# praateekmahajan/moving-mnist-vae

Hardware: AMD Instinct MI355X
Metric: frames/sec/GPU VAE train step, 20×64×64 batch; ELBO vs CPU ref (higher is better)
Workload: dtype bf16; 1 GPU; BASELINE configs[1]: 256 clips x 20 frames x 64x64 per GPU per step (=5120 frames), conv-VAE z=128, Gaussian NLL sigma=0.1 + KL (normal_vae_1_kl_0_mmd), Adam, random-init weights, Bernoulli(0.0521) q=2 labels; parallelism=dp1, rccl_ranks=1, grad_exchange=none, bn=per-rank batch statistics

## Files before the change

### include/mmvae.h

```cpp
#ifndef MMVAE_H_
#define MMVAE_H_

#include <stddef.h>
#include <stdint.h>

#ifdef __cplusplus
extern "C" {
#endif

#if defined(__GNUC__)
#define MMVAE_API __attribute__((visibility("default")))
#else
#define MMVAE_API
#endif

#define MMVAE_OK 0
#define MMVAE_ERR_ARG (-1)
#define MMVAE_ERR_HIP (-2)
#define MMVAE_ERR_WORKSPACE (-3)
#define MMVAE_ERR_UNSUPPORTED (-4)

#define MMVAE_F32 0
#define MMVAE_BF16 1
#define MMVAE_FP8 2

#define MMVAE_ABI_VERSION 3
MMVAE_API int mmvae_abi_version(void);
MMVAE_API const char* mmvae_last_error(void);

typedef struct mmvae_net mmvae_net;
MMVAE_API int mmvae_net_create(mmvae_net** out, int in_channels, int z_dimension, int out_channels, int image_size,
                     int need_logvar, int dtype);
MMVAE_API int mmvae_net_create_ex(mmvae_net** out, int in_channels, int z_dimension, int out_channels, int image_size,
                        int need_logvar, int dtype, int blocks_per_stage);
MMVAE_API void mmvae_net_destroy(mmvae_net* net);
MMVAE_API int mmvae_net_sizes(const mmvae_net* net, int64_t* n_params, int64_t* n_bn_f32, int32_t* n_bn_i64,
                    int64_t* decoder_param_offset, int32_t* decoder_side);
MMVAE_API int mmvae_net_num_entries(const mmvae_net* net);
MMVAE_API int mmvae_net_entry(const mmvae_net* net, int index, char* name, int name_cap, int32_t* ndim, int32_t shape[4],
                    int32_t* kind, int64_t* offset);
MMVAE_API size_t mmvae_net_workspace_bytes(mmvae_net* net, int N);

MMVAE_API int mmvae_encoder_fwd(mmvae_net* net, int N, const float* x, const float* params, float* bn_f32, int64_t* bn_i64,
                      void* workspace, size_t workspace_bytes, float* mu, float* logvar, int training, void* stream);
MMVAE_API int mmvae_net_stage_labels(mmvae_net* net, int N, const void* labels, int label_bytes, float mean, float stdv, float* image,
                           void* workspace, size_t workspace_bytes, void* stream);
MMVAE_API int mmvae_encoder_fwd_staged(mmvae_net* net, int N, const float* x, const float* params, float* bn_f32, int64_t* bn_i64,
                             void* workspace, size_t workspace_bytes, float* mu, float* logvar, int training, void* stream);
MMVAE_API int mmvae_encoder_bwd(mmvae_net* net, int N, const float* d_mu, const float* d_logvar, const float* params, float* grads,
                      void* workspace, size_t workspace_bytes, void* stream);
MMVAE_API int mmvae_decoder_fwd(mmvae_net* net, int N, const float* encoding, const float* params, float* bn_f32, int64_t* bn_i64,
                      void* workspace, size_t workspace_bytes, float* recon, int training, void* stream);
MMVAE_API int mmvae_decoder_bwd(mmvae_net* net, int N, const float* d_recon, const float* params, float* grads, void* workspace,
                      size_t workspace_bytes, float* d_encoding , void* stream);
MMVAE_API int mmvae_decoder_bwd_gauss(mmvae_net* net, int N, const float* target, float sigma, float coef, const float* gscale, const float* params,
                            float* grads, void* workspace, size_t workspace_bytes, float* d_enc, void* stream);

MMVAE_API int mmvae_net_defer_join(mmvae_net* net, int enable);
MMVAE_API int mmvae_net_join(mmvae_net* net, void* stream);
MMVAE_API void* mmvae_net_fork(mmvae_net* net, void* stream);
MMVAE_API void* mmvae_net_side_stream(mmvae_net* net);
MMVAE_API int mmvae_net_set_join_grad(mmvae_net* net, int enable);

typedef int (*mmvae_allreduce_fn)(float* buf, int64_t n, void* stream, void* user);
MMVAE_API int mmvae_net_set_sync_bn(mmvae_net* net, mmvae_allreduce_fn fn, void* user, int world);

typedef struct mmvae_comm mmvae_comm;
#define MMVAE_COMM_ID_BYTES 128
MMVAE_API int mmvae_comm_unique_id(void* id_host );
MMVAE_API int mmvae_comm_init(mmvae_comm** out, int world, int rank, const void* id_host);
MMVAE_API int mmvae_comm_allreduce(mmvae_comm* comm, float* buf, int64_t n, void* stream);
MMVAE_API int mmvae_comm_destroy(mmvae_comm* comm);
MMVAE_API int mmvae_net_set_sync_bn_comm(mmvae_net* net, mmvae_comm* comm);
MMVAE_API int mmvae_net_set_sync_bn_comm2(mmvae_net* net, mmvae_comm* comm_main, mmvae_comm* comm_side);

MMVAE_API int mmvae_rsample_fwd(const float* mu, const float* logvar, const float* eps, float* enc, int64_t n, void* stream);
MMVAE_API int mmvae_rsample_bwd(const float* d_enc, const float* logvar, const float* eps, float* d_mu, float* d_logvar, int64_t n,
                      void* stream);
#define MMVAE_SUM_PARTIALS 1025
MMVAE_API int mmvae_kl_fwd(const float* mu, const float* logvar, int64_t n, double* acc, void* stream);
MMVAE_API int mmvae_kl_fwd_ex(const float* mu, const float* logvar, int64_t n, double* acc, double* partials, void* stream);
MMVAE_API int mmvae_kl_bwd(const float* mu, const float* logvar, float coef, const float* gscale, float* d_mu, float* d_logvar, int64_t n,
                 void* stream);
MMVAE_API int mmvae_gauss_nll_fwd(const float* recon, const float* target, int64_t n, float sigma, double* acc, void* stream);
MMVAE_API int mmvae_gauss_nll_fwd_ex(const float* recon, const float* target, int64_t n, float sigma, double* acc, double* partials,
                                     void* stream);
MMVAE_API int mmvae_gauss_nll_bwd(const float* recon, const float* target, int64_t n, float sigma, float coef, const float* gscale,
                        float* d_recon, void* stream);
MMVAE_API int mmvae_ce_fwd(const float* recon, const int64_t* target, const float* weight, int N, int Q, int HW, double* acc, void* stream);
MMVAE_API int mmvae_ce_fwd_ex(const float* recon, const int64_t* target, const float* weight, int N, int Q, int HW, double* acc,
                              double* partials, void* stream);
MMVAE_API int mmvae_ce_bwd(const float* recon, const int64_t* target, const float* weight, int N, int Q, int HW, float coef,
                 const float* gscale, float* d_recon, void* stream);
MMVAE_API int mmvae_mmd_fwd(const float* x, const float* y, int n, int d, float* scratch, double* acc, void* stream);
MMVAE_API int mmvae_mmd_fwd_ex(const float* x, const float* y, int n, int d, float* scratch, double* acc, double* partials, void* stream);
MMVAE_API int mmvae_mmd_bwd(const float* x, const float* y, int n, int d, float coef, const float* gscale, float* d_y, void* stream);
MMVAE_API int mmvae_rbf_kernel(const float* x, const float* y, int n, int m, int d, float* out, void* stream);
MMVAE_API int mmvae_loss_finish(const double* acc, float* out, float nll, float kl_coef, float mmd_coef, float n, void* stream);

MMVAE_API int mmvae_gauss_nll_per_image(const float* recon, const float* target, int N, int64_t per, float sigma, double* out, void* stream);
MMVAE_API int mmvae_ce_per_image(const float* recon, const int64_t* target, const float* weight, int N, int Q, int HW, double* out, void* stream);
MMVAE_API int mmvae_kl_per_image(const float* mu, const float* logvar, int N, int d, double* out, void* stream);
MMVAE_API int mmvae_latent_logratio(const float* mu, const float* logvar, const float* eps, int N, int d, double* out, void* stream);
MMVAE_API int mmvae_iw_bound(const double* nll, const double* logratio, int K, int N, double* out, void* stream);

MMVAE_API int mmvae_normalise_labels(const int64_t* labels, int64_t n, float mean, float stdv, float* image, void* stream);
MMVAE_API int mmvae_quantise_normalise(const uint8_t* frames, int64_t n, const float* centres, int q, float mean, float stdv,
                             int64_t* labels, float* image, void* stream);
MMVAE_API int mmvae_u8_histogram(const uint8_t* frames, int64_t clip_bytes, const int64_t* clip_index, int64_t n_clips, uint64_t* counts,
                       void* stream);
MMVAE_API int mmvae_kmeans1d_fit(const uint64_t* counts, int q, double* centres, double* inertia);
MMVAE_API int mmvae_quantiser_stats(const uint64_t* counts, const float* centres, int q, uint8_t* lut, double* ratios, double* label_mean,
                          double* label_std);
MMVAE_API int mmvae_resample_coeffs(int in_size, int out_size, int* ksize, int32_t* bounds, int32_t* coeffs);
MMVAE_API int mmvae_resize_quantise_normalise(const uint8_t* frames, int64_t frame_stride_bytes, const int64_t* clip_index,
// ... 32 lines not shown
MMVAE_API int mmvae_scatter_panel(const float* pts, int64_t n, int stride, int col_x, int col_y, const float* xform, int side, int radius16,
                                  const uint8_t* tone, uint8_t* out, int64_t out_row_stride, void* stream);
MMVAE_API int mmvae_latent_stats(const float* mu, const float* logvar, const float* enc, int N, int d, int accumulate, double* acc,
                                 void* stream);

MMVAE_API size_t mmvae_nearest_frames_scratch_bytes(int M, int64_t F, int D, int k);
MMVAE_API int mmvae_nearest_frames(const uint8_t* queries, int M, const uint8_t* frames, int64_t F, int D, const uint8_t* lut, int k,
                                   int32_t* out_dist, int64_t* out_index, void* scratch, size_t scratch_bytes, void* stream);

#define MMVAE_TENSOR_HIST_BINS 64
#define MMVAE_TENSOR_HIST_STATS 8
MMVAE_API int64_t mmvae_tensor_hist_chunks(const int64_t* segments, int T, int64_t chunk_elems, int64_t* chunks, int64_t capacity);
MMVAE_API size_t mmvae_tensor_hist_scratch_bytes(int T, int64_t n_chunks);
MMVAE_API int mmvae_tensor_hist(const float* flat, int64_t flat_numel, const int64_t* segments, const int64_t* segments_dev, int T,
                                const int64_t* chunks, const int64_t* chunks_dev, int64_t n_chunks, int32_t* counts, float* lo, float* hi,
                                double* stats, void* scratch, size_t scratch_bytes, void* stream);

MMVAE_API int mmvae_adam_step(float* params, const float* grads, float* exp_avg, float* exp_avg_sq, int64_t n, float lr, float beta1,
                    float beta2, float eps, float weight_decay, float bc1, float bc2_sqrt, float grad_scale, void* stream);

MMVAE_API int mmvae_adam_step_dev(float* params, const float* grads, float* exp_avg, float* exp_avg_sq, int64_t n, float lr, float beta1,
                        float beta2, float eps, float weight_decay, double* step_dev, float grad_scale, void* stream);

MMVAE_API int mmvae_grad_norm_sq(const float* grads, int64_t n, float grad_scale, double* acc, double* partials, void* stream);

MMVAE_API int mmvae_adam_step_guarded(float* params, const float* grads, float* exp_avg, float* exp_avg_sq, int64_t n, float lr, float beta1,
                            float beta2, float eps, float weight_decay, double* state, double* partials, float grad_scale,
                            float max_norm, void* stream);

MMVAE_API int mmvae_conv2d_fwd(int dtype, int transposed, const void* x, const float* weight, void* y, int N, int H, int W, int Cin, int Cout,
                     int k, int stride, int pad, const float* pro_scale, const float* pro_shift, int pro_relu, float* stats,
                     void* scratch, void* stream);
MMVAE_API int mmvae_conv2d_dgrad(int dtype, int transposed, const void* dy, const float* weight, void* dx, int N, int H, int W, int Cin,
                       int Cout, int k, int stride, int pad, void* scratch, void* stream);
#define MMVAE_DGRAD_EX_W2_OFFSET(numel_w, esize) ((((size_t)(numel_w) * (esize) + 255) / 256) * 256)
#define MMVAE_DGRAD_EX_SCRATCH_BYTES(numel_w, numel_w2, esize) \
  ((numel_w2) > 0 ? MMVAE_DGRAD_EX_W2_OFFSET(numel_w, esize) + (size_t)(numel_w2) * (esize) : (size_t)(numel_w) * (esize))
MMVAE_API int mmvae_conv2d_dgrad_ex(int dtype, int transposed, const void* dy, const float* weight, void* dx, int N, int H, int W, int Cin,
                          int Cout, int k, int stride, int pad, int accumulate, const void* dy2, const float* w2, int C2, void* scratch,
                          void* stream);
#define MMVAE_WGRAD_SCRATCH_BYTES (64u << 20)
MMVAE_API int mmvae_conv2d_wgrad(int dtype, int transposed, const void* x, const void* dy, float* dweight, int N, int H, int W, int Cin,
                       int Cout, int k, int stride, int pad, const float* pro_scale, const float* pro_shift, int pro_relu,
                       void* scratch, void* stream);
MMVAE_API int mmvae_conv2d_wgrad_pair(int dtype, const void* x, const void* dy, const void* dy_shortcut, float* dweight, float* dweight_sc, int N,
                            int H, int W, int Cin, int Cout, const float* pro_scale, const float* pro_shift, int pro_relu, void* scratch,
                            void* stream);
#define MMVAE_BN_SCRATCH_BYTES (16u << 20)
MMVAE_API int mmvae_batchnorm_fwd(int dtype, const void* y, int64_t npix, int C, const float* gamma, const float* beta, float* running_mean,
                        float* running_var, int64_t* nbt, float momentum, float eps, int relu, void* out, float* save_mean, float* save_istd,
                        void* scratch, void* stream);
MMVAE_API int mmvae_batchnorm_bwd(int dtype, const void* dout, const void* y, const void* out, int64_t npix, int C, const float* gamma,
                        const float* save_mean, const float* save_istd, void* dy, float* dgamma, float* dbeta, void* scratch, void* stream);
#define MMVAE_STEM_SCRATCH_BYTES 12800u
MMVAE_API int mmvae_stem_fwd(int dtype, const void* x, const float* weight, void* y, int N, int S, float* stats, void* scratch, void* stream);
MMVAE_API int mmvae_stem_bwd(int dtype, const void* g, const void* y0, const void* x, const float* weight, const float* gamma,
                   const float* bn_scale, const float* bn_shift, const float* save_mean, const float* save_istd, float* dweight,
                   float* dgamma, float* dbeta, int N, int S, void* scratch, void* stream);
MMVAE_API int mmvae_convT_bwd_fused(int dtype, const void* x, const void* dy, const float* weight, float* dweight, void* dx, int N, int H, int W,
                          int Cin, int Cout, int k, int stride, int pad, const float* pro_scale, const float* pro_shift, int pro_relu,
                          const void* x2, const float* w2, float* dw2, void* scratch, void* wscratch, void* stream);
MMVAE_API int mmvae_tail_join_fwd(int dtype, const void* y2, const float* s2, const float* b2, const void* ys, const float* ss, const float* bs,
                        const float* weight, const float* bias, float* r_raw, float* stats, int N, int H, int W, void* stream);
MMVAE_API int mmvae_tail_join_fwd_stream(int dtype, const void* y2, const float* s2, const float* b2, const void* ys, const float* ss, const float* bs,
                               const float* weight, const float* bias, float* r_raw, float* stats, int N, int H, int W, void* stream);
MMVAE_API int mmvae_tail_join_bwd_reduce(int dtype, const float* d_raw, const float* weight, int out_planes, const void* y2, const float* s2,
                               const float* b2, const void* ys, const float* ss, const float* bs, float* partials, float* wpartials,
                               int N, int H, int W, void* stream);
MMVAE_API int mmvae_tail_join_bwd_apply(int dtype, const float* d_raw, const float* weight, int out_planes, const void* y2, const float* s2,
                              const float* b2, const void* ys, const float* ss, const float* bs, const float* A2, const float* B2,
                              const float* C2, const float* As, const float* Bs, const float* Cs, void* dy2, void* dys, int N, int H, int W,
                              void* stream);
MMVAE_API int mmvae_upblock_bwd_fused(const float* d_raw, const float* tail_weight, const void* y2, const float* s2, const float* b2,
                            const void* ys, const float* ss, const float* bs, const float* A2, const float* B2, const float* C2,
                            const float* As, const float* Bs, const float* Cs, const void* y1, const float* s1, const float* b1,
                            const float* w_conv2, float* dw_conv2, void* d_a1, float* bn1_sums, const void* xin, const float* sx,
                            const float* bx, const float* w_up, float* dw_up, void* g_in, int N, void* scratch, void* stream);
MMVAE_API int mmvae_upblock_tail_fwd(const void* y1, const float* s1, const float* b1, const float* w2, const void* x_in, const float* sx,
                                     const float* bx, const float* wu, const float* s2, const float* b2, const float* ss, const float* bs,
                                     const float* tail_weight, const float* tail_bias, float* r_raw, float* stats, int N, void* scratch,
                                     void* stream);
MMVAE_API int mmvae_upblock_tail_fwd_store(const void* y1, const float* s1, const float* b1, const float* w2, const void* x_in, const float* sx,
                                           const float* bx, const float* wu, const float* s2, const float* b2, const float* ss, const float* bs,
                                           const float* tail_weight, const float* tail_bias, float* r_raw, float* stats, void* y2, void* ys,
                                           int N, void* scratch, void* stream);
MMVAE_API int mmvae_convT4_stats(int dtype, const void* x, const float* weight, const float* pro_scale, const float* pro_shift, float* stats,
                                 int N, int e4m3_out, void* scratch, void* stream);
MMVAE_API int mmvae_join_conv1x1_fwd(const void* y2, const float* s2, const float* b2, const void* ys, const float* ss, const float* bs,
                           const float* w_conv1, int C, void* out, void* y1, float* stats, int64_t npix, void* scratch, void* stream);
MMVAE_API int mmvae_conv1x1_bwd_fused(const void* d_a1, const void* y1, const float* s1, const float* b1, const float* A1, const float* B1,
                            const float* C1, const void* xin, const float* sx, const float* bx, const float* w_conv1, float* dw_conv1,
                            void* g_in, int64_t rows, void* scratch, void* stream);
typedef struct mmvae_pixelcnn mmvae_pixelcnn;
MMVAE_API int mmvae_pixelcnn_create(mmvae_pixelcnn** out, int in_channels, int intermediate_channels, int out_channels, int layers, int dtype);
MMVAE_API void mmvae_pixelcnn_destroy(mmvae_pixelcnn* net);
MMVAE_API int64_t mmvae_pixelcnn_num_params(mmvae_pixelcnn* net);
MMVAE_API size_t mmvae_pixelcnn_workspace_bytes(mmvae_pixelcnn* net, int N, int S);
MMVAE_API int mmvae_pixelcnn_fwd(mmvae_pixelcnn* net, int N, int S, const float* x, const float* params, void* workspace, size_t workspace_bytes,
                       float* out, void* stream);
MMVAE_API int mmvae_pixelcnn_bwd(mmvae_pixelcnn* net, int N, int S, const float* x, const float* d_out, const float* params, float* grads,
                       void* workspace, size_t workspace_bytes, float* d_x, void* stream);
MMVAE_API size_t mmvae_pixelcnn_sample_workspace_bytes(mmvae_pixelcnn* net, int N, int S);
MMVAE_API int mmvae_pixelcnn_sample(mmvae_pixelcnn* net, int N, int S, const float* cond, int cond_channels, float* sample, int sample_channels,
                          const float* uniforms, float sub_mean, float data_std, const float* params, void* workspace, size_t workspace_bytes,
                          float* out_logits, float* probs, int64_t* labels, void* stream);

// ... 7 lines not shown
```

### moving-mnist-vae_amd/_lib.py

```python
from __future__ import annotations

import ctypes
import os
from ctypes import POINTER, c_char_p, c_double, c_float, c_int, c_int32, c_int64, c_size_t, c_uint64, c_void_p

import torch

_HERE = os.path.dirname(os.path.abspath(__file__))
LIB_PATH = os.environ.get("MMVAE_LIB_PATH") or os.path.join(_HERE, "libmmvae_hip.so")
_lib = None
ABI_VERSION = 3
SUM_PARTIALS = 1025
BN_SCRATCH_BYTES = 16 << 20
STEM_SCRATCH_BYTES = 12800

P = c_void_p

PROTOTYPES = {
    "mmvae_abi_version": (c_int, []),
    "mmvae_last_error": (c_char_p, []),
    "mmvae_net_create": (c_int, [POINTER(c_void_p), c_int, c_int, c_int, c_int, c_int, c_int]),
    "mmvae_net_create_ex": (c_int, [POINTER(c_void_p), c_int, c_int, c_int, c_int, c_int, c_int, c_int]),
    "mmvae_net_destroy": (None, [P]),
    "mmvae_net_sizes": (c_int, [P, POINTER(c_int64), POINTER(c_int64), POINTER(c_int32), POINTER(c_int64), POINTER(c_int32)]),
    "mmvae_net_num_entries": (c_int, [P]),
    "mmvae_net_entry": (c_int, [P, c_int, c_char_p, c_int, POINTER(c_int32), POINTER(c_int32), POINTER(c_int32), POINTER(c_int64)]),
    "mmvae_net_workspace_bytes": (c_size_t, [P, c_int]),
    "mmvae_encoder_fwd": (c_int, [P, c_int, P, P, P, P, P, c_size_t, P, P, c_int, P]),
    "mmvae_net_stage_labels": (c_int, [P, c_int, P, c_int, c_float, c_float, P, P, c_size_t, P]),
    "mmvae_encoder_fwd_staged": (c_int, [P, c_int, P, P, P, P, P, c_size_t, P, P, c_int, P]),
    "mmvae_encoder_bwd": (c_int, [P, c_int, P, P, P, P, P, c_size_t, P]),
    "mmvae_decoder_fwd": (c_int, [P, c_int, P, P, P, P, P, c_size_t, P, c_int, P]),
    "mmvae_decoder_bwd": (c_int, [P, c_int, P, P, P, P, c_size_t, P, P]),
    "mmvae_decoder_bwd_gauss": (c_int, [P, c_int, P, c_float, c_float, P, P, P, P, c_size_t, P, P]),
    "mmvae_net_defer_join": (c_int, [P, c_int]),
    "mmvae_net_join": (c_int, [P, P]),
    "mmvae_net_fork": (P, [P, P]),
    "mmvae_net_side_stream": (P, [P]),
    "mmvae_net_set_join_grad": (c_int, [P, c_int]),
    "mmvae_net_set_sync_bn": (c_int, [P, P, P, c_int]),
    "mmvae_rsample_fwd": (c_int, [P, P, P, P, c_int64, P]),
    "mmvae_rsample_bwd": (c_int, [P, P, P, P, P, c_int64, P]),
    "mmvae_kl_fwd": (c_int, [P, P, c_int64, P, P]),
    "mmvae_kl_fwd_ex": (c_int, [P, P, c_int64, P, P, P]),
    "mmvae_kl_bwd": (c_int, [P, P, c_float, P, P, P, c_int64, P]),
    "mmvae_gauss_nll_fwd": (c_int, [P, P, c_int64, c_float, P, P]),
    "mmvae_gauss_nll_fwd_ex": (c_int, [P, P, c_int64, c_float, P, P, P]),
    "mmvae_gauss_nll_bwd": (c_int, [P, P, c_int64, c_float, c_float, P, P, P]),
    "mmvae_ce_fwd": (c_int, [P, P, P, c_int, c_int, c_int, P, P]),
    "mmvae_ce_fwd_ex": (c_int, [P, P, P, c_int, c_int, c_int, P, P, P]),
    "mmvae_ce_bwd": (c_int, [P, P, P, c_int, c_int, c_int, c_float, P, P, P]),
    "mmvae_mmd_fwd": (c_int, [P, P, c_int, c_int, P, P, P]),
    "mmvae_mmd_fwd_ex": (c_int, [P, P, c_int, c_int, P, P, P, P]),
    "mmvae_mmd_bwd": (c_int, [P, P, c_int, c_int, c_float, P, P, P]),
    "mmvae_loss_finish": (c_int, [P, P, c_float, c_float, c_float, c_float, P]),
    "mmvae_gauss_nll_per_image": (c_int, [P, P, c_int, c_int64, c_float, P, P]),
    "mmvae_ce_per_image": (c_int, [P, P, P, c_int, c_int, c_int, P, P]),
    "mmvae_kl_per_image": (c_int, [P, P, c_int, c_int, P, P]),
    "mmvae_latent_logratio": (c_int, [P, P, P, c_int, c_int, P, P]),
    "mmvae_iw_bound": (c_int, [P, P, c_int, c_int, P, P]),
    "mmvae_normalise_labels": (c_int, [P, c_int64, c_float, c_float, P, P]),
    "mmvae_quantise_normalise": (c_int, [P, c_int64, P, c_int, c_float, c_float, P, P, P]),
    "mmvae_u8_histogram": (c_int, [P, c_int64, P, c_int64, P, P]),
    "mmvae_kmeans1d_fit": (c_int, [P, c_int, P, P]),
    "mmvae_quantiser_stats": (c_int, [P, P, c_int, P, P, P, P]),
    "mmvae_resample_coeffs": (c_int, [c_int, c_int, POINTER(c_int), P, P]),
    "mmvae_resize_quantise_normalise": (c_int, [P, c_int64, P, c_int, c_int64, c_int, c_int, c_int, c_int, P, P, c_int, P, P, c_int, P, c_int,
                                                c_float, c_float, P, P, P, P]),
    "mmvae_generate_clips": (c_int, [P, c_int64, c_int, P, c_uint64, c_int64, c_int64, c_int, c_int, c_int, P, c_int, c_float, c_float, P, P, P, P]),
    "mmvae_logits_to_labels": (c_int, [P, c_int, c_int, c_int, c_int, P, P, P]),
    "mmvae_panel_sheet": (c_int, [P, c_int, c_int, c_int, P, P]),
    "mmvae_scatter_panel": (c_int, [P, c_int64, c_int, c_int, c_int, P, c_int, c_int, P, P, c_int64, P]),
    "mmvae_latent_stats": (c_int, [P, P, P, c_int, c_int, c_int, P, P]),
    "mmvae_nearest_frames_scratch_bytes": (c_size_t, [c_int, c_int64, c_int, c_int]),
    "mmvae_nearest_frames": (c_int, [P, c_int, P, c_int64, c_int, P, c_int, P, P, P, c_size_t, P]),
    "mmvae_tensor_hist_chunks": (c_int64, [P, c_int, c_int64, P, c_int64]),
    "mmvae_tensor_hist_scratch_bytes": (c_size_t, [c_int, c_int64]),
    "mmvae_tensor_hist": (c_int, [P, c_int64, P, P, c_int, P, P, c_int64, P, P, P, P, P, c_size_t, P]),
    "mmvae_adam_step": (c_int, [P, P, P, P, c_int64, c_float, c_float, c_float, c_float, c_float, c_float, c_float, c_float, P]),
    "mmvae_adam_step_dev": (c_int, [P, P, P, P, c_int64, c_float, c_float, c_float, c_float, c_float, P, c_float, P]),
    "mmvae_grad_norm_sq": (c_int, [P, c_int64, c_float, P, P, P]),
    "mmvae_adam_step_guarded": (c_int, [P, P, P, P, c_int64, c_float, c_float, c_float, c_float, c_float, P, P, c_float, c_float, P]),
    "mmvae_conv2d_fwd": (c_int, [c_int, c_int, P, P, P, c_int, c_int, c_int, c_int, c_int, c_int, c_int, c_int, P, P, c_int, P, P, P]),
    "mmvae_conv2d_dgrad": (c_int, [c_int, c_int, P, P, P, c_int, c_int, c_int, c_int, c_int, c_int, c_int, c_int, P, P]),
    "mmvae_conv2d_dgrad_ex": (c_int, [c_int, c_int, P, P, P, c_int, c_int, c_int, c_int, c_int, c_int, c_int, c_int, c_int, P, P, c_int, P, P]),
    "mmvae_conv2d_wgrad": (c_int, [c_int, c_int, P, P, P, c_int, c_int, c_int, c_int, c_int, c_int, c_int, c_int, P, P, c_int, P, P]),
    "mmvae_conv2d_wgrad_pair": (c_int, [c_int, P, P, P, P, P, c_int, c_int, c_int, c_int, c_int, P, P, c_int, P, P]),
    "mmvae_rbf_kernel": (c_int, [P, P, c_int, c_int, c_int, P, P]),
    "mmvae_comm_unique_id": (c_int, [P]),
    "mmvae_comm_init": (c_int, [POINTER(c_void_p), c_int, c_int, P]),
    "mmvae_comm_allreduce": (c_int, [P, P, c_int64, P]),
    "mmvae_comm_destroy": (c_int, [P]),
    "mmvae_net_set_sync_bn_comm": (c_int, [P, P]),
    "mmvae_net_set_sync_bn_comm2": (c_int, [P, P, P]),
    "mmvae_convT_bwd_fused": (c_int, [c_int, P, P, P, P, P, c_int, c_int, c_int, c_int, c_int, c_int, c_int, c_int, P, P, c_int, P, P, P, P, P, P]),
    "mmvae_batchnorm_fwd": (c_int, [c_int, P, c_int64, c_int, P, P, P, P, P, c_float, c_float, c_int, P, P, P, P, P]),
    "mmvae_batchnorm_bwd": (c_int, [c_int, P, P, P, c_int64, c_int, P, P, P, P, P, P, P, P]),
    "mmvae_stem_fwd": (c_int, [c_int, P, P, P, c_int, c_int, P, P, P]),
    "mmvae_stem_bwd": (c_int, [c_int, P, P, P, P, P, P, P, P, P, P, P, P, c_int, c_int, P, P]),
    "mmvae_tail_join_fwd": (c_int, [c_int, P, P, P, P, P, P, P, P, P, P, c_int, c_int, c_int, P]),
    "mmvae_tail_join_fwd_stream": (c_int, [c_int, P, P, P, P, P, P, P, P, P, P, c_int, c_int, c_int, P]),
    "mmvae_tail_join_bwd_reduce": (c_int, [c_int, P, P, c_int, P, P, P, P, P, P, P, P, c_int, c_int, c_int, P]),
    "mmvae_tail_join_bwd_apply": (c_int, [c_int, P, P, c_int, P, P, P, P, P, P, P, P, P, P, P, P, P, P, c_int, c_int, c_int, P]),
    "mmvae_upblock_bwd_fused": (c_int, [P] * 27 + [c_int, P, P]),
    "mmvae_join_conv1x1_fwd": (c_int, [P, P, P, P, P, P, P, c_int, P, P, P, c_int64, P, P]),
    "mmvae_conv1x1_bwd_fused": (c_int, [P] * 13 + [c_int64, P, P]),
    "mmvae_upblock_tail_fwd": (c_int, [P] * 16 + [c_int, P, P]),
    "mmvae_upblock_tail_fwd_store": (c_int, [P] * 18 + [c_int, P, P]),
    "mmvae_convT4_stats": (c_int, [c_int, P, P, P, P, P, c_int, c_int, P, P]),
    "mmvae_pixelcnn_create": (c_int, [POINTER(c_void_p), c_int, c_int, c_int, c_int, c_int]),
    "mmvae_pixelcnn_destroy": (None, [P]),
    "mmvae_pixelcnn_num_params": (c_int64, [P]),
    "mmvae_pixelcnn_workspace_bytes": (c_size_t, [P, c_int, c_int]),
    "mmvae_pixelcnn_fwd": (c_int, [P, c_int, c_int, P, P, P, c_size_t, P, P]),
    "mmvae_pixelcnn_bwd": (c_int, [P, c_int, c_int, P, P, P, P, P, c_size_t, P, P]),
    "mmvae_pixelcnn_sample_workspace_bytes": (c_size_t, [P, c_int, c_int]),
    "mmvae_pixelcnn_sample": (c_int, [P, c_int, c_int, P, c_int, P, c_int, P, c_float, c_float, P, P, c_size_t, P, P, P, P]),
    "mmvae_convert": (c_int, [c_int, c_int, P, P, c_int64, P]),
}


class MmvaeError(RuntimeError):
    pass


PICK_ARGMAX, PICK_SAMPLE = 0, 1
PANEL_LABELS_U8, PANEL_LABELS_I64, PANEL_LOGITS_ARGMAX, PANEL_LOGITS_SAMPLE, PANEL_IMAGE_F32 = range(5)
PANEL_MAX_COLS, PANEL_MAX_Q, PANEL_MAX_S = 8, 16, 64
SCATTER_MAX_SIDE, SCATTER_MIN_RADIUS16, SCATTER_MAX_RADIUS16 = 512, 12, 128
LATENT_STATS_ROWS, LATENT_STATS_MAX_D = 6, 512
NEAREST_MAX_M, NEAREST_MAX_K, NEAREST_MAX_D = 64, 8, 16384
CLIPGEN_MAX_G, CLIPGEN_MAX_T, CLIPGEN_MAX_K, CLIPGEN_MAX_D, CLIPGEN_DIRECTIONS = 32, 32, 4, 1 << 24, 4096


class PanelCol(ctypes.Structure):
    _fields_ = [("kind", c_int32), ("src", c_void_p), ("Q", c_int32), ("uniforms", c_void_p), ("lut", c_void_p), ("lo", c_float),
                ("hi", c_float)]


def lib():
    global _lib
    if _lib is not None:
        return _lib
    if not os.path.exists(LIB_PATH):
        raise MmvaeError(
            f"{LIB_PATH} is missing: the HIP extension has not been built. "
            "Run `python -c 'import __graft_entry__ as g; g.build()'` (or `make -C moving-mnist-vae_amd/csrc`). "
            "There is no CPU fallback for the product path.")
    l = ctypes.CDLL(LIB_PATH)
    l.mmvae_abi_version.restype, l.mmvae_abi_version.argtypes = c_int, []
# ... 45 lines not shown
```

### moving-mnist-vae_amd/csrc/bn_elem.hip

```cpp
#include "kernels.hpp"
#include "tile_common.hpp"
#include <cstdlib>

namespace mmvae {

constexpr int kElemMaxBlocks = 768;

__host__ __device__ inline int block_threads_for(int cvecs) {
  int b = 256 - (256 % cvecs);
  return b < cvecs ? cvecs : b;
}

static int elem_blocks(long nvec, int threads) {
  constexpr int cap = kElemMaxBlocks;
  long b = (nvec + (long)threads * 4 - 1) / ((long)threads * 4);
  if (b < 1) b = 1;
  if (b > cap) b = cap;
  return (int)b;
}

template <int NV, int VE>
__device__ __forceinline__ void block_channel_reduce(float (&vals)[NV][VE], int cvecs, int C, float* smem, float* out) {
  const int t = threadIdx.x;
#pragma unroll
// ... 266 lines not shown
      if (MODE == 3) { float x = a0[j] * msc[j] + msh[j]; x += a1[j] * msc1[j] + msh1[j]; on = x > 0.f; }
      const float gg = on ? g[j] : 0.f;
      acc[0][j] += gg;
      acc[1][j] += gg * a0[j];
      if (NY == 2) acc[2][j] += gg * a1[j];
    }
  }
  block_channel_reduce<1 + NY, VE>(acc, cvecs, C, smem, partials + (long)blockIdx.x * (1 + NY) * C);
}

template <typename T>
static int launch_bn_bwd_reduce_t(const void* dout, const void* out, const float* ms, const float* mb, const float* ms1,
                                  const float* mb1, const void* y0, const void* y1, long npix, int C, float* partials, hipStream_t s) {
  constexpr int VE = Elem<T>::kVec;
  if (C % VE) { set_error("bn_bwd_reduce: C=%d not a multiple of %d", C, VE); return MMVAE_ERR_UNSUPPORTED; }
  const int cvecs = C / VE, threads = block_threads_for(cvecs);
  const long nvec = npix * cvecs;
  int blocks = elem_blocks(nvec, threads);
  if (blocks > 1024) blocks = 1024;
  const int ny = y1 ? 2 : 1;
  const size_t sm = (size_t)threads * (1 + ny) * VE * sizeof(float);
  const int mode = out ? 0 : (ms ? ((ms1 && ny == 2) ? 3 : 1) : 2);
#define MMVAE_LAUNCH(NY, MODE) hipLaunchKernelGGL((bn_bwd_reduce_kernel<T, NY, MODE>), dim3(blocks), dim3(threads), sm, s, \
    (const T*)dout, (const T*)out, ms, mb, ms1, mb1, (const T*)y0, (const T*)y1, nvec, C, partials)
  if (ny == 2) { if (mode == 0) MMVAE_LAUNCH(2, 0); else if (mode == 1) MMVAE_LAUNCH(2, 1); else if (mode == 3) MMVAE_LAUNCH(2, 3); else MMVAE_LAUNCH(2, 2); }
  else { if (mode == 0) MMVAE_LAUNCH(1, 0); else if (mode == 1) MMVAE_LAUNCH(1, 1); else MMVAE_LAUNCH(1, 2); }
#undef MMVAE_LAUNCH
  note_launch_bytes((double)npix * C * sizeof(T) * (1 + ny + (out ? 1 : 0)));
  int rc = check_launch("bn_bwd_reduce");
  return rc ? rc : blocks;
}
int launch_bn_bwd_reduce(int dt, const void* dout, const void* out, const float* msk_scale, const float* msk_shift,
                         const void* y0, const void* y1, long npix, int C, float* partials, hipStream_t s,
                         const float* msk_scale1, const float* msk_shift1) {
  return dt == DT_F32 ? launch_bn_bwd_reduce_t<float>(dout, out, msk_scale, msk_shift, msk_scale1, msk_shift1, y0, y1, npix, C, partials, s)
                      : launch_bn_bwd_reduce_t<bf16_t>(dout, out, msk_scale, msk_shift, msk_scale1, msk_shift1, y0, y1, npix, C, partials, s);
}

__global__ void bn_bwd_finalize_kernel(BnBwdFinalizeArgs a0, BnBwdFinalizeArgs a1) {
  const BnBwdFinalizeArgs& a = blockIdx.y ? a1 : a0;
  __shared__ double sRed[2 * 4];
  const int c = blockIdx.x;
  const int rows = 1 + a.ny;
  double s0 = 0.0, s1 = 0.0;
  strided_pair_sum<8>(a.partials + c, a.partials + (long)(1 + a.which) * a.C + c, (long)rows * a.C, a.nparts, s0, s1);
  s0 = wave_sum_d(s0); s1 = wave_sum_d(s1);
  const int lane = threadIdx.x & 63, wid = threadIdx.x >> 6;
  if (lane == 0) { sRed[wid] = s0; sRed[4 + wid] = s1; }
  __syncthreads();
  if (threadIdx.x == 0) {
    const int nw = blockDim.x >> 6;
    s0 = 0.0; s1 = 0.0;
    for (int w = 0; w < nw; ++w) { s0 += sRed[w]; s1 += sRed[4 + w]; }
    const double mean = a.mean[c], istd = a.istd[c], g = a.gamma ? a.gamma[c] : 1.0;
    const double sgy = istd * (s1 - mean * s0);
    if (a.dgamma) a.dgamma[c] += (float)sgy;
    if (a.dbeta) a.dbeta[c] += (float)s0;
    const double m1 = s0 / a.count, m2 = sgy / a.count;
    const double A = g * istd;
    const float Af = (float)A, Bf = (float)(-A * m2 * istd), Cf = (float)(-A * m1 + A * m2 * istd * mean);
    a.coefA[c] = Af;
    a.coefB[c] = Bf;
    a.coefC[c] = Cf;
    if (a.dbias_conv) a.dbias_conv[c] += (float)(((double)Af * s0 + (double)Bf * (mean * a.count) + (double)Cf * a.count) * (double)a.dbias_scale);
  }
}
int launch_bn_bwd_finalize(const BnBwdFinalizeArgs& a, hipStream_t s) {
  hipLaunchKernelGGL(bn_bwd_finalize_kernel, dim3(a.C), dim3(256), 0, s, a, a);
  return check_launch("bn_bwd_finalize");
}
int launch_bn_bwd_finalize2(const BnBwdFinalizeArgs& a0, const BnBwdFinalizeArgs& a1, hipStream_t s) {
  if (a0.C != a1.C) { set_error("bn_bwd_finalize2: channel counts differ"); return MMVAE_ERR_ARG; }
  hipLaunchKernelGGL(bn_bwd_finalize_kernel, dim3(a0.C, 2), dim3(256), 0, s, a0, a1);
  return check_launch("bn_bwd_finalize2");
}

template <typename T, int NY, int MODE>
__global__ void bn_bwd_apply_kernel(const T* __restrict__ dout, const T* __restrict__ out, const float* __restrict__ ms,
                                    const float* __restrict__ mb, const float* __restrict__ ms1, const float* __restrict__ mb1,
                                    const T* __restrict__ y0, const float* __restrict__ A0,
                                    const float* __restrict__ B0, const float* __restrict__ C0, T* __restrict__ dy0,
                                    const T* __restrict__ y1, const float* __restrict__ A1, const float* __restrict__ B1,
                                    const float* __restrict__ C1, T* __restrict__ dy1, long nvec, int C) {
  constexpr int VE = Elem<T>::kVec;
  const int cvecs = C / VE;
  const int cg = (int)(((long)blockIdx.x * blockDim.x + threadIdx.x) % cvecs);
  float msc[VE], msh[VE], msc1[VE], msh1[VE], a0[VE], b0[VE], c0[VE], a1[VE], b1[VE], c1[VE];
#pragma unroll
  for (int j = 0; j < VE; ++j) {
    const int ch = cg * VE + j;
    msc[j] = (MODE == 1 || MODE == 3) ? ms[ch] : 0.f; msh[j] = (MODE == 1 || MODE == 3) ? mb[ch] : 0.f;
    msc1[j] = MODE == 3 ? ms1[ch] : 0.f; msh1[j] = MODE == 3 ? mb1[ch] : 0.f;
    a0[j] = A0[ch]; b0[j] = B0[ch]; c0[j] = C0[ch];
    a1[j] = NY == 2 ? A1[ch] : 0.f; b1[j] = NY == 2 ? B1[ch] : 0.f; c1[j] = NY == 2 ? C1[ch] : 0.f;
  }
  const long stride = (long)gridDim.x * blockDim.x;
  for (long v = (long)blockIdx.x * blockDim.x + threadIdx.x; v < nvec; v += stride) {
    float g[VE], o[VE], f0[VE], f1[VE], r0[VE], r1[VE];
    Elem<T>::unpack(reinterpret_cast<const Vec16*>(dout)[v], g);
    Elem<T>::unpack(reinterpret_cast<const Vec16*>(y0)[v], f0);
    if (MODE == 0) Elem<T>::unpack(reinterpret_cast<const Vec16*>(out)[v], o);
    if (NY == 2) Elem<T>::unpack(reinterpret_cast<const Vec16*>(y1)[v], f1);
#pragma unroll
    for (int j = 0; j < VE; ++j) {
      bool on = true;
      if (MODE == 0) on = o[j] > 0.f;
// ... 714 lines not shown
int launch_affine_nchw(const float* raw, const float* scale, const float* shift, float* out, int N, int C, int HW, hipStream_t s) {
  const long total = (long)N * C * HW;
  const int blocks = elem_blocks(total / 4 + 1, 256);
  hipLaunchKernelGGL(affine_nchw_kernel, dim3(blocks), dim3(256), 0, s, raw, scale, shift, out, total, C, HW);
  note_launch_bytes((double)total * 8.0);
  return check_launch("affine_nchw");
}
__global__ __launch_bounds__(256) void gauss_tail_reduce_kernel(const float* __restrict__ raw, const float* __restrict__ tgt, const float* __restrict__ scale,
                                                                 const float* __restrict__ shift, float k, const float* __restrict__ gs, int N, int C,
                                                                 int HW, float* __restrict__ partials) {
  extern __shared__ float sm[];
  float* sAcc = sm;
  const int wid = threadIdx.x >> 6;
  if (gs) k *= gs[0];
  for (int i = threadIdx.x; i < 4 * 2 * C; i += blockDim.x) sAcc[i] = 0.f;
  __syncthreads();
  const int planes = N * C;
  for (int p = blockIdx.x; p < planes; p += gridDim.x) {
    const int c = p % C;
    const float sc = scale[c], sh = shift[c];
    const float* pa = raw + (long)p * HW;
    const float* pt = tgt + (long)p * HW;
    float v0 = 0.f, v1 = 0.f;
    if ((HW & 3) == 0) {
      for (int i = threadIdx.x * 4; i < HW; i += 4 * blockDim.x) {
        const float4 x = *reinterpret_cast<const float4*>(pa + i);
        const float4 t = *reinterpret_cast<const float4*>(pt + i);
        const float d0 = k * ((sc * x.x + sh) - t.x), d1 = k * ((sc * x.y + sh) - t.y), d2 = k * ((sc * x.z + sh) - t.z), d3 = k * ((sc * x.w + sh) - t.w);
        v0 += (d0 + d1) + (d2 + d3);
        v1 += (d0 * x.x + d1 * x.y) + (d2 * x.z + d3 * x.w);
      }
    } else {
      for (int i = threadIdx.x; i < HW; i += blockDim.x) {
        const float x = pa[i], d = k * ((sc * x + sh) - pt[i]);
        v0 += d; v1 += d * x;
      }
    }
    v0 = wave_sum(v0); v1 = wave_sum(v1);
    if ((threadIdx.x & 63) == 0) { sAcc[wid * 2 * C + c] += v0; sAcc[wid * 2 * C + C + c] += v1; }
  }
  __syncthreads();
  for (int i = threadIdx.x; i < 2 * C; i += blockDim.x)
    partials[(long)blockIdx.x * 2 * C + i] = (sAcc[i] + sAcc[2 * C + i]) + (sAcc[2 * 2 * C + i] + sAcc[3 * 2 * C + i]);
}
int launch_gauss_tail_reduce(const float* raw, const float* target, const float* scale, const float* shift, float sigma, float coef, const float* gscale,
                             int N, int C, int HW, float* partials, hipStream_t s) {
  const int blocks = nchw_parts(N, C);
  const size_t sm = (size_t)4 * 2 * C * sizeof(float);
  hipLaunchKernelGGL(gauss_tail_reduce_kernel, dim3(blocks), dim3(256), sm, s, raw, target, scale, shift, coef / (sigma * sigma), gscale, N, C, HW, partials);
  note_launch_bytes((double)N * C * HW * 8.0);
  const int rc = check_launch("gauss_tail_reduce");
  return rc ? rc : blocks;
}
__global__ __launch_bounds__(256) void gauss_tail_apply_kernel(const float* __restrict__ raw, const float* __restrict__ tgt, const float* __restrict__ scale,
                                                                const float* __restrict__ shift, float k, const float* __restrict__ gs,
                                                                const float* __restrict__ A, const float* __restrict__ B, const float* __restrict__ Cc,
                                                                float* __restrict__ dy, int planes, int C, int HW) {
  if (gs) k *= gs[0];
  for (int p = blockIdx.x; p < planes; p += gridDim.x) {
    const int c = p % C;
    const float sc = scale[c], sh = shift[c], ca = A[c], cb = B[c], cc = Cc[c];
    const long base = (long)p * HW;
    if ((HW & 3) == 0) {
      for (int i = threadIdx.x * 4; i < HW; i += 1024) {
        const float4 x = *reinterpret_cast<const float4*>(raw + base + i);
        const float4 t = *reinterpret_cast<const float4*>(tgt + base + i);
        float4 o;
        o.x = ca * (k * ((sc * x.x + sh) - t.x)) + cb * x.x + cc; o.y = ca * (k * ((sc * x.y + sh) - t.y)) + cb * x.y + cc;
        o.z = ca * (k * ((sc * x.z + sh) - t.z)) + cb * x.z + cc; o.w = ca * (k * ((sc * x.w + sh) - t.w)) + cb * x.w + cc;
        *reinterpret_cast<float4*>(dy + base + i) = o;
      }
    } else {
      for (int i = threadIdx.x; i < HW; i += 256) {
        const float x = raw[base + i];
        dy[base + i] = ca * (k * ((sc * x + sh) - tgt[base + i])) + cb * x + cc;
      }
    }
  }
}
int launch_gauss_tail_apply(const float* raw, const float* target, const float* scale, const float* shift, float sigma, float coef, const float* gscale,
                            const float* A, const float* B, const float* Cc, float* dy, int N, int C, int HW, hipStream_t s) {
  if (C > 64) { set_error("gauss_tail_apply: C=%d > 64", C); return MMVAE_ERR_UNSUPPORTED; }
  const int planes = N * C;
  const int blocks = planes < 4096 ? planes : 4096;
  hipLaunchKernelGGL(gauss_tail_apply_kernel, dim3(blocks), dim3(256), 0, s, raw, target, scale, shift, coef / (sigma * sigma), gscale, A, B, Cc, dy, planes, C, HW);
  note_launch_bytes((double)N * C * HW * 12.0);
  return check_launch("gauss_tail_apply");
}

__global__ __launch_bounds__(256) void bn_bwd_apply_nchw_kernel(const float* __restrict__ dout, const float* __restrict__ y,
                                                                const float* __restrict__ A, const float* __restrict__ B,
                                                                const float* __restrict__ Cc, float* __restrict__ dy, int planes, int C,
                                                                int HW) {
  for (int p = blockIdx.x; p < planes; p += gridDim.x) {
    const int c = p % C;
    const float ca = A[c], cb = B[c], cc = Cc[c];
    const long base = (long)p * HW;
    if ((HW & 3) == 0) {
      for (int i = threadIdx.x * 4; i < HW; i += 1024) {
        const float4 d = *reinterpret_cast<const float4*>(dout + base + i);
        const float4 v = *reinterpret_cast<const float4*>(y + base + i);
        float4 o;
        o.x = ca * d.x + cb * v.x + cc; o.y = ca * d.y + cb * v.y + cc; o.z = ca * d.z + cb * v.z + cc; o.w = ca * d.w + cb * v.w + cc;
        *reinterpret_cast<float4*>(dy + base + i) = o;
      }
    } else {
      for (int i = threadIdx.x; i < HW; i += 256) dy[base + i] = ca * dout[base + i] + cb * y[base + i] + cc;
    }
  }
}
int launch_bn_bwd_apply_nchw(const float* dout, const float* y, const float* A, const float* B, const float* Cc, float* dy,
                             int N, int C, int HW, hipStream_t s) {
  if (C > 64) { set_error("bn_bwd_apply_nchw: C=%d > 64", C); return MMVAE_ERR_UNSUPPORTED; }
  const int planes = N * C;
  const int blocks = planes < 4096 ? planes : 4096;
  hipLaunchKernelGGL(bn_bwd_apply_nchw_kernel, dim3(blocks), dim3(256), 0, s, dout, y, A, B, Cc, dy, planes, C, HW);
  return check_launch("bn_bwd_apply_nchw");
}

}
```

### moving-mnist-vae_amd/csrc/capi.cpp

```cpp
#include <cstring>
#include <new>

#include "../../include/mmvae.h"
#include "conv_ops.hpp"
#include "pixel_net.hpp"
#include "quantiser_fit.hpp"
#include "resample.hpp"
#include "vae_net.hpp"

namespace mmvae { const char* last_error(); }
using namespace mmvae;

struct mmvae_net { Net* net; };
struct mmvae_comm { Comm* c; };

static inline hipStream_t stream_of(void* s) { return static_cast<hipStream_t>(s); }

extern "C" {

int mmvae_abi_version(void) { return MMVAE_ABI_VERSION; }
const char* mmvae_last_error(void) { return last_error(); }

int mmvae_net_create(mmvae_net** out, int in_channels, int z, int out_channels, int image_size, int need_logvar, int dtype) {
  return mmvae_net_create_ex(out, in_channels, z, out_channels, image_size, need_logvar, dtype, 1);
// ... 33 lines not shown
  const Entry& e = n->net->entries[i];
  if (name && cap > 0) { std::strncpy(name, e.name.c_str(), cap - 1); name[cap - 1] = 0; }
  if (ndim) *ndim = e.ndim;
  if (shape) for (int k = 0; k < 4; ++k) shape[k] = e.shape[k];
  if (kind) *kind = e.kind;
  if (offset) *offset = e.offset;
  return MMVAE_OK;
}
size_t mmvae_net_workspace_bytes(mmvae_net* n, int N) { return n && N > 0 ? n->net->workspace_bytes(N) : 0; }

int mmvae_encoder_fwd(mmvae_net* n, int N, const float* x, const float* params, float* bn_f32, int64_t* bn_i64, void* ws, size_t wsb,
                      float* mu, float* logvar, int training, void* stream) {
  if (!n || N <= 0 || !x || !params || !ws || !mu) { set_error("encoder_fwd: bad argument"); return MMVAE_ERR_ARG; }
  if (n->net->cfg.need_logvar && !logvar) { set_error("encoder_fwd: logvar required"); return MMVAE_ERR_ARG; }
  if (!bn_f32) { set_error("encoder_fwd: BN buffers required"); return MMVAE_ERR_ARG; }
  return n->net->encoder_fwd(N, x, params, bn_f32, reinterpret_cast<long long*>(bn_i64), ws, wsb, mu, logvar, training, stream_of(stream));
}
int mmvae_net_stage_labels(mmvae_net* n, int N, const void* labels, int label_bytes, float mean, float stdv, float* image, void* ws, size_t wsb,
                           void* stream) {
  if (!n || N <= 0 || !labels || !image || !ws) { set_error("net_stage_labels: bad argument"); return MMVAE_ERR_ARG; }
  return n->net->stage_labels(N, labels, label_bytes, mean, stdv, image, ws, wsb, stream_of(stream));
}
int mmvae_encoder_fwd_staged(mmvae_net* n, int N, const float* x, const float* params, float* bn_f32, int64_t* bn_i64, void* ws, size_t wsb,
                             float* mu, float* logvar, int training, void* stream) {
  if (!n || N <= 0 || !x || !params || !ws || !mu) { set_error("encoder_fwd_staged: bad argument"); return MMVAE_ERR_ARG; }
  if (n->net->cfg.need_logvar && !logvar) { set_error("encoder_fwd_staged: logvar required"); return MMVAE_ERR_ARG; }
  if (!bn_f32) { set_error("encoder_fwd_staged: BN buffers required"); return MMVAE_ERR_ARG; }
  return n->net->encoder_fwd(N, x, params, bn_f32, reinterpret_cast<long long*>(bn_i64), ws, wsb, mu, logvar, training, stream_of(stream), true);
}
int mmvae_encoder_bwd(mmvae_net* n, int N, const float* d_mu, const float* d_logvar, const float* params, float* grads, void* ws,
                      size_t wsb, void* stream) {
  if (!n || N <= 0 || !d_mu || !params || !grads || !ws) { set_error("encoder_bwd: bad argument"); return MMVAE_ERR_ARG; }
  if (n->net->cfg.need_logvar && !d_logvar) { set_error("encoder_bwd: d_logvar required"); return MMVAE_ERR_ARG; }
  return n->net->encoder_bwd(N, d_mu, d_logvar, params, grads, ws, wsb, stream_of(stream));
}
int mmvae_decoder_fwd(mmvae_net* n, int N, const float* enc, const float* params, float* bn_f32, int64_t* bn_i64, void* ws, size_t wsb,
                      float* recon, int training, void* stream) {
  if (!n || N <= 0 || !enc || !params || !ws || !recon || !bn_f32) { set_error("decoder_fwd: bad argument"); return MMVAE_ERR_ARG; }
  return n->net->decoder_fwd(N, enc, params, bn_f32, reinterpret_cast<long long*>(bn_i64), ws, wsb, recon, training, stream_of(stream));
}
int mmvae_decoder_bwd(mmvae_net* n, int N, const float* d_recon, const float* params, float* grads, void* ws, size_t wsb, float* d_enc,
                      void* stream) {
  if (!n || N <= 0 || !d_recon || !params || !grads || !ws) { set_error("decoder_bwd: bad argument"); return MMVAE_ERR_ARG; }
  return n->net->decoder_bwd(N, d_recon, params, grads, ws, wsb, d_enc, stream_of(stream));
}

int mmvae_decoder_bwd_gauss(mmvae_net* n, int N, const float* target, float sigma, float coef, const float* gscale, const float* params, float* grads,
                            void* ws, size_t wsb, float* d_enc, void* stream) {
  if (!n || N <= 0 || !target || !params || !grads || !ws || !(sigma > 0.f)) { set_error("decoder_bwd_gauss: bad argument"); return MMVAE_ERR_ARG; }
  const Net::GaussTail gt{target, sigma, coef, gscale};
  return n->net->decoder_bwd(N, nullptr, params, grads, ws, wsb, d_enc, stream_of(stream), &gt);
}

int mmvae_net_defer_join(mmvae_net* n, int enable) {
  if (!n) { set_error("net_defer_join: bad argument"); return MMVAE_ERR_ARG; }
  n->net->set_defer_join(enable != 0);
  return MMVAE_OK;
}
int mmvae_net_join(mmvae_net* n, void* stream) {
  if (!n) { set_error("net_join: bad argument"); return MMVAE_ERR_ARG; }
  return n->net->join(stream_of(stream));
}

void* mmvae_net_fork(mmvae_net* n, void* stream) {
  if (!n) return stream;
  return reinterpret_cast<void*>(n->net->fork(stream_of(stream)));
}

int mmvae_net_set_join_grad(mmvae_net* n, int enable) {
  if (!n) { set_error("net_set_join_grad: bad argument"); return MMVAE_ERR_ARG; }
  n->net->set_join_grad(enable != 0);
  return MMVAE_OK;
}

void* mmvae_net_side_stream(mmvae_net* n) { return n ? reinterpret_cast<void*>(n->net->side()) : nullptr; }

int mmvae_net_set_sync_bn(mmvae_net* n, mmvae_allreduce_fn fn, void* user, int world) {
  if (!n || (fn && world < 1)) { set_error("net_set_sync_bn: bad argument"); return MMVAE_ERR_ARG; }
  n->net->set_sync_bn(reinterpret_cast<mmvae::Net::AllReduceFn>(fn), user, world);
  return MMVAE_OK;
}

int mmvae_comm_unique_id(void* id) {
  if (!id) { set_error("comm_unique_id: bad argument"); return MMVAE_ERR_ARG; }
  return comm_unique_id(id);
}
int mmvae_comm_init(mmvae_comm** out, int world, int rank, const void* id) {
  if (!out || !id || world < 1 || rank < 0 || rank >= world) { set_error("comm_init: bad argument"); return MMVAE_ERR_ARG; }
  mmvae_comm* h = new (std::nothrow) mmvae_comm;
  if (!h) return MMVAE_ERR_ARG;
  h->c = nullptr;
  const int rc = comm_init(&h->c, world, rank, id);
  if (rc < 0) { delete h; return rc; }
  *out = h;
  return MMVAE_OK;
}
int mmvae_comm_allreduce(mmvae_comm* c, float* buf, int64_t n, void* st) {
  if (!c || (!buf && n > 0)) { set_error("comm_allreduce: bad argument"); return MMVAE_ERR_ARG; }
  return comm_allreduce_sum(c->c, buf, (long long)n, stream_of(st));
}
int mmvae_comm_destroy(mmvae_comm* c) {
  if (!c) return MMVAE_OK;
  const int rc = comm_destroy(c->c);
  delete c;
  return rc;
}
// ... 318 lines not shown
  if (rc == 0) { set_error("conv2d_wgrad_pair: shape not supported (bf16, 32 -> 32 channels, 32x32 -> 16x16)"); return MMVAE_ERR_UNSUPPORTED; }
  return rc < 0 ? rc : MMVAE_OK;
}
int mmvae_convT_bwd_fused(int dt, const void* x, const void* dy, const float* w, float* dw, void* dx, int N, int H, int W, int Cin, int Cout, int k,
                          int s, int p, const float* ps, const float* pb, int relu, const void* x2, const float* w2, float* dw2, void* scratch,
                          void* wscratch, void* st) {
  const ConvGeom g = geom_for(1, Cin, Cout, k, s, p);
  const int Ho = out_size(1, H, k, s, p), Wo = out_size(1, W, k, s, p);
  if (!scratch || !wscratch) { set_error("convT_bwd_fused: scratch buffers required"); return MMVAE_ERR_ARG; }
  if (!op_bwd_fusable(dt, g, N, H, W, Ho, Wo)) { set_error("convT_bwd_fused: shape not supported (bf16, 16 / 32 -> 16 channels, k4 s2 p1, 32x32 -> 64x64 or 16x16 -> 32x32)"); return MMVAE_ERR_UNSUPPORTED; }
  char* sc = static_cast<char*>(scratch);
  int rc = op_pack_down(dt, g, w, sc, stream_of(st)); if (rc < 0) return rc;
  const void* w2p = nullptr;
  if (x2 && w2) {
    PackArgs pa; std::memset(&pa, 0, sizeof(pa));
    pa.src = w2; pa.dst = sc + (size_t)Cin * Cout * k * k * dtype_size(dt); pa.cols = Cin; pa.K = 16; pa.ntaps = 1; pa.s_col = 16; pa.s_k = 1; pa.scale = 1.f; pa.tap_off[0] = 0;
    rc = launch_pack(dt, pa, stream_of(st)); if (rc < 0) return rc;
    w2p = pa.dst;
  }
  if (dw2 && !w2p) { set_error("convT_bwd_fused: dw2 needs x2 and w2"); return MMVAE_ERR_ARG; }
  rc = op_run_bwd_fused(dt, g, N, x, H, W, ps, pb, relu, dy, Ho, Wo, sc, dx, w2p ? x2 : nullptr, w2p, dw, stream_of(st), static_cast<float*>(wscratch), 1.f,
                        nullptr, dw2, 1.f);
  if (rc == 0) { set_error("convT_bwd_fused: not taken"); return MMVAE_ERR_UNSUPPORTED; }
  return rc < 0 ? rc : MMVAE_OK;
}
static_assert(MMVAE_BN_SCRATCH_BYTES >= (1024u * 3 * 512 + 8 * 512) * 4, "BatchNorm scratch: 1024 partial rows x 3 x C<=512 + coefficient rows");
int mmvae_batchnorm_fwd(int dt, const void* y, int64_t npix, int C, const float* gamma, const float* beta, float* rm, float* rv, int64_t* nbt,
                        float momentum, float eps, int relu, void* out, float* save_mean, float* save_istd, void* scratch, void* st) {
  if (!scratch || !save_mean || !save_istd || C < 1 || C > 512 || npix < 1) { set_error("batchnorm_fwd: bad arguments (C <= 512, scratch and save_* required)"); return MMVAE_ERR_ARG; }
  float* part = static_cast<float*>(scratch);
  float* coef = part + 1024L * 3 * 512;
  const int np = launch_chan_stats_nhwc(dt, y, npix, C, part, stream_of(st));
  if (np < 0) return np;
  BnFinalizeArgs f;
  f.partials = part; f.nparts = np; f.C = C; f.count = (double)npix; f.gamma = gamma; f.beta = beta; f.running_mean = rm; f.running_var = rv;
  f.nbt = reinterpret_cast<long long*>(nbt); f.mean = save_mean; f.istd = save_istd; f.scale = coef; f.shift = coef + C; f.momentum = momentum; f.eps = eps;
  int rc = launch_bn_finalize(f, stream_of(st));
  if (rc < 0) return rc;
  return launch_affine_act(dt, y, coef, coef + C, relu, out, npix, C, stream_of(st));
}
int mmvae_batchnorm_bwd(int dt, const void* dout, const void* y, const void* out, int64_t npix, int C, const float* gamma, const float* save_mean,
                        const float* save_istd, void* dy, float* dgamma, float* dbeta, void* scratch, void* st) {
  if (!scratch || C < 1 || C > 512 || npix < 1) { set_error("batchnorm_bwd: bad arguments (C <= 512, scratch required)"); return MMVAE_ERR_ARG; }
  float* part = static_cast<float*>(scratch);
  float* coef = part + 1024L * 3 * 512;
  const int np = launch_bn_bwd_reduce(dt, dout, out, nullptr, nullptr, y, nullptr, npix, C, part, stream_of(st));
  if (np < 0) return np;
  BnBwdFinalizeArgs f; std::memset(&f, 0, sizeof(f));
  f.partials = part; f.nparts = np; f.C = C; f.which = 0; f.ny = 1; f.count = (double)npix; f.gamma = gamma; f.mean = save_mean; f.istd = save_istd;
  f.dgamma = dgamma; f.dbeta = dbeta; f.coefA = coef; f.coefB = coef + C; f.coefC = coef + 2 * C;
  int rc = launch_bn_bwd_finalize(f, stream_of(st));
  if (rc < 0) return rc;
  return launch_bn_bwd_apply(dt, dout, out, nullptr, nullptr, y, coef, coef + C, coef + 2 * C, dy, nullptr, nullptr, nullptr, nullptr, nullptr, npix, C, stream_of(st));
}
static_assert(MMVAE_STEM_SCRATCH_BYTES >= 32 * 25 * 16, "stem scratch: 32 columns x 25 taps x one 16-byte vector of padded input channels");
int mmvae_stem_fwd(int dt, const void* x, const float* w, void* y, int N, int Sz, float* stats, void* scratch, void* st) {
  if (!scratch || N < 1 || Sz < 9 || Sz > 64) { set_error("stem_fwd: bad arguments"); return MMVAE_ERR_ARG; }
  if (stem_fwd_stream_ok(dt, Sz)) return launch_stem_fwd_stream(dt, x, w, y, stats, N, Sz, stream_of(st));
  const int H1 = (Sz + 4 - 5) / 2 + 1;
  const int cpad = dt == DT_F32 ? 4 : 8;
  PackArgs pa; std::memset(&pa, 0, sizeof(pa));
  pa.src = w; pa.dst = scratch;
  pa.cols = 32; pa.K = cpad; pa.K_valid = 1; pa.ntaps = 25; pa.s_col = 25; pa.s_k = 25; pa.scale = 1.f;
  for (int t = 0; t < 25; ++t) pa.tap_off[t] = t;
  int rc = launch_pack(dt, pa, stream_of(st));
  if (rc < 0) return rc;
  GatherArgs a; std::memset(&a, 0, sizeof(a));
  a.x = x; a.w = scratch; a.y = y; a.stats = stats;
  a.x_planar = 2; a.x_planes = 1;
  a.N = N; a.Hi = Sz; a.Wi = Sz; a.Cin = cpad; a.Ho = H1; a.Wo = H1; a.Cout = 32; a.SI = 2; a.SO = 1;
  a.nphase = 1; a.phases[0] = Phase{0, 0, H1, H1, 25, 0, 0};
  for (int kh = 0; kh < 5; ++kh) for (int kw = 0; kw < 5; ++kw) a.taps[kh * 5 + kw] = Tap{kh - 2, kw - 2};
  return launch_gather_gemm(dt, dt, a, stream_of(st));
}
int mmvae_stem_bwd(int dt, const void* g, const void* y0, const void* x, const float* w, const float* gamma, const float* bn_scale,
                   const float* bn_shift, const float* save_mean, const float* save_istd, float* dw, float* dgamma, float* dbeta, int N, int Sz,
                   void* scratch, void* st) {
  if (!scratch || N < 1) { set_error("stem_bwd: bad arguments"); return MMVAE_ERR_ARG; }
  if (!stem_bwd_fusable(Sz)) { set_error("stem_bwd: image size %d unsupported (64, 32, 16)", Sz); return MMVAE_ERR_UNSUPPORTED; }
  const int H1 = (Sz + 4 - 5) / 2 + 1;
  double* R = static_cast<double*>(scratch);
  float* gram = reinterpret_cast<float*>(R + 1024);
  const long gram_floats = 1024L * stem_bwd_part_floats();
  float* part = gram + gram_floats;
  const long part_floats = (long)(MMVAE_BN_SCRATCH_BYTES - 1024 * 8) / 4 - gram_floats;
  int rc = launch_stem_gram(dt, x, gram, gram_floats, R, N, Sz, H1, H1, stream_of(st));
  if (rc < 0) return rc;
  const int np = launch_stem_bwd(dt, g, y0, x, bn_scale, bn_shift, part, part_floats, N, Sz, H1, H1, stream_of(st));
  if (np < 0) return np;
  return launch_stem_bwd_finalize(part, np, R, w, nullptr, (double)N * H1 * H1, gamma, save_mean, save_istd, dgamma, dbeta, dw, stream_of(st));
}
int mmvae_tail_join_fwd(int dt, const void* y2, const float* s2, const float* b2, const void* ys, const float* ss, const float* bs,
                        const float* w, const float* bias, float* r_raw, float* stats, int N, int H, int W, void* st) {
  return launch_tail_join_fwd(dt, y2, s2, b2, ys, ss, bs, w, bias, r_raw, stats, N, H, W, stream_of(st));
}
int mmvae_tail_join_fwd_stream(int dt, const void* y2, const float* s2, const float* b2, const void* ys, const float* ss, const float* bs,
                               const float* w, const float* bias, float* r_raw, float* stats, int N, int H, int W, void* st) {
  return launch_tail_fwd_stream(dt, y2, s2, b2, ys, ss, bs, w, bias, r_raw, stats, N, H, W, stream_of(st));
}
int mmvae_tail_join_bwd_reduce(int dt, const float* d_raw, const float* w, int oc, const void* y2, const float* s2, const float* b2,
                               const void* ys, const float* ss, const float* bs, float* partials, float* wpartials, int N, int H, int W,
                               void* st) {
  return launch_tail_join_bwd_reduce(dt, d_raw, w, oc, N, H, W, s2, b2, ss, bs, y2, ys, partials, stream_of(st), wpartials);
}
int mmvae_tail_join_bwd_apply(int dt, const float* d_raw, const float* w, int oc, const void* y2, const float* s2, const float* b2,
                              const void* ys, const float* ss, const float* bs, const float* A2, const float* B2, const float* C2,
// ... 95 lines not shown
```

### moving-mnist-vae_amd/csrc/kernels.hpp

```cpp
#pragma once
#include "common.hpp"

namespace mmvae {

enum DType : int { DT_F32 = 0, DT_BF16 = 1 };
inline size_t dtype_size(int dt) { return dt == DT_F32 ? 4 : 2; }

struct Tap { int dh, dw; };
constexpr int kMaxTaps = 25;
constexpr int kMaxPhases = 4;
struct Phase { int ph, pw, Hq, Wq, ntaps, tap0; long w_off;  };
struct GatherArgs {
  const void* x; const void* w; void* y;
  const float* pro_scale; const float* pro_shift; int pro_relu;
  const float* bias;
  float* stats;
  int accumulate;
  int N, Hi, Wi, Cin, Ho, Wo, Cout;
  int SI, SO;
  int nphase; Phase phases[kMaxPhases]; Tap taps[kMaxTaps];
  int cin_vecs;
  int x_planar, x_planes;
  int y_planes;
  const void* x2; const void* w2; int Cin2, x2_ph, x2_pw;
// ... 139 lines not shown
bool stem_bwd_fusable(int S);
bool conv3_stream_ok(int dt, int Cin, int Cout, int k, int s, int p, int Hin, int Win);
int launch_conv3_stream_bwd(int dt, const void* dy, const void* w_flipped, void* dx, const void* ym, const float* ms, const float* mb, float* sums,
                            int N, int H, hipStream_t s);
int launch_conv3_stream(int dt, int stride, const void* x, const void* w, const void* wsc, void* y, void* ysc, const float* pro_scale,
                        const float* pro_shift, int pro_relu, float* stats, float* stats_sc, int N, int Ho, hipStream_t s);
bool convT4_stream_ok(int dt, int Cin, int Cout, int k, int s, int p, int Hin, int Win);
int launch_convT4_stream(int dt, const void* x, const void* w_up, void* y, const float* pro_scale, const float* pro_shift, int pro_relu, float* stats,
                         int N, int Hin, hipStream_t s, int f8out = 0);
bool tail_fwd_stream_ok(int dt, int OC, int H, int W);
int launch_tail_fwd_stream(int dt, const void* y2, const float* s2, const float* b2, const void* ys, const float* ss, const float* bs, const float* w,
                           const float* bias, float* r_raw, float* stats, int N, int H, int W, hipStream_t s, int f8in = 0);
bool up5_tail_fwd_ok(int dt, int OC, int C, int Cin, int Hin, int Hout);
int launch_up5_tail_fwd(const void* y1, const float* p1s, const float* p1b, const void* w2_up, const void* xin, const float* pxs, const float* pxb,
                        const void* wu_up, const float* s2, const float* b2, const float* ss, const float* bs, const float* w, const float* bias,
                        float* r_raw, float* stats, int N, hipStream_t s, void* y2 = nullptr, void* ys = nullptr);
bool stem_fwd_stream_ok(int dt, int S);
int launch_stem_fwd_stream(int dt, const void* x, const float* w, void* y, float* stats, int N, int S, hipStream_t s);
int stem_bwd_part_floats();
int launch_stem_gram(int dt, const void* x, float* scratch, long scratch_cap_floats, double* R, int N, int S, int Ho, int Wo, hipStream_t s);
int launch_stem_bwd(int dt, const void* g, const void* y0, const void* x, const float* ms, const float* mb, float* partials,
                    long partials_cap_floats, int N, int S, int Ho, int Wo, hipStream_t s);
bool stem_bwd_dg_ok(int dt, int S);
int launch_stem_bwd_dg(const void* dy1, const void* dys, const void* wd1, const void* wds, const void* y0, const void* x, const float* ms, const float* mb,
                       float* partials, long partials_cap_floats, int N, int S, int Ho, int Wo, hipStream_t s);
int launch_stem_bwd_finalize(const float* partials, int nparts, const double* R, const float* w, const float* global_sums, double count,
                             const float* gamma, const float* mean, const float* istd, float* dgamma, float* dbeta, float* dW, hipStream_t s);

int launch_chan_stats_nhwc(int dt, const void* y, long npix, int C, float* partials, hipStream_t s);
int chan_stats_parts(long npix, int C);
struct BnFinalizeArgs {
  float in_scale = 1.f;
  const float* partials; int nparts; int C; double count;
  const float* gamma; const float* beta; float* running_mean; float* running_var; long long* nbt;
  float* mean; float* istd; float* scale; float* shift; float momentum, eps;
};
int launch_bn_finalize(const BnFinalizeArgs& a, hipStream_t s);
int launch_partial_rowsum(const float* partials, int nparts, int width, float* out, hipStream_t s, int row_stride = 0);
struct BnFoldEntry { int g_off, b_off, rm_off, rv_off, scale_off, shift_off, C; float in_scale; };
constexpr int kBnFoldMax = 96;
struct BnFoldTable { BnFoldEntry e[kBnFoldMax]; };
int launch_bn_fold_eval(const BnFoldEntry* entries, int n, const float* params, const float* bnbuf, float* bnws, float eps, hipStream_t s);
int launch_join_fwd(int dt, const void* a, const float* sa, const float* ba, const void* b, const float* sb, const float* bb,
                    void* out, long npix, int C, hipStream_t s);
int launch_affine_act(int dt, const void* a, const float* sa, const float* ba, int relu, void* out, long npix, int C,
                      hipStream_t s);
int launch_bn_bwd_reduce(int dt, const void* dout, const void* out, const float* msk_scale, const float* msk_shift,
                         const void* y0, const void* y1, long npix, int C, float* partials, hipStream_t s,
                         const float* msk_scale1 = nullptr, const float* msk_shift1 = nullptr);
struct BnBwdFinalizeArgs {
  const float* partials; int nparts; int C; int which ; int ny; double count;
  const float* gamma; const float* mean; const float* istd; float* dgamma; float* dbeta; float* coefA; float* coefB; float* coefC;
  float* dbias_conv = nullptr; float dbias_scale = 1.f;
};
int launch_bn_bwd_finalize(const BnBwdFinalizeArgs& a, hipStream_t s);
int launch_bn_bwd_finalize2(const BnBwdFinalizeArgs& a0, const BnBwdFinalizeArgs& a1, hipStream_t s);
int launch_bn_bwd_apply(int dt, const void* dout, const void* out, const float* msk_scale, const float* msk_shift,
                        const void* y0, const float* A0, const float* B0, const float* C0, void* dy0,
                        const void* y1, const float* A1, const float* B1, const float* C1, void* dy1,
                        long npix, int C, hipStream_t s, const float* msk_scale1 = nullptr, const float* msk_shift1 = nullptr);
bool tail_join_fusable(int dt, int OC, int N, int H, int W);
int launch_tail_join_bwd_reduce(int dt, const float* d_raw, const float* w, int OC, int N, int H, int W, const float* ms, const float* mb,
                                const float* ms1, const float* mb1, const void* y0, const void* y1, float* partials, hipStream_t s,
                                float* wpartials = nullptr, int f8in = 0);
int launch_tail_wgrad_finalize(const float* wpartials, int nparts, float* dW, hipStream_t s);
int launch_tail_join_bwd_apply(int dt, const float* d_raw, const float* w, int OC, int N, int H, int W, const float* ms, const float* mb,
                               const float* ms1, const float* mb1, const void* y0, const float* A0, const float* B0, const float* C0, void* dy0,
                               const void* y1, const float* A1, const float* B1, const float* C1, void* dy1, hipStream_t s);
bool tail_fwd_fusable(int dt, int OC, int N, int H, int W);
int launch_tail_join_fwd(int dt, const void* y0, const float* ms, const float* mb, const void* y1, const float* ms1, const float* mb1,
                         const float* w, const float* bias, float* r_raw, float* stats, int N, int H, int W, hipStream_t s);
int launch_affine_nchw(const float* raw, const float* scale, const float* shift, float* out, int N, int C, int HW, hipStream_t s);
int launch_bn_bwd_reduce_nchw(const float* dout, const float* y, int N, int C, int HW, float* partials, hipStream_t s);
int launch_bn_bwd_apply_nchw(const float* dout, const float* y, const float* A, const float* B, const float* Cc, float* dy,
                             int N, int C, int HW, hipStream_t s);
int launch_gauss_tail_reduce(const float* raw, const float* target, const float* scale, const float* shift, float sigma, float coef, const float* gscale,
                             int N, int C, int HW, float* partials, hipStream_t s);
int launch_gauss_tail_apply(const float* raw, const float* target, const float* scale, const float* shift, float sigma, float coef, const float* gscale,
                            const float* A, const float* B, const float* Cc, float* dy, int N, int C, int HW, hipStream_t s);

int launch_inorm_planar_fwd(int dt, const float* x, void* xn16, float* stats, int N, int C, int HW, hipStream_t s);
int launch_inorm_planar2_fwd(int dt, const float* xa, int Ca, const float* xb, int Cb, void* xn16, float* stats, int N, int HW, hipStream_t s);
int launch_inorm_planar_bwd(int dt, const void* g16, const float* x, const float* stats, float* dx, int N, int C, int HW, hipStream_t s);
int launch_inorm_nhwc_fwd(int dt, const void* h, void* a, float* stats, int N, int C, int HW, int relu, hipStream_t s);
int launch_inorm_nhwc_bwd(int dt, const void* g, const void* h, const float* stats, void* dh, int N, int C, int HW, int relu, hipStream_t s);
int launch_nhwc16_to_planar(int dt, const void* o16, float* out, int N, int C, int HW, hipStream_t s);
int launch_planar_to_nhwc16(int dt, const float* in, void* o16, int N, int C, int HW, hipStream_t s);
int launch_planar_to_nhwc16(int dt, const void* in, int in_dt, void* o16, int N, int C, int HW, hipStream_t s);

struct PixelHeadArgs {
  const void* a;
  const void* w;
  const float* bias;
  const float* uniforms;
  float* sample;
  float* probs;
  long long* labels;
  int S, C, Q, ntaps, Cs, pix;
  float sub_mean, data_std;
};
int launch_pixel_head(int dt, const PixelHeadArgs& h, int N, hipStream_t s);

int launch_rsample_fwd(int dt, const float* mu, const float* logvar, const float* eps, float* enc_f32, void* enc_t, long n,
                       hipStream_t s);
int launch_rsample_bwd(const float* d_enc, const float* logvar, const float* eps, float* d_mu, float* d_logvar, long n, hipStream_t s);
int launch_kl_fwd(const float* mu, const float* logvar, long n, double* out, double* part, hipStream_t s);
int launch_kl_bwd(const float* mu, const float* logvar, float coef, const float* gscale, float* d_mu, float* d_logvar, long n, hipStream_t s);
int launch_gauss_nll_fwd(const float* r, const float* t, long n, float sigma, double* out, double* part, hipStream_t s);
int launch_gauss_nll_bwd(const float* r, const float* t, long n, float sigma, float coef, const float* gscale, float* d_r, hipStream_t s);
int launch_ce_fwd(const float* r, const long long* t, const float* w, int N, int Q, int HW, double* out, double* part, hipStream_t s);
int launch_ce_bwd(const float* r, const long long* t, const float* w, int N, int Q, int HW, float coef, const float* gscale, float* d_r,
                  hipStream_t s);
int launch_mmd_fwd(const float* x, const float* y, int n, int d, double* out, double* part, hipStream_t s);
int launch_mmd_fwd_mfma(const float* x, const float* y, int n, int d, float* scratch , double* out, double* part, hipStream_t s);
int launch_rbf_matrix(const float* x, const float* y, int n, int m, int d, float* out, hipStream_t s);
int launch_mmd_bwd(const float* x, const float* y, int n, int d, float coef, const float* gscale, float* d_y, hipStream_t s);

int launch_gauss_nll_per_image(const float* r, const float* t, int N, long per, float sigma, double* out, hipStream_t s);
int launch_ce_per_image(const float* r, const long long* t, const float* w, int N, int Q, int HW, double* out, hipStream_t s);
int launch_kl_per_image(const float* mu, const float* logvar, int N, int d, double* out, hipStream_t s);
int launch_latent_logratio(const float* mu, const float* logvar, const float* eps, int N, int d, double* out, hipStream_t s);
int launch_iw_bound(const double* nll, const double* logratio, int K, int N, double* out, hipStream_t s);

struct AdamArgs { float* p; const float* g; float* m; float* v; long n; float lr, beta1, beta2, eps, weight_decay; float bc1, bc2; float grad_scale; };
int launch_adam(const AdamArgs& a, hipStream_t s);
int launch_adam_dev(const AdamArgs& a, double* state, hipStream_t s);
int launch_grad_norm_sq(const float* g, long n, float grad_scale, double* acc, double* part, hipStream_t s);
int launch_adam_guarded(const AdamArgs& a, double* state, double* part, float max_norm, hipStream_t s);
int launch_normalise(int dt, const void* labels, int label_bytes, long n, float mean, float stdv, void* img_t, float* img_f32, hipStream_t s);
int launch_quantise_normalise(const unsigned char* frames, long n, const float* centres, int q, float mean, float stdv,
                              long long* labels, float* image, hipStream_t s);
int launch_u8_histogram(const unsigned char* frames, long clip_bytes, const long long* clip_index, long n_clips,
                        unsigned long long* counts, hipStream_t s);
int launch_resize_quantise_normalise(const unsigned char* frames, long frame_stride, const long long* clip_index, int frames_per_clip,
                                     long n_frames, int in_h, int in_w, int out_h, int out_w, const int* h_bounds, const int* h_coeffs,
                                     int h_ksize, const int* v_bounds, const int* v_coeffs, int v_ksize, const float* centres, int q,
                                     float mean, float stdv, long long* labels, float* image, unsigned char* resized, hipStream_t s);
constexpr int kClipGenMaxG = MMVAE_CLIPGEN_MAX_G, kClipGenMaxT = MMVAE_CLIPGEN_MAX_T, kClipGenMaxK = MMVAE_CLIPGEN_MAX_K;
constexpr long kClipGenMaxD = MMVAE_CLIPGEN_MAX_D;
int launch_generate_clips(const unsigned char* bank, long D, int G, const int* vel, unsigned long long seed, long first_clip, long n_clips,
                          int T, int S, int K, const float* centres, int q, float mean, float stdv, long long* labels, float* image,
                          unsigned char* bytes, hipStream_t s);
int launch_logits_to_labels(const float* logits, int N, int Q, int HW, int mode, const float* uniforms, long long* labels, hipStream_t s);
int launch_panel_sheet(const mmvae_panel_col* cols, int ncols, int n, int S, unsigned char* out, hipStream_t s);
int launch_scatter_panel(const float* pts, long n, int stride, int col_x, int col_y, const float* xform, int side, int radius16,
                         const unsigned char* tone, unsigned char* out, long out_row_stride, hipStream_t s);
int launch_latent_stats(const float* mu, const float* logvar, const float* enc, int N, int d, int accumulate, double* acc, hipStream_t s);
size_t nearest_frames_scratch_bytes(int M, long F, int D, int k);
int launch_nearest_frames(const unsigned char* queries, int M, const unsigned char* frames, long F, int D, const unsigned char* lut, int k,
                          int* out_dist, long long* out_index, void* scratch, size_t scratch_bytes, hipStream_t s);
long long tensor_hist_chunks(const long long* segments, int T, long long chunk_elems, long long* chunks, long long capacity);
size_t tensor_hist_scratch_bytes(int T, long long n_chunks);
int launch_tensor_hist(const float* flat, long long flat_numel, const long long* seg_host, const long long* seg_dev, int T,
                       const long long* chunk_host, const long long* chunk_dev, long long n_chunks, int* counts, float* lo, float* hi,
                       double* stats, void* scratch, size_t scratch_bytes, hipStream_t s);
int launch_convert(int dt_in, int dt_out, const void* in, void* out, long n, hipStream_t s);
int launch_fill_f32(float* p, float v, long n, hipStream_t s);
int launch_concat2_to_t(int dt, const float* a, const float* b, int rows, int ca, int cb, void* out, hipStream_t s);
int launch_loss_finish(const double* acc, float* out, float nll, float klc, float mmdc, float n, hipStream_t s);
int launch_partials_add(const float* partials, int nparts, int row_stride, int C, float* out, hipStream_t s);

}
```

### moving-mnist-vae_amd/csrc/latent_loss.hip

```cpp
#include "kernels.hpp"

namespace mmvae {

static int rblocks(long n, int cap = 1024) {
  long b = (n + 1023) / 1024;
  if (b < 1) b = 1;
  if (b > cap) b = cap;
  return (int)b;
}

constexpr int kSumBlocks = MMVAE_SUM_PARTIALS - 1;
static unsigned sum_grid(long blocks, const double* part) { return part ? (unsigned)(blocks < kSumBlocks ? blocks : kSumBlocks) : 1u; }
__device__ __forceinline__ void block_sum_ordered(double v, double* out, double* part, double extra = 0.0) {
  __shared__ double sred[4];
  __shared__ int last;
  v = wave_sum_d(v);
  const int lane = threadIdx.x & 63, wid = threadIdx.x >> 6;
  if (lane == 0) sred[wid] = v;
  __syncthreads();
  unsigned* ticket = reinterpret_cast<unsigned*>(part);
  if (threadIdx.x == 0) {
    double s = 0.0;
    for (int w = 0; w < (int)(blockDim.x >> 6); ++w) s += sred[w];
    if (!part) {
// ... 504 lines not shown
  block_sum_ordered(acc, out, part);
}
int launch_grad_norm_sq(const float* g, long n, float grad_scale, double* acc, double* part, hipStream_t s) {
  if (n <= 0) return MMVAE_OK;
  long head = (long)((16 - reinterpret_cast<uintptr_t>(g) % 16) % 16 / 4);
  if (head > n) head = n;
  hipLaunchKernelGGL(grad_norm_sq_kernel, dim3(sum_grid(rblocks((n - head) / 4 + 1, 256), part)), dim3(256), 0, s, g, n, head, grad_scale, acc, part);
  return check_launch("grad_norm_sq");
}
__global__ void adam_guarded_kernel(AdamArgs a, const double* state, float max_norm) {
  __shared__ float sbc[3];
  __shared__ int skip;
  if (threadIdx.x == 0) {
    const double nsq = state[3];
    skip = !isfinite(nsq);
    const double t = state[0] + 1.0;
    const double total = sqrt(nsq);
    const double clip = max_norm > 0.f ? fmin(1.0, (double)max_norm / (total + 1e-6)) : 1.0;
    sbc[0] = (float)(1.0 - pow((double)a.beta1, t));
    sbc[1] = (float)sqrt(1.0 - pow((double)a.beta2, t));
    sbc[2] = (float)((double)a.grad_scale * clip);
  }
  __syncthreads();
  if (skip) return;
  const float bc1 = sbc[0], bc2 = sbc[1], gscale = sbc[2];
  for (long i = (long)blockIdx.x * blockDim.x + threadIdx.x; i < a.n; i += (long)gridDim.x * blockDim.x) {
    float g = a.g[i] * gscale;
    float p = a.p[i];
    if (a.weight_decay != 0.f) g += a.weight_decay * p;
    float m = a.m[i], v = a.v[i];
    m = m + (g - m) * (1.0f - a.beta1);
    v = v * a.beta2 + (1.0f - a.beta2) * g * g;
    const float denom = sqrtf(v) / bc2 + a.eps;
    p = p - (a.lr / bc1) * (m / denom);
    a.p[i] = p; a.m[i] = m; a.v[i] = v;
  }
}
__global__ void adam_guard_tail_kernel(double* state) {
  const double nsq = state[3];
  state[1] = sqrt(nsq);
  if (isfinite(nsq)) state[0] += 1.0;
  else state[2] += 1.0;
  state[3] = 0.0;
}
int launch_adam_guarded(const AdamArgs& a, double* state, double* part, float max_norm, hipStream_t s) {
  if (a.n <= 0) return MMVAE_OK;
  const int rc = launch_grad_norm_sq(a.g, a.n, a.grad_scale, state + 3, part, s);
  if (rc != MMVAE_OK) return rc;
  hipLaunchKernelGGL(adam_guarded_kernel, dim3(rblocks(a.n, 2048)), dim3(256), 0, s, a, (const double*)state, max_norm);
  hipLaunchKernelGGL(adam_guard_tail_kernel, dim3(1), dim3(1), 0, s, state);
  return check_launch("adam_guarded");
}

template <typename T, typename TL>
__global__ void normalise_kernel(const TL* __restrict__ labels, long n, long nq, float mean, float stdv, T* __restrict__ img, float* __restrict__ img32) {
  for (long q = (long)blockIdx.x * blockDim.x + threadIdx.x; q < nq; q += (long)gridDim.x * blockDim.x) {
    float v[4];
    if constexpr (sizeof(TL) == 8) {
      const longlong2 a = reinterpret_cast<const longlong2*>(labels)[2 * q], b = reinterpret_cast<const longlong2*>(labels)[2 * q + 1];
      v[0] = (float)a.x; v[1] = (float)a.y; v[2] = (float)b.x; v[3] = (float)b.y;
    } else {
      const uchar4 a = reinterpret_cast<const uchar4*>(labels)[q];
      v[0] = (float)a.x; v[1] = (float)a.y; v[2] = (float)a.z; v[3] = (float)a.w;
    }
#pragma unroll
    for (int j = 0; j < 4; ++j) v[j] = (v[j] - mean) / stdv;
    if (img32) reinterpret_cast<float4*>(img32)[q] = make_float4(v[0], v[1], v[2], v[3]);
    if (img) {
      if constexpr (sizeof(T) == 4) reinterpret_cast<float4*>(img)[q] = make_float4(v[0], v[1], v[2], v[3]);
      else reinterpret_cast<uint2*>(img)[q] = make_uint2(pack2_bf16(v[0], v[1]), pack2_bf16(v[2], v[3]));
    }
  }
  for (long i = (nq << 2) + (long)blockIdx.x * blockDim.x + threadIdx.x; i < n; i += (long)gridDim.x * blockDim.x) {
    const float v = ((float)labels[i] - mean) / stdv;
    if (img) Elem<T>::store(img + i, v);
    if (img32) img32[i] = v;
  }
}
int launch_normalise(int dt, const void* labels, int label_bytes, long n, float mean, float stdv, void* img_t, float* img_f32, hipStream_t s) {
  if (n <= 0) return MMVAE_OK;
  if (label_bytes != 8 && label_bytes != 1) { set_error("normalise: labels must be int64 or uint8"); return MMVAE_ERR_ARG; }
  const bool aligned = reinterpret_cast<uintptr_t>(labels) % (label_bytes == 8 ? 16 : 4) == 0 && reinterpret_cast<uintptr_t>(img_f32) % 16 == 0 &&
                       reinterpret_cast<uintptr_t>(img_t) % (dt == DT_F32 ? 16 : 8) == 0;
  const long nq = aligned ? n >> 2 : 0;
  const dim3 g(rblocks(aligned ? (n >> 2) + 1 : n, 2048)), b(256);
  if (label_bytes == 8) {
    if (dt == DT_F32) hipLaunchKernelGGL((normalise_kernel<float, long long>), g, b, 0, s, (const long long*)labels, n, nq, mean, stdv, (float*)img_t, img_f32);
    else hipLaunchKernelGGL((normalise_kernel<bf16_t, long long>), g, b, 0, s, (const long long*)labels, n, nq, mean, stdv, (bf16_t*)img_t, img_f32);
  } else {
    if (dt == DT_F32) hipLaunchKernelGGL((normalise_kernel<float, unsigned char>), g, b, 0, s, (const unsigned char*)labels, n, nq, mean, stdv, (float*)img_t, img_f32);
    else hipLaunchKernelGGL((normalise_kernel<bf16_t, unsigned char>), g, b, 0, s, (const unsigned char*)labels, n, nq, mean, stdv, (bf16_t*)img_t, img_f32);
  }
  return check_launch("normalise");
}

__global__ void quantise_normalise_kernel(const unsigned char* __restrict__ frames, long n, const float* __restrict__ centres, int q,
                                          float mean, float stdv, long long* __restrict__ labels, float* __restrict__ image) {
  for (long i = (long)blockIdx.x * blockDim.x + threadIdx.x; i < n; i += (long)gridDim.x * blockDim.x) {
    const int best = quantise_byte(frames[i], centres, q);
    if (labels) labels[i] = best;
    if (image) image[i] = ((float)best - mean) / stdv;
  }
}
int launch_quantise_normalise(const unsigned char* frames, long n, const float* centres, int q, float mean, float stdv,
                              long long* labels, float* image, hipStream_t s) {
  if (n <= 0) return MMVAE_OK;
  if (q < 1 || q > 256) { set_error("quantise: q=%d out of range", q); return MMVAE_ERR_ARG; }
  hipLaunchKernelGGL(quantise_normalise_kernel, dim3(rblocks(n, 2048)), dim3(256), 0, s, frames, n, centres, q, mean, stdv, labels, image);
  return check_launch("quantise_normalise");
}

template <typename TI, typename TOo>
__global__ void convert_kernel(const TI* __restrict__ in, TOo* __restrict__ out, long n) {
  for (long i = (long)blockIdx.x * blockDim.x + threadIdx.x; i < n; i += (long)gridDim.x * blockDim.x)
    Elem<TOo>::store(out + i, Elem<TI>::load(in + i));
}
int launch_convert(int dt_in, int dt_out, const void* in, void* out, long n, hipStream_t s) {
  if (n <= 0) return MMVAE_OK;
  const dim3 g(rblocks(n, 2048)), b(256);
  if (dt_in == DT_F32 && dt_out == DT_F32) hipLaunchKernelGGL((convert_kernel<float, float>), g, b, 0, s, (const float*)in, (float*)out, n);
  else if (dt_in == DT_F32) hipLaunchKernelGGL((convert_kernel<float, bf16_t>), g, b, 0, s, (const float*)in, (bf16_t*)out, n);
  else if (dt_out == DT_F32) hipLaunchKernelGGL((convert_kernel<bf16_t, float>), g, b, 0, s, (const bf16_t*)in, (float*)out, n);
  else hipLaunchKernelGGL((convert_kernel<bf16_t, bf16_t>), g, b, 0, s, (const bf16_t*)in, (bf16_t*)out, n);
  return check_launch("convert");
}

__global__ void fill_f32_kernel(float* p, float v, long n) {
  const long i = (long)blockIdx.x * blockDim.x + threadIdx.x;
  if (i < n) p[i] = v;
}
int launch_fill_f32(float* p, float v, long n, hipStream_t s) {
  if (n <= 0) return MMVAE_OK;
  hipLaunchKernelGGL(fill_f32_kernel, dim3((unsigned)((n + 255) / 256)), dim3(256), 0, s, p, v, n);
  return check_launch("fill_f32");
}

template <typename T>
__global__ void concat2_kernel(const float* __restrict__ a, const float* __restrict__ b, int rows, int ca, int cb, T* __restrict__ out) {
  const long total = (long)rows * (ca + cb);
  for (long i = (long)blockIdx.x * blockDim.x + threadIdx.x; i < total; i += (long)gridDim.x * blockDim.x) {
    const int r = (int)(i / (ca + cb)), c = (int)(i - (long)r * (ca + cb));
    const float v = c < ca ? a[(long)r * ca + c] : b[(long)r * cb + (c - ca)];
    Elem<T>::store(out + i, v);
  }
// ... 39 lines not shown
```

### moving-mnist-vae_amd/csrc/vae_net.cpp

```cpp
#include "vae_net.hpp"

#include <algorithm>
#include <cmath>
#include <cstdlib>
#include <cstring>

#include "conv_ops.hpp"

namespace mmvae {

#define MM_TRY(expr)            \
  do {                          \
    int rc__ = (expr);          \
    if (rc__ < 0) return rc__;  \
  } while (0)

static inline long align_up(long v, long a) { return (v + a - 1) / a * a; }
static inline int down_size(int H, int k, int s, int p) { return conv_down_size(H, k, s, p); }

void Net::add_entry(const std::string& name, std::initializer_list<int> shape, int kind, long off) {
  Entry e; e.name = name; e.ndim = (int)shape.size(); e.kind = kind; e.offset = off;
  int i = 0; for (int d : shape) e.shape[i++] = d;
  for (; i < 4; ++i) e.shape[i] = 1;
  entries.push_back(e);
// ... 127 lines not shown

Net::~Net() {
  if (side_state_ != 1) return;
  if (side_) { (void)hipStreamSynchronize(side_); (void)hipStreamDestroy(side_); }
  for (hipEvent_t e : ev_) if (e) (void)hipEventDestroy(e);
  for (hipEvent_t e : blk_ev_) if (e) (void)hipEventDestroy(e);
  if (gram_ev_) (void)hipEventDestroy(gram_ev_);
  (void)hipGetLastError();
}

size_t Net::workspace_bytes(int N) { return plan(N).bytes; }

const Plan& Net::plan(int N) {
  if (plan_.N == N) return plan_;
  Plan P; P.N = N;
  long cur = 0, maxact = 0;
  const long e = (long)esz();
  auto take = [&](long bytes) { long o = cur; cur = align_up(cur + std::max(bytes, 16L), 256); return o; };
  auto act = [&](long elems) { maxact = std::max(maxact, elems * e); return take(elems * e); };
  P.x_t = act((long)N * cfg.in_ch * cfg.S * cfg.S);
  P.y0 = act((long)N * H1 * W1 * 32);
  for (Block& B : enc) {
    const long n = (long)N * B.Hout * B.Wout * B.C;
    B.y1 = act(n); B.y2 = act(n); B.ys = B.identity ? 0 : act(n); B.out = act(n);
  }
  P.enc_t = act((long)N * cfg.z);
  P.y0d = act((long)N * 4 * 128);
  P.act0d = cfg.blocks > 1 ? act((long)N * 4 * 128) : 0;
  for (Block& B : dec) {
    const long n = (long)N * B.Hout * B.Wout * B.C;
    B.y1 = act((long)N * B.Hin * B.Win * B.C); B.y2 = act(n); B.ys = B.identity ? 0 : act(n); B.out = act(n);
  }
  P.cvec = take(512 * 4);
  P.r_raw = take((long)N * cfg.out_ch * Sd * Sd * 4);
  P.d_raw = take((long)N * cfg.out_ch * Sd * Sd * 4);
  P.col = act(cfg.in_ch == 1 ? (long)N * H1 * W1 * 32 : (long)N * cfg.S * cfg.S * 16);
  P.packed = take(n_packed * e);
  P.bnws = take(n_bnws * 4);
  P.partials = take(2 * kPartialFloats * 4);
  P.syncbuf = take(2 * 1024 * 4);
  for (int i = 0; i < 2; ++i) P.g[i] = take(maxact);
  for (int i = 0; i < 2; ++i) { P.dy1[i] = take(maxact); P.dy2[i] = take(maxact); P.dys[i] = take(maxact); }
  for (int i = 0; i < 2; ++i) {
    const Block& B = enc[enc.size() - 2 + i];
    const long nb = (long)N * B.Hout * B.Wout * B.C * e;
    P.edy1[i] = take(nb); P.edy2[i] = take(nb); P.edys[i] = take(nb);
  }
  P.da1 = take(maxact);
  P.dh = take((long)N * 2 * cfg.z * e);
  P.wscratch = take((long)kWgradScratchBytes);
  P.wscratch2 = take(2L * 1024 * 4096 * 4);
  P.stem_R = take(1024 * 8);
  P.stem_gram = take(1024L * stem_bwd_part_floats() * 4);
  P.bytes = (size_t)cur;
  plan_ = P;
  return plan_;
}

int Net::begin_pass(Pass& ps, int N, void* ws, size_t ws_bytes, const float* params, float* grads, float* bnbuf, long long* nbt, bool training) {
  const Plan& P = plan(N);
  if (ws_bytes < P.bytes) { set_error("workspace too small: %zu < %zu", ws_bytes, P.bytes); return MMVAE_ERR_WORKSPACE; }
  ps.P = &P; ps.base = static_cast<char*>(ws); ps.params = params; ps.grads = grads; ps.bnbuf = bnbuf; ps.nbt = nbt; ps.N = N;
  ps.training = training; ps.esz = esz();
  ps.part = reinterpret_cast<float*>(ps.base + P.partials);
  ps.wscratch = reinterpret_cast<float*>(ps.base + P.wscratch);
  return MMVAE_OK;
}

int Net::fill_consts(const Pass& ps, hipStream_t s) {
  float* c = reinterpret_cast<float*>(ps.base + ps.P->cvec);
  MM_TRY(launch_fill_f32(c, 1.f, 256, s));
  return launch_fill_f32(c + 256, 0.f, 256, s);
}

static inline ConvGeom geom(const ConvW& w) { return ConvGeom{w.D0, w.D1, w.k, w.s, w.p}; }

int Net::pack_down(const Pass& ps, const ConvW& w, hipStream_t s) {
  return op_pack_down(dt(), geom(w), ps.params + w.off, ps.packed(w.packD), s, w.wscale, (w.fp8 && !w.tr) ? 1 : 0, w.fragD);
}
int Net::pack_up(const Pass& ps, const ConvW& w, hipStream_t s) {
  return op_pack_up(dt(), geom(w), ps.params + w.off, ps.packed(w.packU), s, w.wscale, (w.fp8 && w.tr) ? 1 : 0, w.fragU);
}
int Net::run_down(const Pass& ps, const ConvW& w, const void* L, int Hl, int Wl, void* S, int Hs, int Ws,
                  const float* pro_s, const float* pro_b, int relu, float* stats, int accumulate, int out_dt, hipStream_t s,
                  const ConvW* w2, const void* x2) {
  SecondSrc q;
  if (w2) { q.x2 = x2; q.w2 = ps.packed(w2->packU); q.Cin2 = w2->D0; }
  q.fp8 = (w.fp8 && !w.tr) ? 1 : 0;
  q.wfrag = w.fragD; q.wfrag2 = w2 ? w2->fragU : 0;
  return op_run_down(dt(), out_dt, geom(w), ps.packed(w.packD), ps.N, L, Hl, Wl, S, Hs, Ws, pro_s, pro_b, relu, stats, accumulate, s, q);
}
int Net::run_up(const Pass& ps, const ConvW& w, const void* S, int Hs, int Ws, void* L, int Hl, int Wl,
                const float* pro_s, const float* pro_b, int relu, float* stats, int accumulate, hipStream_t s,
                const ConvW* w2, const void* x2) {
  SecondSrc q;
  if (w2) { q.x2 = x2; q.w2 = ps.packed(w2->packU); q.Cin2 = w2->D0; }
  q.fp8 = (w.fp8 && w.tr) ? 1 : 0;
  q.wfrag = w.fragU; q.wfrag2 = w2 ? w2->fragU : 0;
  return op_run_up(dt(), geom(w), ps.packed(w.packU), ps.N, S, Hs, Ws, L, Hl, Wl, pro_s, pro_b, relu, stats, accumulate, s, q);
}
hipStream_t Net::wgrad_stream(hipStream_t s) {
  if (side_state_ == 0) {
    side_state_ = 1;
    bool ok = hipStreamCreateWithFlags(&side_, hipStreamNonBlocking) == hipSuccess;
    for (int i = 0; i < kForkEvents && ok; ++i) ok = hipEventCreateWithFlags(&ev_[i], hipEventDisableTiming) == hipSuccess;
    for (int i = 0; i < 16 && ok; ++i) ok = hipEventCreateWithFlags(&blk_ev_[i], hipEventDisableTiming) == hipSuccess;
// ... 82 lines not shown
}

int Net::bn_fwd(const Pass& ps, const Bn& bn, int nparts, double count, hipStream_t s, long part_off, float in_scale) {
  if (!ps.training) {
    if (eval_folded_) return MMVAE_OK;
    set_error("bn_eval: the entry point did not fold its BatchNorms"); return MMVAE_ERR_ARG;
  }
  BnFinalizeArgs a;
  a.in_scale = in_scale;
  a.partials = ps.part + part_off; a.nparts = nparts; a.C = bn.C; a.count = count;
  if (sync_bn_on()) {
    float* row = nullptr;
    MM_TRY(sync_rows(ps, a.partials, nparts, 2 * bn.C, s, &row));
    a.partials = row; a.nparts = 1; a.count = count * ar_world_;
  }
  a.gamma = ps.params + bn.g_off; a.beta = ps.params + bn.b_off;
  a.running_mean = ps.bnbuf ? ps.bnbuf + bn.rm_off : nullptr; a.running_var = ps.bnbuf ? ps.bnbuf + bn.rv_off : nullptr;
  a.nbt = ps.nbt ? ps.nbt + bn.nbt_idx : nullptr;
  const BnRows r = ps.rows(bn);
  a.mean = r.mean; a.istd = r.istd; a.scale = r.scale; a.shift = r.shift;
  a.momentum = 0.1f; a.eps = 1e-5f;
  return launch_bn_finalize(a, s);
}

int Net::fold_bn_eval(const Pass& ps, int which, hipStream_t s) {
  std::vector<BnFoldEntry> tab;
  auto add = [&](const Bn& bn, float in_scale) {
    BnFoldEntry e;
    e.g_off = (int)bn.g_off; e.b_off = (int)bn.b_off; e.rm_off = (int)bn.rm_off; e.rv_off = (int)bn.rv_off;
    e.scale_off = (int)bn.row(Bn::SCALE); e.shift_off = (int)bn.row(Bn::SHIFT); e.C = bn.C; e.in_scale = in_scale;
    tab.push_back(e);
  };
  if (which == 0) add(bn0, 1.f); else add(dbn0, dstem.wscale);
  for (const Block& B : which == 0 ? enc : dec) {
    add(B.b1, B.c1.wscale); add(B.b2, B.c2.wscale);
    if (!B.identity) add(B.bs, B.cs.wscale);
  }
  if (which == 1) add(bn_out, 1.f);
  MM_TRY(launch_bn_fold_eval(tab.data(), (int)tab.size(), ps.params, ps.bnbuf, reinterpret_cast<float*>(ps.base + ps.P->bnws), 1e-5f, s));
  eval_folded_ = true;
  return MMVAE_OK;
}

BnBwdFinalizeArgs Net::bwd_finalize_args(const Pass& ps, const Bn& bn, const float* partials, int nparts, int ny, int which,
                                         double count) const {
  const BnRows r = ps.rows(bn);
  BnBwdFinalizeArgs a;
  a.partials = partials; a.nparts = nparts; a.C = bn.C; a.which = which; a.ny = ny;
  a.count = count; a.gamma = ps.params + bn.g_off; a.mean = r.mean; a.istd = r.istd;
  a.dgamma = ps.grads + bn.g_off; a.dbeta = ps.grads + bn.b_off;
  a.coefA = r.A; a.coefB = r.B; a.coefC = r.C;
  return a;
}
int Net::bn_backward_coefs(const Pass& ps, const Bn& bn, int nparts, int ny, int which, double count, hipStream_t s, float* dbias_conv) {
  BnBwdFinalizeArgs l = bwd_finalize_args(ps, bn, ps.part, nparts, ny, which, count);
  if (!sync_bn_on()) l.dbias_conv = dbias_conv;
  MM_TRY(launch_bn_bwd_finalize(l, s));
  if (!sync_bn_on()) return MMVAE_OK;
  float* row = nullptr;
  MM_TRY(sync_rows(ps, ps.part, nparts, (1 + ny) * bn.C, s, &row));
  BnBwdFinalizeArgs g = bwd_finalize_args(ps, bn, row, 1, ny, which, count * ar_world_);
  g.dgamma = nullptr; g.dbeta = nullptr;
  g.dbias_conv = dbias_conv; g.dbias_scale = 1.f / (float)ar_world_;
  return launch_bn_bwd_finalize(g, s);
}
int Net::bn_backward_coefs_join(const Pass& ps, const Bn& b2, const Bn& bs, int nparts, double count, hipStream_t s) {
  MM_TRY(launch_bn_bwd_finalize2(bwd_finalize_args(ps, b2, ps.part, nparts, 2, 0, count),
                                 bwd_finalize_args(ps, bs, ps.part, nparts, 2, 1, count), s));
  if (!sync_bn_on()) return MMVAE_OK;
  float* row = nullptr;
  MM_TRY(sync_rows(ps, ps.part, nparts, 3 * b2.C, s, &row));
  BnBwdFinalizeArgs g2 = bwd_finalize_args(ps, b2, row, 1, 2, 0, count * ar_world_);
  BnBwdFinalizeArgs gs = bwd_finalize_args(ps, bs, row, 1, 2, 1, count * ar_world_);
  g2.dgamma = g2.dbeta = gs.dgamma = gs.dbeta = nullptr;
  return launch_bn_bwd_finalize2(g2, gs, s);
}

int Net::packs_enc_fwd(const Pass& ps, hipStream_t s) {
  {
    const int cpad = dt() == DT_F32 ? 4 : 8;
    PackArgs pa; std::memset(&pa, 0, sizeof(pa));
    pa.src = ps.params + stem.off; pa.dst = ps.packed(stem_pack);
    pa.cols = 32; pa.K = cpad; pa.K_valid = cfg.in_ch; pa.ntaps = 25; pa.s_col = 25 * cfg.in_ch; pa.s_k = 25; pa.scale = 1.f;
    for (int t = 0; t < 25; ++t) pa.tap_off[t] = t;
    MM_TRY(launch_pack(dt(), pa, s));
  }
  for (const Block& B : enc) {
    MM_TRY(pack_down(ps, B.c1, s));
    MM_TRY(pack_down(ps, B.c2, s));
    if (!B.identity) MM_TRY(pack_down(ps, B.cs, s));
  }
  const int nt = Hf * Wf;
  for (int h = 0; h < (cfg.need_logvar ? 2 : 1); ++h) {
    const ConvW& hw = h == 0 ? head_mu : head_lv;
    const long poff = h == 0 ? head_pack_mu : head_pack_lv;
    PackArgs pa; std::memset(&pa, 0, sizeof(pa));
    pa.src = ps.params + hw.off; pa.dst = ps.packed(poff);
    pa.cols = cfg.z; pa.K = 256; pa.ntaps = nt; pa.s_col = 256; pa.s_k = 1; pa.scale = 1.0f / nt;
    MM_TRY(launch_pack(dt(), pa, s));
  }
  return MMVAE_OK;
}

int Net::packs_enc_bwd(const Pass& ps, hipStream_t s) {
  const int Ch = cfg.need_logvar ? 2 * cfg.z : cfg.z;
  PackArgs pa; std::memset(&pa, 0, sizeof(pa));
  pa.src = ps.params + head_mu.off; pa.dst = ps.packed(head_pack_dg);
  pa.cols = 256; pa.K = Ch; pa.ntaps = 1; pa.s_col = 1; pa.s_k = 256; pa.scale = 1.0f / (Hf * Wf);
  MM_TRY(launch_pack(dt(), pa, s));
  for (const Block& B : enc) {
    MM_TRY(pack_up(ps, B.c2, s));
    MM_TRY(pack_up(ps, B.c1, s));
    if (!B.identity) MM_TRY(pack_up(ps, B.cs, s));
  }
  if (l1_dgrad_stream()) {
    const ConvW& w = enc[0].c2;
    PackArgs pf; std::memset(&pf, 0, sizeof(pf));
    pf.src = ps.params + w.off; pf.dst = ps.packed(l1c2_flip);
    pf.cols = 32; pf.K = 32; pf.ntaps = 9; pf.s_col = 9; pf.s_k = 32 * 9; pf.scale = w.wscale;
    for (int t = 0; t < 9; ++t) pf.tap_off[t] = 8 - t;
    MM_TRY(launch_pack(dt(), pf, s));
  }
  return MMVAE_OK;
}

int Net::packs_dec_fwd(const Pass& ps, hipStream_t s) {
  MM_TRY(pack_up(ps, dstem, s));
  for (const Block& B : dec) {
    MM_TRY(pack_down(ps, B.c1, s));
    if (B.identity) MM_TRY(pack_down(ps, B.c2, s));
    else { MM_TRY(pack_up(ps, B.c2, s)); MM_TRY(pack_up(ps, B.cs, s)); }
  }
  PackArgs pa; std::memset(&pa, 0, sizeof(pa));
  pa.src = ps.params + tail.off; pa.dst = ps.packed(tail_pack_f);
  pa.cols = 16; pa.cols_valid = cfg.out_ch; pa.K = 16; pa.ntaps = 9; pa.s_col = 144; pa.s_k = 9; pa.scale = 1.f;
  for (int t = 0; t < 9; ++t) pa.tap_off[t] = t;
  MM_TRY(launch_pack(dt(), pa, s));
  return MMVAE_OK;
}

int Net::packs_dec_bwd(const Pass& ps, bool need_denc, hipStream_t s) {
  PackArgs pa; std::memset(&pa, 0, sizeof(pa));
  pa.src = ps.params + tail.off; pa.dst = ps.packed(tail_pack_d);
  pa.cols = 16; pa.K = 8; pa.K_valid = cfg.out_ch; pa.ntaps = 9; pa.s_col = 9; pa.s_k = 144; pa.scale = 1.f;
  for (int t = 0; t < 9; ++t) pa.tap_off[t] = t;
  MM_TRY(launch_pack(dt(), pa, s));
  for (const Block& B : dec) {
    MM_TRY(pack_up(ps, B.c1, s));
    if (B.identity) MM_TRY(pack_up(ps, B.c2, s));
    else { MM_TRY(pack_down(ps, B.c2, s)); MM_TRY(pack_down(ps, B.cs, s)); }
  }
  if (need_denc) MM_TRY(pack_down(ps, dstem, s));
  return MMVAE_OK;
}

int Net::stage_labels(int N, const void* labels, int label_bytes, float mean, float stdv, float* image, void* ws, size_t ws_bytes, hipStream_t s) {
  Pass ps;
  MM_TRY(begin_pass(ps, N, ws, ws_bytes));
  return launch_normalise(dt(), labels, label_bytes, (long)N * cfg.in_ch * cfg.S * cfg.S, mean, stdv, ps.base + ps.P->x_t, image, s);
}

int Net::encoder_fwd(int N, const float* x, const float* params, float* bnbuf, long long* nbt, void* ws, size_t ws_bytes,
                     float* mu, float* logvar, int training, hipStream_t s, bool staged) {
  if (Hf > 2) { set_error("encoder: image size %d unsupported (final map %dx%d)", cfg.S, Hf, Wf); return MMVAE_ERR_UNSUPPORTED; }
  Pass ps;
  MM_TRY(begin_pass(ps, N, ws, ws_bytes, params, nullptr, bnbuf, nbt, training != 0));
  const Plan& P = *ps.P;
  char* const base = ps.base;
  float* const part = ps.part;
  float* stats = training ? part : nullptr;
  const int S = cfg.S;
  pack_batch_begin();
  MM_TRY(packs_enc_fwd(ps, s));
  MM_TRY(pack_batch_flush(dt(), s));
  eval_folded_ = false;
  gram_ready_ = false; gram_fwd_N_ = training ? N : 0; gram_fwd_ws_ = ws;
  if (!training) MM_TRY(fold_bn_eval(ps, 0, s));
  if (!staged) MM_TRY(launch_convert(DT_F32, dt(), x, base + P.x_t, (long)N * cfg.in_ch * S * S, s));
  int np;
  if (cfg.in_ch == 1 && stem_fwd_stream_ok(dt(), S)) {
    np = launch_stem_fwd_stream(dt(), base + P.x_t, params + stem.off, base + P.y0, stats, N, S, s);
  } else {
    const int cpad = dt() == DT_F32 ? 4 : 8;
    GatherArgs a; std::memset(&a, 0, sizeof(a));
    a.x = base + P.x_t; a.w = ps.packed(stem_pack); a.y = base + P.y0; a.stats = stats;
    a.x_planar = 2; a.x_planes = cfg.in_ch;
    a.N = N; a.Hi = S; a.Wi = S; a.Cin = cpad; a.Ho = H1; a.Wo = W1; a.Cout = 32; a.SI = 2; a.SO = 1;
    a.nphase = 1; a.phases[0] = Phase{0, 0, H1, W1, 25, 0, 0};
    for (int kh = 0; kh < 5; ++kh) for (int kw = 0; kw < 5; ++kw) a.taps[kh * 5 + kw] = Tap{kh - 2, kw - 2};
    np = launch_gather_gemm(dt(), dt(), a, s);
  }
  MM_TRY(np);
  MM_TRY(bn_fwd(ps, bn0, np, (double)N * H1 * W1, s));
  const void* xin = base + P.y0;
  const float* xs = ps.rows(bn0).scale;
  const float* xb = ps.rows(bn0).shift;
  if (cfg.blocks > 1) MM_TRY(fill_consts(ps, s));
  for (size_t i = 0; i < enc.size(); ++i) {
    Block& B = enc[i];
    const double cnt = (double)N * B.Hout * B.Wout;
    const BnRows r1 = ps.rows(B.b1), r2 = ps.rows(B.b2);
    const Shortcut sc = ps.shortcut(B, xin);
    const bool stream1 = !B.identity && !B.c1.fp8 && !B.cs.fp8 && B.cs.k == 1 && B.cs.s == 2 &&
                         conv3_stream_ok(dt(), B.Cin, B.C, B.c1.k, B.c1.s, B.c1.p, B.Hin, B.Win);
    const bool stream2 = !B.c2.fp8 && conv3_stream_ok(dt(), B.C, B.C, B.c2.k, B.c2.s, B.c2.p, B.Hout, B.Wout);
    const bool fork = !B.identity && !stream1;
    if (stream1) {
      np = launch_conv3_stream(dt(), 2, xin, ps.packed(B.c1.packD), ps.packed(B.cs.packD), base + B.y1,
                               base + B.ys, xs, xb, 1, stats, stats ? stats + kPartialFloats : nullptr, N, B.Hout, s);
      MM_TRY(np);
      MM_TRY(bn_fwd(ps, B.bs, np, cnt, s, kPartialFloats, B.cs.wscale));
      MM_TRY(bn_fwd(ps, B.b1, np, cnt, s, 0, B.c1.wscale));
// ... 132 lines not shown
                    base + dyso));
    cur ^= 1;
  }
  if (stem_bwd_fused()) {
    const long npix = (long)N * H1 * W1;
    const Block& B0 = enc[0];
    const int np = stem_dg_fused()
        ? launch_stem_bwd_dg(base + stem_dy1, base + stem_dys, ps.packed(B0.c1.packU), ps.packed(B0.cs.packU), base + P.y0, base + P.x_t,
                             r0.scale, r0.shift, part, kPartialFloats, N, cfg.S, H1, W1, s)
        : launch_stem_bwd(dt(), base + P.g[cur], base + P.y0, base + P.x_t, r0.scale, r0.shift, part, kPartialFloats, N, cfg.S, H1, W1, s);
    MM_TRY(np);
    const float* gsum = nullptr; double cnt = (double)npix;
    if (sync_bn_on()) {
      float* row = nullptr;
      MM_TRY(sync_rows(ps, part, np, 64, s, &row, stem_bwd_part_floats()));
      gsum = row; cnt *= ar_world_;
    }
    if (side_state_ == 1 && hipStreamWaitEvent(s, gram_ev_, 0) != hipSuccess) { set_error("side stream wait failed"); return MMVAE_ERR_HIP; }
    MM_TRY(launch_stem_bwd_finalize(part, np, reinterpret_cast<const double*>(base + P.stem_R), params + stem.off, gsum, cnt,
                                    params + bn0.g_off, r0.mean, r0.istd, grads + bn0.g_off, grads + bn0.b_off, grads + stem.off, s));
    return side_join(s);
  }
  MM_TRY(side_wait_mark(1, s));
  const int ds = 1;
  {
    const long npix = (long)N * H1 * W1;
    int np = launch_bn_bwd_reduce(dt(), base + P.g[cur], nullptr, r0.scale, r0.shift, base + P.y0, nullptr, npix, 32, part, s);
    MM_TRY(np);
    MM_TRY(bn_backward_coefs(ps, bn0, np, 1, 0, (double)npix, s));
    MM_TRY(launch_bn_bwd_apply(dt(), base + P.g[cur], nullptr, r0.scale, r0.shift, base + P.y0, r0.A, r0.B, r0.C, base + P.dy1[ds], nullptr,
                               nullptr, nullptr, nullptr, nullptr, npix, 32, s));
    MM_TRY(side_fork(s));
    hipStream_t wsm = wgrad_stream(s);
    WgradArgs a; std::memset(&a, 0, sizeof(a));
    a.P = base + P.dy1[ds]; a.dW = grads + stem.off; a.scratch = ps.wscratch;
    a.N = N; a.Hp = H1; a.Wp = W1; a.Ca = 32; a.scale = 1.f;
    if (cfg.in_ch > 1) {
      MM_TRY(launch_planar_to_nhwc16(dt(), static_cast<const void*>(base + P.x_t), dt(), base + P.col, N, cfg.in_ch, cfg.S * cfg.S, wsm));
      a.G = base + P.col; a.Hg = cfg.S; a.Wg = cfg.S; a.Cb = 16; a.Cb_valid = cfg.in_ch;
      a.stride = 2; a.pad = 2; a.ksz = 5; a.sA = 25 * cfg.in_ch; a.sB = 25; a.ntaps = 25;
      for (int t = 0; t < 25; ++t) a.tap_off[t] = t;
    } else {
      if (wsm == s) MM_TRY(launch_stem_im2col(dt(), base + P.x_t, base + P.col, N, cfg.S, cfg.S, H1, W1, wsm));
      a.G = base + P.col; a.Hg = H1; a.Wg = W1; a.Cb = 32; a.Cb_valid = 25;
      a.stride = 1; a.pad = 0; a.ksz = 1; a.sA = 25; a.sB = 1; a.ntaps = 1;
    }
    MM_TRY(launch_wgrad(dt(), a, wsm));
    MM_TRY(side_join(s));
  }
  return MMVAE_OK;
}

int Net::decoder_fwd(int N, const float* encv, const float* params, float* bnbuf, long long* nbt, void* ws, size_t ws_bytes,
                     float* recon, int training, hipStream_t s) {
  Pass ps;
  MM_TRY(begin_pass(ps, N, ws, ws_bytes, params, nullptr, bnbuf, nbt, training != 0));
  const Plan& P = *ps.P;
  char* const base = ps.base;
  float* const part = ps.part;
  float* stats = training ? part : nullptr;
  pack_batch_begin();
  MM_TRY(packs_dec_fwd(ps, s));
  MM_TRY(pack_batch_flush(dt(), s));
  eval_folded_ = false;
  if (!training) MM_TRY(fold_bn_eval(ps, 1, s));
  MM_TRY(launch_convert(DT_F32, dt(), encv, base + P.enc_t, (long)N * cfg.z, s));
  int np = run_up(ps, dstem, base + P.enc_t, 1, 1, base + P.y0d, 2, 2, nullptr, nullptr, 0, stats, 0, s);
  MM_TRY(np);
  MM_TRY(bn_fwd(ps, dbn0, np, (double)N * 4, s, 0, dstem.wscale));
  const void* xin = base + P.y0d;
  const float* xs = ps.rows(dbn0).scale;
  const float* xb = ps.rows(dbn0).shift;
  const int nd = (int)dec.size();
  if (cfg.blocks > 1) {
    MM_TRY(fill_consts(ps, s));
    MM_TRY(launch_affine_act(dt(), base + P.y0d, xs, xb, 1, base + P.act0d, (long)N * 4, 128, s));
    xin = base + P.act0d; xs = xb = nullptr;
  }
  int c1_done = 0;
  bool up5_route = false;
  if (nd > 0 && tail_fwd_fused()) {
    const Block& B = dec.back();
    up5_route = !store8 && !B.identity && !B.c2.fp8 && !B.cs.fp8 && tail_fwd_stream_ok(dt(), cfg.out_ch, Sd, Sd) &&
                up5_tail_fwd_ok(dt(), cfg.out_ch, B.C, B.Cin, B.Hin, B.Hout) && convT4_stream_ok(dt(), B.c2.D0, B.c2.D1, B.c2.k, B.c2.s, B.c2.p, B.Hin, B.Win) &&
                convT4_stream_ok(dt(), B.cs.D0, B.cs.D1, B.cs.k, B.cs.s, B.cs.p, B.Hin, B.Win);
  }
  for (int i = 0; i < nd; ++i) {
    Block& B = dec[i];
    const double cnt = (double)N * B.Hout * B.Wout;
    const BnRows r1 = ps.rows(B.b1), r2 = ps.rows(B.b2);
    const Shortcut sc = ps.shortcut(B, xin);
    const bool stats_only = up5_route && i == nd - 1;
    if (!B.identity) {
      MM_TRY(side_fork(s));
      hipStream_t ss = wgrad_stream(s);
      if (stats_only && !stats) np = 1;
      else if (!B.cs.fp8 && convT4_stream_ok(dt(), B.cs.D0, B.cs.D1, B.cs.k, B.cs.s, B.cs.p, B.Hin, B.Win))
        np = launch_convT4_stream(dt(), xin, ps.packed(B.cs.packU), stats_only ? nullptr : base + B.ys, xs, xb, 1, stats ? stats + kPartialFloats : nullptr,
                                  N, B.Hin, ss, (store8 && i == nd - 1) ? 1 : 0);
      else
        np = run_up(ps, B.cs, xin, B.Hin, B.Win, base + B.ys, B.Hout, B.Wout, xs, xb, 1, stats ? stats + kPartialFloats : nullptr, 0, ss);
      MM_TRY(np);
      MM_TRY(bn_fwd(ps, B.bs, np, cnt, ss, kPartialFloats, B.cs.wscale));
    }
    np = c1_done > 0 ? c1_done : run_down(ps, B.c1, xin, B.Hin, B.Win, base + B.y1, B.Hin, B.Win, xs, xb, 1, stats, 0, dt(), s);
    c1_done = 0;
    MM_TRY(np);
    MM_TRY(bn_fwd(ps, B.b1, np, (double)N * B.Hin * B.Win, s, 0, B.c1.wscale));
    if (B.identity)
      np = run_down(ps, B.c2, base + B.y1, B.Hin, B.Win, base + B.y2, B.Hout, B.Wout, r1.scale, r1.shift, 1, stats, 0, dt(), s);
    else
      if (stats_only && !stats) np = 1;
      else if (!B.c2.fp8 && convT4_stream_ok(dt(), B.c2.D0, B.c2.D1, B.c2.k, B.c2.s, B.c2.p, B.Hin, B.Win))
        np = launch_convT4_stream(dt(), base + B.y1, ps.packed(B.c2.packU), stats_only ? nullptr : base + B.y2, r1.scale, r1.shift, 1, stats, N, B.Hin, s,
                                  (store8 && i == nd - 1) ? 1 : 0);
      else
        np = run_up(ps, B.c2, base + B.y1, B.Hin, B.Win, base + B.y2, B.Hout, B.Wout, r1.scale, r1.shift, 1, stats, 0, s);
    MM_TRY(np);
    MM_TRY(bn_fwd(ps, B.b2, np, cnt, s, 0, B.c2.wscale));
    if (!B.identity) MM_TRY(side_join(s));
    if (i == nd - 1 && tail_fwd_fused()) break;
    if (i == nd - 1 && store8) { set_error("fp8 storage of the last up-block needs the fused tail kernels"); return MMVAE_ERR_UNSUPPORTED; }
    const bool fuse_c1 = i + 1 < nd && !B.identity && !dec[i + 1].identity && !dec[i + 1].c1.fp8 && dec[i + 1].c1.k == 1 && dec[i + 1].c1.s == 1 &&
                         dec[i + 1].c1.D1 == B.C && !dec[i + 1].c1.fragD && dec[i + 1].c1.wscale == 1.f &&
                         join_conv1_fwd_ok(dt(), B.C, dec[i + 1].c1.D0, (long)N * B.Hout * B.Wout);
    if (fuse_c1) {
      c1_done = launch_join_conv1_fwd(B.C, base + B.y2, r2.scale, r2.shift, sc.y, sc.scale, sc.shift, ps.packed(dec[i + 1].c1.packD),
                                      base + B.out, base + dec[i + 1].y1, stats, (long)N * B.Hout * B.Wout, s);
      MM_TRY(c1_done);
    } else
    MM_TRY(launch_join_fwd(dt(), base + B.y2, r2.scale, r2.shift, sc.y, sc.scale, sc.shift, base + B.out,
                           (long)N * B.Hout * B.Wout, B.C, s));
    xin = base + B.out; xs = xb = nullptr;
  }
  float* r_raw = reinterpret_cast<float*>(base + P.r_raw);
  if (tail_fwd_fused()) {
    const Block& B = dec.back();
    const BnRows r1 = ps.rows(B.b1), r2 = ps.rows(B.b2);
    const Shortcut sc = ps.shortcut(B, xin);
    if (up5_route)
      np = launch_up5_tail_fwd(base + B.y1, r1.scale, r1.shift, ps.packed(B.c2.packU), xin, xs, xb, ps.packed(B.cs.packU), r2.scale, r2.shift,
                               sc.scale, sc.shift, params + tail.off, params + tail_bias, r_raw, stats, N, s,
                               stats ? base + B.y2 : nullptr, stats ? base + B.ys : nullptr);
    else if (tail_fwd_stream_ok(dt(), cfg.out_ch, Sd, Sd))
      np = launch_tail_fwd_stream(dt(), base + B.y2, r2.scale, r2.shift, sc.y, sc.scale, sc.shift, params + tail.off, params + tail_bias,
                                  r_raw, stats, N, Sd, Sd, s, store8 ? 1 : 0);
    else if (store8) { set_error("fp8 storage of the last up-block needs tail_fwd_stream"); return MMVAE_ERR_UNSUPPORTED; }
    else
      np = launch_tail_join_fwd(dt(), base + B.y2, r2.scale, r2.shift, sc.y, sc.scale, sc.shift, params + tail.off, params + tail_bias,
                                r_raw, stats, N, Sd, Sd, s);
  } else {
    GatherArgs a; std::memset(&a, 0, sizeof(a));
    a.x = xin; a.w = ps.packed(tail_pack_f); a.y = r_raw; a.bias = params + tail_bias; a.stats = stats; a.y_planes = cfg.out_ch;
    a.N = N; a.Hi = Sd; a.Wi = Sd; a.Cin = 16; a.Ho = Sd; a.Wo = Sd; a.Cout = 16; a.SI = 1; a.SO = 1;
    a.nphase = 1; a.phases[0] = Phase{0, 0, Sd, Sd, 9, 0, 0};
    for (int kh = 0; kh < 3; ++kh) for (int kw = 0; kw < 3; ++kw) a.taps[kh * 3 + kw] = Tap{kh - 1, kw - 1};
    np = launch_gather_gemm(dt(), DT_F32, a, s);
  }
  MM_TRY(np);
  MM_TRY(bn_fwd(ps, bn_out, np, (double)N * Sd * Sd, s));
  MM_TRY(launch_affine_nchw(r_raw, ps.rows(bn_out).scale, ps.rows(bn_out).shift, recon, N, cfg.out_ch, Sd * Sd, s));
  return MMVAE_OK;
}

int Net::decoder_bwd(int N, const float* d_recon, const float* params, float* grads, void* ws, size_t ws_bytes, float* d_enc,
                     hipStream_t s, const GaussTail* gauss) {
  Pass ps;
  MM_TRY(begin_pass(ps, N, ws, ws_bytes, params, grads));
  const Plan& P = *ps.P;
  char* const base = ps.base;
  float* const part = ps.part;
  float* r_raw = reinterpret_cast<float*>(base + P.r_raw);
  float* d_raw = reinterpret_cast<float*>(base + P.d_raw);
  const BnRows r0 = ps.rows(dbn0), ro = ps.rows(bn_out);
  const int HW = Sd * Sd;
  pack_batch_begin();
  MM_TRY(packs_dec_bwd(ps, d_enc != nullptr, s));
  MM_TRY(pack_batch_flush(dt(), s));
  if (stem_bwd_fused() && !gram_ready_ && gram_fwd_N_ == N && gram_fwd_ws_ == ws && wgrad_stream(s) != s) {
    MM_TRY(side_fork(s));
    MM_TRY(launch_stem_gram(dt(), base + P.x_t, reinterpret_cast<float*>(base + P.stem_gram), 1024L * stem_bwd_part_floats(),
                            reinterpret_cast<double*>(base + P.stem_R), N, cfg.S, H1, W1, wgrad_stream(s)));
    if (hipEventRecord(gram_ev_, side_) != hipSuccess) { set_error("side stream mark failed"); return MMVAE_ERR_HIP; }
    gram_ready_ = true;
  }
  int np = gauss ? launch_gauss_tail_reduce(r_raw, gauss->target, ro.scale, ro.shift, gauss->sigma, gauss->coef, gauss->gscale, N, cfg.out_ch,
                                            HW, part, s)
                 : launch_bn_bwd_reduce_nchw(d_recon, r_raw, N, cfg.out_ch, HW, part, s);
  MM_TRY(np);
  MM_TRY(bn_backward_coefs(ps, bn_out, np, 1, 0, (double)N * HW, s, grads + tail_bias));
  if (gauss)
    MM_TRY(launch_gauss_tail_apply(r_raw, gauss->target, ro.scale, ro.shift, gauss->sigma, gauss->coef, gauss->gscale, ro.A, ro.B, ro.C, d_raw,
                                   N, cfg.out_ch, HW, s));
  else
    MM_TRY(launch_bn_bwd_apply_nchw(d_recon, r_raw, ro.A, ro.B, ro.C, d_raw, N, cfg.out_ch, HW, s));
  const bool tail_fused = !dec.empty() && dec.back().C == 16 && tail_join_fusable(dt(), cfg.out_ch, N, Sd, Sd);
  const bool tail_wg_in_reduce = tail_fwd_fused() && tail_fused;
  if (store8 && !tail_wg_in_reduce) { set_error("fp8 storage of the last up-block needs the fused tail backward"); return MMVAE_ERR_UNSUPPORTED; }
  if (!tail_wg_in_reduce) {
    if (tail_fwd_fused()) { set_error("decoder_bwd: the fused tail forward (no stored join) needs the fused tail backward"); return MMVAE_ERR_UNSUPPORTED; }
    WgradArgs a; std::memset(&a, 0, sizeof(a));
    a.P = d_raw; a.P_planar = 1; a.P_planes = cfg.out_ch; a.G = base + dec.back().out; a.dW = grads + tail.off; a.scratch = ps.wscratch;
    a.N = N; a.Hp = Sd; a.Wp = Sd; a.Ca = 16; a.Ca_valid = cfg.out_ch; a.Hg = Sd; a.Wg = Sd; a.Cb = 16; a.Cb_valid = 16;
    a.stride = 1; a.pad = 1; a.ksz = 3; a.sA = 16 * 9; a.sB = 9; a.ntaps = 9; a.scale = 1.f;
    for (int t = 0; t < 9; ++t) a.tap_off[t] = t;
    MM_TRY(side_fork(s));
    MM_TRY(launch_wgrad(dt(), a, wgrad_stream(s)));
  }
  int cur = 0;
  if (!tail_fused) {
    GatherArgs a; std::memset(&a, 0, sizeof(a));
    a.x = d_raw; a.w = ps.packed(tail_pack_d); a.y = base + P.g[cur]; a.x_planar = 1; a.x_planes = cfg.out_ch;
    a.N = N; a.Hi = Sd; a.Wi = Sd; a.Cin = 8; a.Ho = Sd; a.Wo = Sd; a.Cout = 16; a.SI = 1; a.SO = 1;
    a.nphase = 1; a.phases[0] = Phase{0, 0, Sd, Sd, 9, 0, 0};
    for (int kh = 0; kh < 3; ++kh) for (int kw = 0; kw < 3; ++kw) a.taps[kh * 3 + kw] = Tap{1 - kh, 1 - kw};
    MM_TRY(launch_gather_gemm(dt(), dt(), a, s));
  }
  const int nd = (int)dec.size();
  auto jg_block = [&](int j) {
    if (j < 0 || j >= nd || dt() != DT_BF16 || !join_grad_) return false;
    const Block& Bj = dec[j];
    if (Bj.identity || Bj.C != 16 || Bj.c2.fp8 || Bj.cs.fp8 || Bj.c1.fp8 || (j == 0 && cfg.blocks <= 1)) return false;
    return op_bwd_fusable_jg(dt(), geom(Bj.c2), N, Bj.Hin, Bj.Win, Bj.Hout, Bj.Wout, true, false, true) &&
           op_bwd_fusable_jg(dt(), geom(Bj.cs), N, Bj.Hin, Bj.Win, Bj.Hout, Bj.Wout, false, true, false);
  };
  bool g_masked = false;
  for (int i = nd - 1; i >= 0; --i) {
    Block& B = dec[i];
    const bool jg = g_masked;
    g_masked = false;
    const long npo = (long)N * B.Hout * B.Wout, npi = (long)N * B.Hin * B.Win;
    const void* xin = i == 0 ? (cfg.blocks > 1 ? base + P.act0d : base + P.y0d) : base + dec[i - 1].out;
    const float* xs = (i == 0 && cfg.blocks <= 1) ? r0.scale : nullptr;
    const float* xb = (i == 0 && cfg.blocks <= 1) ? r0.shift : nullptr;
    const BnRows r1 = ps.rows(B.b1), r2 = ps.rows(B.b2);
    const Shortcut sc = ps.shortcut(B, xin);
    const int ds = i & 1;
    if (i + 2 <= nd - 1) MM_TRY(side_wait_mark(i + 2, s));
    const bool from_tail = tail_fused && i == nd - 1;
    const long dyso = B.identity ? P.g[cur ^ 1] : P.dys[ds];
    if (from_tail) {
      np = launch_tail_join_bwd_reduce(dt(), d_raw, params + tail.off, cfg.out_ch, N, Sd, Sd, r2.scale, r2.shift, sc.scale, sc.shift, base + B.y2,
                                       sc.y, part, s, tail_wg_in_reduce ? ps.wscratch : nullptr, store8 ? 1 : 0);
      if (tail_wg_in_reduce && np > 0) {
        MM_TRY(side_fork(s));
        MM_TRY(launch_tail_wgrad_finalize(ps.wscratch, np, grads + tail.off, wgrad_stream(s)));
// ... 115 lines not shown
```

### moving-mnist-vae_amd/csrc/vae_net.hpp

```cpp
#pragma once
#include <string>
#include <vector>

#include "comm.hpp"
#include "conv_ops.hpp"
#include "kernels.hpp"

namespace mmvae {

struct NetCfg { int in_ch, z, out_ch, S, need_logvar, dtype, blocks, fp8; };

enum EntryKind : int { EK_PARAM = 0, EK_BN_F32 = 1, EK_BN_I64 = 2 };
struct Entry { std::string name; int ndim; int shape[4]; int kind; long offset; };

struct ConvW { long off; int D0, D1, k, s, p; long packD, packU; int Hl = 0;  bool tr = false;  bool fp8 = false; float wscale = 1.f;
               bool fragD = false, fragU = false;  };
struct Bn {
  long g_off, b_off, rm_off, rv_off; int nbt_idx; int C; long ws;
  enum Row { MEAN, ISTD, SCALE, SHIFT, COEF_A, COEF_B, COEF_C, kRows };
  long row_floats() const { return (C + 3L) / 4 * 4; }
  long row(Row r) const { return ws + r * row_floats(); }
  long scratch_floats() const { return kRows * row_floats(); }
};
struct BnRows { float *mean, *istd, *scale, *shift, *A, *B, *C; };

struct Block {
  ConvW c1, c2, cs; Bn b1, b2, bs;
  int Cin, C, Hin, Win, Hmid, Wmid, Hout, Wout;
  long y1, y2, ys, out;
  bool identity = false;
};

struct Plan {
  int N = -1;
  size_t bytes = 0;
  long x_t, y0, enc_t, y0d, r_raw, d_raw, col;
  long packed;
  long bnws;
  long partials;
  long syncbuf;
  long edy1[2], edy2[2], edys[2];
  long g[2], dy1[2], dy2[2], dys[2], da1, dh;
  long wscratch;
  long wscratch2;
  long stem_R, stem_gram;
  long cvec;
  long act0d;
  long enc_ws_end;
};

constexpr long kPartialFloats = 4096L * 3 * 256;

class Net {
 public:
  explicit Net(const NetCfg& c);
  ~Net();
  Net(const Net&) = delete;
  Net& operator=(const Net&) = delete;
  NetCfg cfg;
  std::vector<Entry> entries;
  long n_params = 0, n_bnbuf = 0; int n_nbt = 0;
  long dec_param_off = 0;
  long n_packed = 0;
  long n_bnws = 0;
  long max_w = 0;
  int H1, W1, Hf, Wf, Sd, nup;
  ConvW stem; Bn bn0;
  std::vector<Block> enc;
  ConvW head_mu, head_lv; long head_pack_mu, head_pack_lv, head_pack_dg;
  ConvW dstem; Bn dbn0;
  std::vector<Block> dec;
  ConvW tail; long tail_bias; Bn bn_out;
  long stem_pack, tail_pack_f, tail_pack_d;

  size_t workspace_bytes(int N);
  const Plan& plan(int N);

  int encoder_fwd(int N, const float* x, const float* params, float* bnbuf, long long* nbt, void* ws, size_t ws_bytes,
                  float* mu, float* logvar, int training, hipStream_t s, bool staged = false);
  int stage_labels(int N, const void* labels, int label_bytes, float mean, float stdv, float* image, void* ws, size_t ws_bytes, hipStream_t s);
  int encoder_bwd(int N, const float* d_mu, const float* d_logvar, const float* params, float* grads, void* ws, size_t ws_bytes,
                  hipStream_t s);
  int decoder_fwd(int N, const float* enc, const float* params, float* bnbuf, long long* nbt, void* ws, size_t ws_bytes,
                  float* recon, int training, hipStream_t s);
  struct GaussTail { const float* target; float sigma; float coef; const float* gscale; };
  int decoder_bwd(int N, const float* d_recon, const float* params, float* grads, void* ws, size_t ws_bytes, float* d_enc,
                  hipStream_t s, const GaussTail* gauss = nullptr);

 private:
  Plan plan_;
  struct Shortcut { const void* y; const float *scale, *shift, *A, *B, *C; };
  struct Pass {
    const Plan* P; char* base; const float* params; float* grads; float* bnbuf; long long* nbt; int N; bool training;
    float* part;
    float* wscratch;
    size_t esz;
    BnRows rows(const Bn& bn) const {
      float* f = reinterpret_cast<float*>(base + P->bnws);
      return BnRows{f + bn.row(Bn::MEAN), f + bn.row(Bn::ISTD), f + bn.row(Bn::SCALE), f + bn.row(Bn::SHIFT),
                    f + bn.row(Bn::COEF_A), f + bn.row(Bn::COEF_B), f + bn.row(Bn::COEF_C)};
    }
    char* packed(long slot) const { return base + P->packed + slot * (long)esz; }
    const float* ones() const { return reinterpret_cast<const float*>(base + P->cvec); }
    const float* zeros() const { return ones() + 256; }
    Shortcut shortcut(const Block& B, const void* xin) const {
      if (B.identity) return Shortcut{xin, ones(), zeros(), ones(), zeros(), zeros()};
      const BnRows r = rows(B.bs);
      return Shortcut{base + B.ys, r.scale, r.shift, r.A, r.B, r.C};
    }
  };
  int begin_pass(Pass& ps, int N, void* ws, size_t ws_bytes, const float* params = nullptr, float* grads = nullptr, float* bnbuf = nullptr,
                 long long* nbt = nullptr, bool training = false);
  static constexpr int kForkEvents = 192;
  hipStream_t side_ = nullptr; hipEvent_t ev_[kForkEvents] = {}; int evi_ = 0; int side_state_ = 0;
  hipStream_t wgrad_stream(hipStream_t s);
  int side_fork(hipStream_t s);
  int side_join(hipStream_t s);
  hipEvent_t gram_ev_ = nullptr;
  bool gram_ready_ = false; int gram_fwd_N_ = 0; const void* gram_fwd_ws_ = nullptr;
  hipEvent_t blk_ev_[16] = {};
  int side_mark(int slot);
  int side_wait_mark(int slot, hipStream_t s);
  int dt() const { return cfg.dtype; }
  size_t esz() const { return dtype_size(cfg.dtype); }
  ConvW add_conv(const std::string& name, int D0, int D1, int k, int s, int p, bool pack, bool transposed = false);
  void settle_layout(ConvW& w) const;
  Bn add_bn(const std::string& prefix, int C);
  void add_entry(const std::string& name, std::initializer_list<int> shape, int kind, long off);

  int packs_enc_fwd(const Pass& ps, hipStream_t s);
  int packs_enc_bwd(const Pass& ps, hipStream_t s);
  int packs_dec_fwd(const Pass& ps, hipStream_t s);
  int packs_dec_bwd(const Pass& ps, bool need_denc, hipStream_t s);
  int pack_down(const Pass& ps, const ConvW& w, hipStream_t s);
  int pack_up(const Pass& ps, const ConvW& w, hipStream_t s);
  int run_down(const Pass& ps, const ConvW& w, const void* L, int Hl, int Wl, void* S, int Hs, int Ws,
               const float* pro_s, const float* pro_b, int relu, float* stats, int accumulate, int out_dt, hipStream_t s,
               const ConvW* w2 = nullptr, const void* x2 = nullptr);
  int run_up(const Pass& ps, const ConvW& w, const void* S, int Hs, int Ws, void* L, int Hl, int Wl,
             const float* pro_s, const float* pro_b, int relu, float* stats, int accumulate, hipStream_t s,
             const ConvW* w2 = nullptr, const void* x2 = nullptr);
  int run_wgrad(const Pass& ps, const ConvW& w, const void* P, int Hs, int Ws, const float* proP_s, const float* proP_b,
                const void* G, int Hl, int Wl, const float* proG_s, const float* proG_b, hipStream_t s);
  int reduce_wgrad_parts(const Pass& ps, const ConvW& w, const float* parts, int nparts, int ntaps, hipStream_t s);
  bool tail_fwd_fused() const;
  bool stem_bwd_fused() const;
  bool stem_dg_fused() const;
  bool defer_join_ = false;
  int (*ar_fn_)(float*, long long, void*, void*) = nullptr; void* ar_user_ = nullptr; int ar_world_ = 1;
  Comm* comm_ = nullptr; Comm* comm_side_ = nullptr;
  int sync_rows(const Pass& ps, const float* partials, int nparts, int width, hipStream_t s, float** out, int row_stride = 0);
 public:
  void set_defer_join(bool v) { defer_join_ = v; }
  bool join_grad_ = true;
  void set_join_grad(bool v) { join_grad_ = v; }
  typedef int (*AllReduceFn)(float* buf, long long n, void* stream, void* user);
  void set_sync_bn(AllReduceFn fn, void* user, int world) { ar_fn_ = fn; ar_user_ = user; ar_world_ = fn ? world : 1; comm_ = comm_side_ = nullptr; }
  void set_sync_bn_comm(Comm* c, Comm* side = nullptr) { comm_ = c; comm_side_ = c ? side : nullptr; ar_fn_ = nullptr; ar_user_ = nullptr; ar_world_ = c ? comm_world(c) : 1; }
  bool sync_bn_on() const { return ar_fn_ != nullptr || comm_ != nullptr; }
  int join(hipStream_t s) { return side_join(s); }
  hipStream_t side() const { return side_state_ == 1 ? side_ : nullptr; }
  hipStream_t fork(hipStream_t s) { return side_fork(s) == MMVAE_OK ? wgrad_stream(s) : s; }
 private:
  int bn_fwd(const Pass& ps, const Bn& bn, int nparts, double count, hipStream_t s, long part_off = 0, float in_scale = 1.f);
  int fold_bn_eval(const Pass& ps, int which, hipStream_t s);
  bool l1_dgrad_stream() const;
  long l1c2_flip = 0;
  bool eval_folded_ = false;
  bool store8 = false;
  int fill_consts(const Pass& ps, hipStream_t s);
  int bn_backward_coefs(const Pass& ps, const Bn& bn, int nparts, int ny, int which, double count, hipStream_t s, float* dbias_conv = nullptr);
  BnBwdFinalizeArgs bwd_finalize_args(const Pass& ps, const Bn& bn, const float* partials, int nparts, int ny, int which, double count) const;
  int bn_backward_coefs_join(const Pass& ps, const Bn& b2, const Bn& bs, int nparts, double count, hipStream_t s);
};

}
```

### moving-mnist-vae_amd/steps.py

```python
from typing import NamedTuple

import torch

from ._lib import SUM_PARTIALS, check, cur_stream, lib, ptr

_Staged = NamedTuple("_Staged", [("image_ref", object), ("version", int), ("ws_ptr", int), ("N", int)])
_Recon = NamedTuple("_Recon", [("data_ptr", int), ("stamp", int)])
_Tail = NamedTuple("_Tail", [("token", torch.Tensor), ("target", torch.Tensor), ("sigma", float), ("coef", float), ("gscale", torch.Tensor),
                             ("stamp", int)])


class _PendingLoss:
    __slots__ = ("side", "closure", "out", "launched")

    def __init__(self, side):
        self.side, self.closure, self.out, self.launched = side, None, None, False

    def launch_on(self, st):
        if not self.launched:
            self.launched = True
            self.closure(st)


class _StepState:
    __slots__ = ("staged", "recon", "tail", "nan_token", "loss")

    def __init__(self):
        self.loss = None
        self.reset()

    def reset(self):
        self.staged = self.recon = self.tail = None
        self.nan_token = None

    @property
    def loss_pending(self):
        return self.loss is not None and not self.loss.launched

    def flush_loss(self, st, only=None):
        if self.loss is not None and (only is None or self.loss.out is only):
            self.loss.launch_on(st)

    def take_staged(self, x, ws, N):
        s, self.staged = self.staged, None
        return s is not None and s.image_ref() is x and s.version == x._version and s.ws_ptr == ws.data_ptr() and s.N == N

    def tail_token(self, like):
        if self.nan_token is None or self.nan_token.device != like.device:
            self.nan_token = torch.full((1,), float("nan"), device=like.device, dtype=torch.float32)
        return self.nan_token.expand(like.shape)


class _EncoderFn(torch.autograd.Function):
    @staticmethod
    def forward(ctx, model, x, *params):
        N = x.shape[0]
        z = model.z_dimensions
        mu = torch.empty((N, z, 1, 1), device=x.device, dtype=torch.float32)
        logvar = torch.empty_like(mu) if model.require_rsample else None
        training = bool(model.training)
        ws = model._workspace(N, training)
        fn = lib().mmvae_encoder_fwd_staged if model._step.take_staged(x, ws, N) else lib().mmvae_encoder_fwd
        check(fn(model._h, N, ptr(x), model._net_ptr(model._flat), ptr(model._bnf), ptr(model._bni), ptr(ws), ws.numel(),
                 ptr(mu), ptr(logvar), int(training), cur_stream()), "mmvae_encoder_fwd")
        ctx.model, ctx.N, ctx.training = model, N, training
        ctx.token = model._stamp("enc", training)
        return mu if logvar is None else (mu, logvar)

    @staticmethod
    def backward(ctx, d_mu, d_logvar=None):
        model = ctx.model
        model._check_stamp("enc", ctx.token, ctx.training)
        z, N = model.z_dimensions, ctx.N
        dev = model._flat.device
        d_mu = torch.zeros((N, z), device=dev) if d_mu is None else d_mu.contiguous().float()
        if model.require_rsample:
            d_logvar = torch.zeros((N, z), device=dev) if d_logvar is None else d_logvar.contiguous().float()
        G = model._grad_target()
        G[model._poff:model._dec_off].zero_()
        ws = model._workspace(N, True)
        check(lib().mmvae_encoder_bwd(model._h, N, ptr(d_mu), ptr(d_logvar), model._net_ptr(model._flat), model._net_ptr(G), ptr(ws), ws.numel(),
                                      cur_stream()), "mmvae_encoder_bwd")
        if model._sync is not None:
            model._sync.bucket_ready(G, 0, model._dec_off)
        return (None, None) + model._grad_views(G, model._enc_rows)


class _DecoderFn(torch.autograd.Function):
    @staticmethod
    def forward(ctx, model, encoding, *params):
        N = encoding.shape[0]
        training = bool(model.training)
        recon = torch.empty((N, model.decoder_out_channels, model._dec_side, model._dec_side), device=encoding.device, dtype=torch.float32)
        ws = model._workspace(N, training)
        check(lib().mmvae_decoder_fwd(model._h, N, ptr(encoding), model._net_ptr(model._flat), ptr(model._bnf), ptr(model._bni), ptr(ws), ws.numel(),
                                      ptr(recon), int(training), cur_stream()), "mmvae_decoder_fwd")
        ctx.model, ctx.N, ctx.training = model, N, training
        ctx.token = model._stamp("dec", training)
        ctx.need_denc = bool(ctx.needs_input_grad[1])
        model._step.recon = _Recon(recon.data_ptr(), ctx.token) if training else None
        return recon

    @staticmethod
    def backward(ctx, d_recon):
        model = ctx.model
        model._check_stamp("dec", ctx.token, ctx.training)
        N = ctx.N
        step = model._step
        tail, step.tail = step.tail, None
        fused_tail = (tail is not None and tail.stamp == ctx.token and d_recon.stride(0) == 0 and d_recon.data_ptr() == tail.token.data_ptr())
        if not fused_tail:
            d_recon = d_recon.contiguous().float()
        d_enc = torch.empty((N, model.z_dimensions, 1, 1), device=d_recon.device, dtype=torch.float32) if ctx.need_denc else None
        G = model._grad_target()
        G[model._dec_off:].zero_()
        ws = model._workspace(N, True)
        h, st = model._h, cur_stream()

        def join_at_end_of_backward():
            torch.autograd.Variable._execution_engine.queue_callback(lambda: check(lib().mmvae_net_join(h, st), "mmvae_net_join"))
        defer = model.defer_join
        check(lib().mmvae_net_defer_join(h, int(defer)), "mmvae_net_defer_join")
        if fused_tail:
            check(lib().mmvae_decoder_bwd_gauss(h, N, ptr(tail.target), tail.sigma, tail.coef, ptr(tail.gscale), model._net_ptr(model._flat),
                                                model._net_ptr(G), ptr(ws), ws.numel(), ptr(d_enc), st), "mmvae_decoder_bwd_gauss")
        else:
            check(lib().mmvae_decoder_bwd(h, N, ptr(d_recon), model._net_ptr(model._flat), model._net_ptr(G), ptr(ws), ws.numel(), ptr(d_enc), st),
                  "mmvae_decoder_bwd")
        if defer:
            join_at_end_of_backward()
        if model._sync is not None:
            model._sync.bucket_ready(G, model._dec_off, model._n_params, side_of=model if defer else None)
        if step.loss_pending:
            side = lib().mmvae_net_side_stream(h)
            step.loss.launch_on(side if side else st)
            if side and not defer:
                join_at_end_of_backward()
        return (None, d_enc) + model._grad_views(G, model._dec_rows)


class _PixelFn(torch.autograd.Function):

    @staticmethod
    def forward(ctx, model, x, *params):
        N, S = x.shape[0], x.shape[2]
        x = x.contiguous().float()
        with torch.no_grad():
            model._flat[:model._poff].mul_(model._pix_mask)
        out = torch.empty((N, model.pixelcnn_out_channels, S, S), device=x.device, dtype=torch.float32)
        ws = model._pixel_workspace(N, S)
        check(lib().mmvae_pixelcnn_fwd(model._hp, N, S, ptr(x), ptr(model._flat), ptr(ws), ws.numel(), ptr(out), cur_stream()), "mmvae_pixelcnn_fwd")
        ctx.model, ctx.N, ctx.S = model, N, S
        ctx.token = model._stamp("pix", True)
        ctx.need_dx = bool(ctx.needs_input_grad[1])
        ctx.save_for_backward(x)
        return out

    @staticmethod
    def backward(ctx, d_out):
        model, N, S = ctx.model, ctx.N, ctx.S
        model._check_stamp("pix", ctx.token, True, "the saved activations of this PixelCNN forward were overwritten by a later forward")
        (x,) = ctx.saved_tensors
        d_out = d_out.contiguous().float()
        G = model._grad_target()
        G[:model._poff].zero_()
        d_x = torch.empty_like(x) if ctx.need_dx else None
        ws = model._pixel_workspace(N, S)
        check(lib().mmvae_pixelcnn_bwd(model._hp, N, S, ptr(x), ptr(d_out), ptr(model._flat), ptr(G), ptr(ws), ws.numel(), ptr(d_x), cur_stream()),
              "mmvae_pixelcnn_bwd")
        return (None, d_x) + model._grad_views(G, model._pix_rows)


class _RsampleFn(torch.autograd.Function):
    @staticmethod
    def forward(ctx, mu, logvar, eps):
        mu, logvar, eps = mu.contiguous(), logvar.contiguous(), eps.contiguous()
        enc = torch.empty_like(mu)
        check(lib().mmvae_rsample_fwd(ptr(mu), ptr(logvar), ptr(eps), ptr(enc), mu.numel(), cur_stream()), "mmvae_rsample_fwd")
# ... 3 lines not shown
    @staticmethod
    def backward(ctx, d_enc):
        logvar, eps = ctx.saved_tensors
        d_enc = d_enc.contiguous()
        d_mu, d_lv = torch.empty_like(d_enc), torch.empty_like(d_enc)
        check(lib().mmvae_rsample_bwd(ptr(d_enc), ptr(logvar), ptr(eps), ptr(d_mu), ptr(d_lv), d_enc.numel(), cur_stream()), "mmvae_rsample_bwd")
        return d_mu, d_lv, None


class _LossFn(torch.autograd.Function):

    @staticmethod
    def forward(ctx, model, rec, target, mu, logvar, encoding, recon, true_samples, weight):
        L = lib()
        N, dev, step = target.shape[0], recon.device, model._step
        acc = torch.zeros(4 + SUM_PARTIALS, dtype=torch.float64, device=dev)
        out = torch.empty(4, dtype=torch.float32, device=dev)
        step.flush_loss(cur_stream())
        base, part = acc.data_ptr(), acc.data_ptr() + 32
        recon = recon.contiguous()
        categorical = model.is_categorical()
        if mu is not None and logvar is not None:
            mu, logvar = mu.contiguous(), logvar.contiguous()
        scratch = None
        if encoding is not None:
            encoding = encoding.contiguous()
            scratch = torch.empty(2 * N, dtype=torch.float32, device=dev)
        target = target.contiguous()
        nll_c, kl_c, mmd_c, sigma = float(model.nll), float(model.kl), float(model.mmd), float(model.sigma_decoder)
        det = lambda t: None if t is None else t.detach()
        k_mu, k_lv, k_enc, k_rec, k_tgt, k_ts, k_w = det(mu), det(logvar), det(encoding), det(recon), det(target), det(true_samples), det(weight)

        def launch(st):
            if k_mu is not None and k_lv is not None:
                check(L.mmvae_kl_fwd_ex(ptr(k_mu), ptr(k_lv), k_mu.numel(), base + 8, part, st), "mmvae_kl_fwd_ex")
            if k_enc is not None:
                check(L.mmvae_mmd_fwd_ex(ptr(k_ts), ptr(k_enc), N, k_enc.shape[1], ptr(scratch), base + 16, part, st), "mmvae_mmd_fwd_ex")
            if categorical:
                Q, HW = k_rec.shape[1], k_rec.shape[2] * k_rec.shape[3]
                check(L.mmvae_ce_fwd_ex(ptr(k_rec), ptr(k_tgt), ptr(k_w), N, Q, HW, base, part, st), "mmvae_ce_fwd_ex")
            else:
                check(L.mmvae_gauss_nll_fwd_ex(ptr(k_rec), ptr(k_tgt), k_rec.numel(), sigma, base, part, st), "mmvae_gauss_nll_fwd_ex")
            check(L.mmvae_loss_finish(base, ptr(out), nll_c, kl_c, mmd_c, float(N), st), "mmvae_loss_finish")
            _ = acc

        rec.closure, rec.out = launch, out
        step.loss = rec
        if not rec.side:
            rec.launch_on(cur_stream())
        ctx.model, ctx.N, ctx.categorical = model, N, categorical
        lr = step.recon
        ctx.direct_tail = (lr.stamp if (lr is not None and lr.data_ptr == recon.data_ptr() and not categorical and model.fuse_loss_tail and
                                        target.dtype == torch.float32 and target.shape == recon.shape) else None)
        ctx.save_for_backward(target, mu, logvar, encoding, recon, true_samples, weight)
        return out[0]

    @staticmethod
    def backward(ctx, g):
        L = lib()
        model, N = ctx.model, ctx.N
        target, mu, logvar, encoding, recon, ts, weight = ctx.saved_tensors
        st = cur_stream()
        g = g.contiguous().float()
        sigma, coef = float(model.sigma_decoder), float(model.nll) / N
        if ctx.direct_tail is not None and model._stamps.get(("dec", True)) == ctx.direct_tail:
            d_recon = model._step.tail_token(recon)
            model._step.tail = _Tail(d_recon, target, sigma, coef, g, ctx.direct_tail)
        else:
            d_recon = torch.empty_like(recon)
            if ctx.categorical:
                Q, HW = recon.shape[1], recon.shape[2] * recon.shape[3]
                check(L.mmvae_ce_bwd(ptr(recon), ptr(target), ptr(weight), N, Q, HW, coef, ptr(g), ptr(d_recon), st), "mmvae_ce_bwd")
            else:
                check(L.mmvae_gauss_nll_bwd(ptr(recon), ptr(target), recon.numel(), sigma, coef, ptr(g), ptr(d_recon), st), "mmvae_gauss_nll_bwd")
        d_mu = d_lv = d_enc = None
        if mu is not None and logvar is not None:
            d_mu, d_lv = torch.empty_like(mu), torch.empty_like(logvar)
            check(L.mmvae_kl_bwd(ptr(mu), ptr(logvar), float(model.kl) / N, ptr(g), ptr(d_mu), ptr(d_lv), mu.numel(), st), "mmvae_kl_bwd")
        if encoding is not None and float(model.mmd) != 0.0:
            d_enc = torch.zeros_like(encoding)
            check(L.mmvae_mmd_bwd(ptr(ts), ptr(encoding), N, encoding.shape[1], float(model.mmd) / N, ptr(g), ptr(d_enc), st), "mmvae_mmd_bwd")
        return None, None, None, d_mu, d_lv, d_enc, d_recon, None, None
```

Before: 866,300 frames/s.

## Compute Gaussian tail BN-backward sums during decoder forward and read byte targets

The decoder forward now fuses the final affine write with the per-channel reductions of the Gaussian NLL gradient (sum of d and d*x), using the staged target image. The backward can then skip its separate tail reduce pass and scale the stored sums by the loss gradient scale. Both the forward tail and the backward apply can read the target from a uint8 label buffer through a 256-entry shared-memory lookup table, which cuts bytes read. The cost is more bookkeeping: stamps, weakrefs and version checks to make sure the forward sums still match the target used in backward.

```diff
diff --git a/include/mmvae.h b/include/mmvae.h
--- a/include/mmvae.h
+++ b/include/mmvae.h
@@ -61,6 +61,14 @@
 MMVAE_API void* mmvae_net_fork(mmvae_net* net, void* stream);
 MMVAE_API void* mmvae_net_side_stream(mmvae_net* net);
 MMVAE_API int mmvae_net_set_join_grad(mmvae_net* net, int enable);
+MMVAE_API int mmvae_decoder_fwd_tail(mmvae_net* net, int N, const float* encoding, const float* params, float* bn_f32, int64_t* bn_i64,
+                           void* workspace, size_t workspace_bytes, float* recon, int training, const float* target, float sigma, float coef,
+                           void* stream);
+MMVAE_API int mmvae_decoder_bwd_gauss_sums(mmvae_net* net, int N, const float* target, float sigma, float coef, const float* gscale,
+                                 const float* params, float* grads, void* workspace, size_t workspace_bytes, float* d_enc, int use_fwd_sums,
+                                 void* stream);
+MMVAE_API int mmvae_net_set_fwd_tail_sums(mmvae_net* net, int enable);
+MMVAE_API int64_t mmvae_net_tail_reduce_launches(mmvae_net* net);
 
 typedef int (*mmvae_allreduce_fn)(float* buf, int64_t n, void* stream, void* user);
 MMVAE_API int mmvae_net_set_sync_bn(mmvae_net* net, mmvae_allreduce_fn fn, void* user, int world);
@@ -199,6 +207,17 @@
                         void* scratch, void* stream);
 MMVAE_API int mmvae_batchnorm_bwd(int dtype, const void* dout, const void* y, const void* out, int64_t npix, int C, const float* gamma,
                         const float* save_mean, const float* save_istd, void* dy, float* dgamma, float* dbeta, void* scratch, void* stream);
+MMVAE_API int mmvae_affine_nchw(const float* raw, const float* scale, const float* shift, float* out, int N, int C, int HW, void* stream);
+MMVAE_API int mmvae_recon_tail_fwd(const float* raw, const float* scale, const float* shift, float* out, const float* target,
+                         const uint8_t* target_u8, float mean, float stdv, float sigma, float coef, int N, int C, int HW, float* partials,
+                         void* stream);
+MMVAE_API int mmvae_gauss_tail_reduce(const float* raw, const float* target, const float* scale, const float* shift, float sigma, float coef,
+                            const float* gscale, int N, int C, int HW, float* partials, void* stream);
+MMVAE_API int mmvae_gauss_tail_finalize(const float* partials, int rows, int C, double count, const float* gamma, const float* mean, const float* istd,
+                              const float* sum_scale, float* dgamma, float* dbeta, float* A, float* B, float* Cc, void* stream);
+MMVAE_API int mmvae_gauss_tail_apply(const float* raw, const float* target, const uint8_t* target_u8, float mean, float stdv, const float* scale,
+                           const float* shift, float sigma, float coef, const float* gscale, const float* A, const float* B, const float* Cc,
+                           float* d_raw, int N, int C, int HW, void* stream);
 #define MMVAE_STEM_SCRATCH_BYTES 12800u
 MMVAE_API int mmvae_stem_fwd(int dtype, const void* x, const float* weight, void* y, int N, int S, float* stats, void* scratch, void* stream);
 MMVAE_API int mmvae_stem_bwd(int dtype, const void* g, const void* y0, const void* x, const float* weight, const float* gamma,
diff --git a/moving-mnist-vae_amd/_lib.py b/moving-mnist-vae_amd/_lib.py
--- a/moving-mnist-vae_amd/_lib.py
+++ b/moving-mnist-vae_amd/_lib.py
@@ -38,6 +38,10 @@
     "mmvae_net_fork": (P, [P, P]),
     "mmvae_net_side_stream": (P, [P]),
     "mmvae_net_set_join_grad": (c_int, [P, c_int]),
+    "mmvae_decoder_fwd_tail": (c_int, [P, c_int, P, P, P, P, P, c_size_t, P, c_int, P, c_float, c_float, P]),
+    "mmvae_decoder_bwd_gauss_sums": (c_int, [P, c_int, P, c_float, c_float, P, P, P, P, c_size_t, P, c_int, P]),
+    "mmvae_net_set_fwd_tail_sums": (c_int, [P, c_int]),
+    "mmvae_net_tail_reduce_launches": (c_int64, [P]),
     "mmvae_net_set_sync_bn": (c_int, [P, P, P, c_int]),
     "mmvae_rsample_fwd": (c_int, [P, P, P, P, c_int64, P]),
     "mmvae_rsample_bwd": (c_int, [P, P, P, P, P, c_int64, P]),
@@ -96,6 +100,11 @@
     "mmvae_convT_bwd_fused": (c_int, [c_int, P, P, P, P, P, c_int, c_int, c_int, c_int, c_int, c_int, c_int, c_int, P, P, c_int, P, P, P, P, P, P]),
     "mmvae_batchnorm_fwd": (c_int, [c_int, P, c_int64, c_int, P, P, P, P, P, c_float, c_float, c_int, P, P, P, P, P]),
     "mmvae_batchnorm_bwd": (c_int, [c_int, P, P, P, c_int64, c_int, P, P, P, P, P, P, P, P]),
+    "mmvae_affine_nchw": (c_int, [P, P, P, P, c_int, c_int, c_int, P]),
+    "mmvae_recon_tail_fwd": (c_int, [P, P, P, P, P, P, c_float, c_float, c_float, c_float, c_int, c_int, c_int, P, P]),
+    "mmvae_gauss_tail_reduce": (c_int, [P, P, P, P, c_float, c_float, P, c_int, c_int, c_int, P, P]),
+    "mmvae_gauss_tail_finalize": (c_int, [P, c_int, c_int, c_double, P, P, P, P, P, P, P, P, P, P]),
+    "mmvae_gauss_tail_apply": (c_int, [P, P, P, c_float, c_float, P, P, c_float, c_float, P, P, P, P, P, c_int, c_int, c_int, P]),
     "mmvae_stem_fwd": (c_int, [c_int, P, P, P, c_int, c_int, P, P, P]),
     "mmvae_stem_bwd": (c_int, [c_int, P, P, P, P, P, P, P, P, P, P, P, P, c_int, c_int, P, P]),
     "mmvae_tail_join_fwd": (c_int, [c_int, P, P, P, P, P, P, P, P, P, P, c_int, c_int, c_int, P]),
diff --git a/moving-mnist-vae_amd/csrc/bn_elem.hip b/moving-mnist-vae_amd/csrc/bn_elem.hip
--- a/moving-mnist-vae_amd/csrc/bn_elem.hip
+++ b/moving-mnist-vae_amd/csrc/bn_elem.hip
@@ -342,6 +342,7 @@
     const int nw = blockDim.x >> 6;
     s0 = 0.0; s1 = 0.0;
     for (int w = 0; w < nw; ++w) { s0 += sRed[w]; s1 += sRed[4 + w]; }
+    if (a.sum_scale) { const double up = (double)a.sum_scale[0]; s0 *= up; s1 *= up; }
     const double mean = a.mean[c], istd = a.istd[c], g = a.gamma ? a.gamma[c] : 1.0;
     const double sgy = istd * (s1 - mean * s0);
     if (a.dgamma) a.dgamma[c] += (float)sgy;
@@ -1162,10 +1163,123 @@
   const int rc = check_launch("gauss_tail_reduce");
   return rc ? rc : blocks;
 }
-__global__ __launch_bounds__(256) void gauss_tail_apply_kernel(const float* __restrict__ raw, const float* __restrict__ tgt, const float* __restrict__ scale,
-                                                                const float* __restrict__ shift, float k, const float* __restrict__ gs,
-                                                                const float* __restrict__ A, const float* __restrict__ B, const float* __restrict__ Cc,
-                                                                float* __restrict__ dy, int planes, int C, int HW) {
+struct ByteTarget { const unsigned char* lab8; float mean, stdv; };
+template <bool BYTES>
+__device__ __forceinline__ void tail_target_table(float* sLut, const ByteTarget& bt) {
+  if (BYTES) sLut[threadIdx.x] = ((float)threadIdx.x - bt.mean) / bt.stdv;
+}
+template <bool BYTES>
+__device__ __forceinline__ float tail_target1(const float* __restrict__ pt, const unsigned char* __restrict__ pl, const float* sLut, int i) {
+  if (!BYTES) return pt[i];
+  const unsigned char b = pl[i];
+  return b != 255 ? sLut[b] : pt[i];
+}
+template <bool BYTES>
+__device__ __forceinline__ float4 tail_target4(const float* __restrict__ pt, const unsigned char* __restrict__ pl, const float* sLut, int i) {
+  if (!BYTES) return *reinterpret_cast<const float4*>(pt + i);
+  const uchar4 b = *reinterpret_cast<const uchar4*>(pl + i);
+  float4 t;
+  t.x = b.x != 255 ? sLut[b.x] : pt[i]; t.y = b.y != 255 ? sLut[b.y] : pt[i + 1];
+  t.z = b.z != 255 ? sLut[b.z] : pt[i + 2]; t.w = b.w != 255 ? sLut[b.w] : pt[i + 3];
+  return t;
+}
+
+template <bool SUMS, bool BYTES>
+__global__ __launch_bounds__(256) void recon_tail_fwd_kernel(const float* __restrict__ raw, const float* __restrict__ tgt, ByteTarget bt,
+                                                              const float* __restrict__ scale, const float* __restrict__ shift, float k, int N, int C,
+                                                              int HW, float* __restrict__ recon, float* __restrict__ partials) {
+  extern __shared__ float sm[];
+  __shared__ float sLut[BYTES ? 256 : 1];
+  float* sAcc = sm;
+  const int wid = threadIdx.x >> 6;
+  if (SUMS) {
+    for (int i = threadIdx.x; i < 4 * 2 * C; i += blockDim.x) sAcc[i] = 0.f;
+    tail_target_table<BYTES>(sLut, bt);
+    __syncthreads();
+  }
+  const int planes = N * C;
+  for (int p = blockIdx.x; p < planes; p += gridDim.x) {
+    const int c = p % C;
+    const float sc = scale[c], sh = shift[c];
+    const float* pa = raw + (long)p * HW;
+    const float* pt = SUMS ? tgt + (long)p * HW : nullptr;
+    const unsigned char* pl = BYTES ? bt.lab8 + (long)p * HW : nullptr;
+    float* po = recon + (long)p * HW;
+    float v0 = 0.f, v1 = 0.f;
+    if ((HW & 3) == 0) {
+      constexpr int U = 4;
+      const int stride = 4 * blockDim.x;
+      for (int i0 = threadIdx.x * 4; i0 < HW; i0 += U * stride) {
+        float4 x[U], t[U];
+#pragma unroll
+        for (int u = 0; u < U; ++u) {
+          const int i = i0 + u * stride;
+          if (i < HW) {
+            x[u] = *reinterpret_cast<const float4*>(pa + i);
+            if (SUMS) t[u] = tail_target4<BYTES>(pt, pl, sLut, i);
+          }
+        }
+#pragma unroll
+        for (int u = 0; u < U; ++u) {
+          const int i = i0 + u * stride;
+          if (i < HW) {
+            float4 r;
+            r.x = __builtin_fmaf(sc, x[u].x, sh); r.y = __builtin_fmaf(sc, x[u].y, sh); r.z = __builtin_fmaf(sc, x[u].z, sh); r.w = __builtin_fmaf(sc, x[u].w, sh);
+            *reinterpret_cast<float4*>(po + i) = r;
+            if (SUMS) {
+              const float d0 = k * (r.x - t[u].x), d1 = k * (r.y - t[u].y), d2 = k * (r.z - t[u].z), d3 = k * (r.w - t[u].w);
+              v0 += (d0 + d1) + (d2 + d3);
+              v1 += (d0 * x[u].x + d1 * x[u].y) + (d2 * x[u].z + d3 * x[u].w);
+            }
+          }
+        }
+      }
+    } else {
+      for (int i = threadIdx.x; i < HW; i += blockDim.x) {
+        const float x = pa[i], r = __builtin_fmaf(sc, x, sh);
+        po[i] = r;
+        if (SUMS) { const float d = k * (r - tail_target1<BYTES>(pt, pl, sLut, i)); v0 += d; v1 += d * x; }
+      }
+    }
+    if (SUMS) {
+      v0 = wave_sum(v0); v1 = wave_sum(v1);
+      if ((threadIdx.x & 63) == 0) { sAcc[wid * 2 * C + c] += v0; sAcc[wid * 2 * C + C + c] += v1; }
+    }
+  }
+  if (SUMS) {
+    __syncthreads();
+    for (int i = threadIdx.x; i < 2 * C; i += blockDim.x)
+      partials[(long)blockIdx.x * 2 * C + i] = (sAcc[i] + sAcc[2 * C + i]) + (sAcc[2 * 2 * C + i] + sAcc[3 * 2 * C + i]);
+  }
+}
+int launch_recon_tail_fwd(const float* raw, const float* scale, const float* shift, float* recon, const float* target, float sigma, float coef,
+                          int N, int C, int HW, float* partials, hipStream_t s, const unsigned char* lab8, float mean, float stdv) {
+  if (target && !partials) { set_error("recon_tail_fwd: a target needs the partial rows' buffer"); return MMVAE_ERR_ARG; }
+  const ByteTarget bt{lab8, mean, stdv};
+  if (target) {
+    const int blocks = nchw_parts(N, C);
+    const size_t sm = (size_t)4 * 2 * C * sizeof(float);
+    const float k = coef / (sigma * sigma);
+    if (lab8) hipLaunchKernelGGL((recon_tail_fwd_kernel<true, true>), dim3(blocks), dim3(256), sm, s, raw, target, bt, scale, shift, k, N, C, HW, recon, partials);
+    else hipLaunchKernelGGL((recon_tail_fwd_kernel<true, false>), dim3(blocks), dim3(256), sm, s, raw, target, bt, scale, shift, k, N, C, HW, recon, partials);
+    note_launch_bytes((double)N * C * HW * (lab8 ? 9.0 : 12.0));
+    const int rc = check_launch("recon_tail_fwd");
+    return rc ? rc : blocks;
+  }
+  const int planes = N * C;
+  hipLaunchKernelGGL((recon_tail_fwd_kernel<false, false>), dim3(planes < 4096 ? planes : 4096), dim3(256), 0, s, raw, nullptr, bt, scale, shift, 0.f, N, C, HW, recon,
+                     nullptr);
+  note_launch_bytes((double)N * C * HW * 8.0);
+  return check_launch("recon_tail_fwd");
+}
+
+template <bool BYTES>
+__global__ __launch_bounds__(256) void gauss_tail_apply_kernel(const float* __restrict__ raw, const float* __restrict__ tgt, ByteTarget bt,
+                                                                const float* __restrict__ scale, const float* __restrict__ shift, float k,
+                                                                const float* __restrict__ gs, const float* __restrict__ A, const float* __restrict__ B,
+                                                                const float* __restrict__ Cc, float* __restrict__ dy, int planes, int C, int HW) {
+  __shared__ float sLut[BYTES ? 256 : 1];
+  if (BYTES) { tail_target_table<BYTES>(sLut, bt); __syncthreads(); }
   if (gs) k *= gs[0];
   for (int p = blockIdx.x; p < planes; p += gridDim.x) {
     const int c = p % C;
@@ -1174,7 +1288,7 @@
     if ((HW & 3) == 0) {
       for (int i = threadIdx.x * 4; i < HW; i += 1024) {
         const float4 x = *reinterpret_cast<const float4*>(raw + base + i);
-        const float4 t = *reinterpret_cast<const float4*>(tgt + base + i);
+        const float4 t = tail_target4<BYTES>(tgt + base, BYTES ? bt.lab8 + base : nullptr, sLut, i);
         float4 o;
         o.x = ca * (k * ((sc * x.x + sh) - t.x)) + cb * x.x + cc; o.y = ca * (k * ((sc * x.y + sh) - t.y)) + cb * x.y + cc;
         o.z = ca * (k * ((sc * x.z + sh) - t.z)) + cb * x.z + cc; o.w = ca * (k * ((sc * x.w + sh) - t.w)) + cb * x.w + cc;
@@ -1183,18 +1297,22 @@
     } else {
       for (int i = threadIdx.x; i < HW; i += 256) {
         const float x = raw[base + i];
-        dy[base + i] = ca * (k * ((sc * x + sh) - tgt[base + i])) + cb * x + cc;
+        dy[base + i] = ca * (k * ((sc * x + sh) - tail_target1<BYTES>(tgt + base, BYTES ? bt.lab8 + base : nullptr, sLut, i))) + cb * x + cc;
       }
     }
   }
 }
 int launch_gauss_tail_apply(const float* raw, const float* target, const float* scale, const float* shift, float sigma, float coef, const float* gscale,
-                            const float* A, const float* B, const float* Cc, float* dy, int N, int C, int HW, hipStream_t s) {
+                            const float* A, const float* B, const float* Cc, float* dy, int N, int C, int HW, hipStream_t s,
+                            const unsigned char* lab8, float mean, float stdv) {
   if (C > 64) { set_error("gauss_tail_apply: C=%d > 64", C); return MMVAE_ERR_UNSUPPORTED; }
   const int planes = N * C;
   const int blocks = planes < 4096 ? planes : 4096;
-  hipLaunchKernelGGL(gauss_tail_apply_kernel, dim3(blocks), dim3(256), 0, s, raw, target, scale, shift, coef / (sigma * sigma), gscale, A, B, Cc, dy, planes, C, HW);
-  note_launch_bytes((double)N * C * HW * 12.0);
+  const ByteTarget bt{lab8, mean, stdv};
+  const float k = coef / (sigma * sigma);
+  if (lab8) hipLaunchKernelGGL((gauss_tail_apply_kernel<true>), dim3(blocks), dim3(256), 0, s, raw, target, bt, scale, shift, k, gscale, A, B, Cc, dy, planes, C, HW);
+  else hipLaunchKernelGGL((gauss_tail_apply_kernel<false>), dim3(blocks), dim3(256), 0, s, raw, target, bt, scale, shift, k, gscale, A, B, Cc, dy, planes, C, HW);
+  note_launch_bytes((double)N * C * HW * (lab8 ? 9.0 : 12.0));
   return check_launch("gauss_tail_apply");
 }
 
diff --git a/moving-mnist-vae_amd/csrc/capi.cpp b/moving-mnist-vae_amd/csrc/capi.cpp
--- a/moving-mnist-vae_amd/csrc/capi.cpp
+++ b/moving-mnist-vae_amd/csrc/capi.cpp
@@ -109,6 +109,27 @@
   return n->net->decoder_bwd(N, nullptr, params, grads, ws, wsb, d_enc, stream_of(stream), &gt);
 }
 
+int mmvae_decoder_fwd_tail(mmvae_net* n, int N, const float* enc, const float* params, float* bn_f32, int64_t* bn_i64, void* ws, size_t wsb,
+                           float* recon, int training, const float* target, float sigma, float coef, void* stream) {
+  if (!n || N <= 0 || !enc || !params || !ws || !recon || !bn_f32) { set_error("decoder_fwd_tail: bad argument"); return MMVAE_ERR_ARG; }
+  if (target && !(sigma > 0.f)) { set_error("decoder_fwd_tail: sigma must be positive"); return MMVAE_ERR_ARG; }
+  const Net::GaussTail gt{target, sigma, coef, nullptr};
+  return n->net->decoder_fwd(N, enc, params, bn_f32, reinterpret_cast<long long*>(bn_i64), ws, wsb, recon, training, stream_of(stream),
+                             target ? &gt : nullptr);
+}
+int mmvae_decoder_bwd_gauss_sums(mmvae_net* n, int N, const float* target, float sigma, float coef, const float* gscale, const float* params,
+                                 float* grads, void* ws, size_t wsb, float* d_enc, int use_fwd_sums, void* stream) {
+  if (!n || N <= 0 || !target || !params || !grads || !ws || !(sigma > 0.f)) { set_error("decoder_bwd_gauss_sums: bad argument"); return MMVAE_ERR_ARG; }
+  const Net::GaussTail gt{target, sigma, coef, gscale};
+  return n->net->decoder_bwd(N, nullptr, params, grads, ws, wsb, d_enc, stream_of(stream), &gt, use_fwd_sums != 0);
+}
+int mmvae_net_set_fwd_tail_sums(mmvae_net* n, int enable) {
+  if (!n) { set_error("net_set_fwd_tail_sums: bad argument"); return MMVAE_ERR_ARG; }
+  n->net->set_fwd_tail_sums(enable != 0);
+  return MMVAE_OK;
+}
+int64_t mmvae_net_tail_reduce_launches(mmvae_net* n) { return n ? (int64_t)n->net->tail_reduce_launches() : -1; }
+
 int mmvae_net_defer_join(mmvae_net* n, int enable) {
   if (!n) { set_error("net_defer_join: bad argument"); return MMVAE_ERR_ARG; }
   n->net->set_defer_join(enable != 0);
@@ -533,6 +554,45 @@
   int rc = launch_bn_bwd_finalize(f, stream_of(st));
   if (rc < 0) return rc;
   return launch_bn_bwd_apply(dt, dout, out, nullptr, nullptr, y, coef, coef + C, coef + 2 * C, dy, nullptr, nullptr, nullptr, nullptr, nullptr, npix, C, stream_of(st));
+}
+static bool tail_op_shape_ok(const char* what, int N, int C, int HW) {
+  if (N >= 1 && C >= 1 && HW >= 1 && (long)N * C <= 0x7fffffffL) return true;
+  set_error("%s: bad shape", what);
+  return false;
+}
+int mmvae_affine_nchw(const float* raw, const float* scale, const float* shift, float* out, int N, int C, int HW, void* st) {
+  if (!raw || !scale || !shift || !out) { set_error("affine_nchw: bad argument"); return MMVAE_ERR_ARG; }
+  if (!tail_op_shape_ok("affine_nchw", N, C, HW)) return MMVAE_ERR_ARG;
+  return launch_affine_nchw(raw, scale, shift, out, N, C, HW, stream_of(st));
+}
+int mmvae_recon_tail_fwd(const float* raw, const float* scale, const float* shift, float* out, const float* target, const uint8_t* target_u8,
+                         float mean, float stdv, float sigma, float coef, int N, int C, int HW, float* partials, void* st) {
+  if (!raw || !scale || !shift || !out || (target && (!partials || !(sigma > 0.f))) || (target_u8 && !target)) {
+    set_error("recon_tail_fwd: bad argument"); return MMVAE_ERR_ARG;
+  }
+  if (!tail_op_shape_ok("recon_tail_fwd", N, C, HW)) return MMVAE_ERR_ARG;
+  return launch_recon_tail_fwd(raw, scale, shift, out, target, target ? sigma : 1.f, coef, N, C, HW, partials, stream_of(st), target_u8, mean, stdv);
+}
+int mmvae_gauss_tail_reduce(const float* raw, const float* target, const float* scale, const float* shift, float sigma, float coef,
+                            const float* gscale, int N, int C, int HW, float* partials, void* st) {
+  if (!raw || !target || !scale || !shift || !partials || !(sigma > 0.f)) { set_error("gauss_tail_reduce: bad argument"); return MMVAE_ERR_ARG; }
+  if (!tail_op_shape_ok("gauss_tail_reduce", N, C, HW)) return MMVAE_ERR_ARG;
+  return launch_gauss_tail_reduce(raw, target, scale, shift, sigma, coef, gscale, N, C, HW, partials, stream_of(st));
+}
+int mmvae_gauss_tail_finalize(const float* partials, int rows, int C, double count, const float* gamma, const float* mean, const float* istd,
+                              const float* sum_scale, float* dgamma, float* dbeta, float* A, float* B, float* Cc, void* st) {
+  if (!partials || rows < 1 || C < 1 || !(count > 0.0) || !mean || !istd || !A || !B || !Cc) { set_error("gauss_tail_finalize: bad argument"); return MMVAE_ERR_ARG; }
+  BnBwdFinalizeArgs f; std::memset(&f, 0, sizeof(f));
+  f.partials = partials; f.nparts = rows; f.C = C; f.which = 0; f.ny = 1; f.count = count; f.gamma = gamma; f.mean = mean; f.istd = istd;
+  f.dgamma = dgamma; f.dbeta = dbeta; f.coefA = A; f.coefB = B; f.coefC = Cc; f.dbias_scale = 1.f; f.sum_scale = sum_scale;
+  return launch_bn_bwd_finalize(f, stream_of(st));
+}
+int mmvae_gauss_tail_apply(const float* raw, const float* target, const uint8_t* target_u8, float mean, float stdv, const float* scale,
+                           const float* shift, float sigma, float coef, const float* gscale, const float* A, const float* B, const float* Cc,
+                           float* d_raw, int N, int C, int HW, void* st) {
+  if (!raw || !target || !scale || !shift || !A || !B || !Cc || !d_raw || !(sigma > 0.f)) { set_error("gauss_tail_apply: bad argument"); return MMVAE_ERR_ARG; }
+  if (!tail_op_shape_ok("gauss_tail_apply", N, C, HW)) return MMVAE_ERR_ARG;
+  return launch_gauss_tail_apply(raw, target, scale, shift, sigma, coef, gscale, A, B, Cc, d_raw, N, C, HW, stream_of(st), target_u8, mean, stdv);
 }
 static_assert(MMVAE_STEM_SCRATCH_BYTES >= 32 * 25 * 16, "stem scratch: 32 columns x 25 taps x one 16-byte vector of padded input channels");
 int mmvae_stem_fwd(int dt, const void* x, const float* w, void* y, int N, int Sz, float* stats, void* scratch, void* st) {
diff --git a/moving-mnist-vae_amd/csrc/kernels.hpp b/moving-mnist-vae_amd/csrc/kernels.hpp
--- a/moving-mnist-vae_amd/csrc/kernels.hpp
+++ b/moving-mnist-vae_amd/csrc/kernels.hpp
@@ -215,6 +215,7 @@
   const float* partials; int nparts; int C; int which ; int ny; double count;
   const float* gamma; const float* mean; const float* istd; float* dgamma; float* dbeta; float* coefA; float* coefB; float* coefC;
   float* dbias_conv = nullptr; float dbias_scale = 1.f;
+  const float* sum_scale = nullptr;
 };
 int launch_bn_bwd_finalize(const BnBwdFinalizeArgs& a, hipStream_t s);
 int launch_bn_bwd_finalize2(const BnBwdFinalizeArgs& a0, const BnBwdFinalizeArgs& a1, hipStream_t s);
@@ -240,7 +241,10 @@
 int launch_gauss_tail_reduce(const float* raw, const float* target, const float* scale, const float* shift, float sigma, float coef, const float* gscale,
                              int N, int C, int HW, float* partials, hipStream_t s);
 int launch_gauss_tail_apply(const float* raw, const float* target, const float* scale, const float* shift, float sigma, float coef, const float* gscale,
-                            const float* A, const float* B, const float* Cc, float* dy, int N, int C, int HW, hipStream_t s);
+                            const float* A, const float* B, const float* Cc, float* dy, int N, int C, int HW, hipStream_t s,
+                            const unsigned char* lab8 = nullptr, float mean = 0.f, float stdv = 1.f);
+int launch_recon_tail_fwd(const float* raw, const float* scale, const float* shift, float* recon, const float* target, float sigma, float coef,
+                          int N, int C, int HW, float* partials, hipStream_t s, const unsigned char* lab8 = nullptr, float mean = 0.f, float stdv = 1.f);
 
 int launch_inorm_planar_fwd(int dt, const float* x, void* xn16, float* stats, int N, int C, int HW, hipStream_t s);
 int launch_inorm_planar2_fwd(int dt, const float* xa, int Ca, const float* xb, int Cb, void* xn16, float* stats, int N, int HW, hipStream_t s);
@@ -290,7 +294,8 @@
 int launch_adam_dev(const AdamArgs& a, double* state, hipStream_t s);
 int launch_grad_norm_sq(const float* g, long n, float grad_scale, double* acc, double* part, hipStream_t s);
 int launch_adam_guarded(const AdamArgs& a, double* state, double* part, float max_norm, hipStream_t s);
-int launch_normalise(int dt, const void* labels, int label_bytes, long n, float mean, float stdv, void* img_t, float* img_f32, hipStream_t s);
+int launch_normalise(int dt, const void* labels, int label_bytes, long n, float mean, float stdv, void* img_t, float* img_f32, hipStream_t s,
+                     unsigned char* lab8 = nullptr);
 int launch_quantise_normalise(const unsigned char* frames, long n, const float* centres, int q, float mean, float stdv,
                               long long* labels, float* image, hipStream_t s);
 int launch_u8_histogram(const unsigned char* frames, long clip_bytes, const long long* clip_index, long n_clips,
diff --git a/moving-mnist-vae_amd/csrc/latent_loss.hip b/moving-mnist-vae_amd/csrc/latent_loss.hip
--- a/moving-mnist-vae_amd/csrc/latent_loss.hip
+++ b/moving-mnist-vae_amd/csrc/latent_loss.hip
@@ -580,16 +580,21 @@
   return check_launch("adam_guarded");
 }
 
+template <typename TL>
+__device__ __forceinline__ unsigned char label_byte(TL l) { return (unsigned long long)l < 255ull ? (unsigned char)l : (unsigned char)255; }
 template <typename T, typename TL>
-__global__ void normalise_kernel(const TL* __restrict__ labels, long n, long nq, float mean, float stdv, T* __restrict__ img, float* __restrict__ img32) {
+__global__ void normalise_kernel(const TL* __restrict__ labels, long n, long nq, float mean, float stdv, T* __restrict__ img, float* __restrict__ img32,
+                                 unsigned char* __restrict__ lab8) {
   for (long q = (long)blockIdx.x * blockDim.x + threadIdx.x; q < nq; q += (long)gridDim.x * blockDim.x) {
     float v[4];
     if constexpr (sizeof(TL) == 8) {
       const longlong2 a = reinterpret_cast<const longlong2*>(labels)[2 * q], b = reinterpret_cast<const longlong2*>(labels)[2 * q + 1];
       v[0] = (float)a.x; v[1] = (float)a.y; v[2] = (float)b.x; v[3] = (float)b.y;
+      if (lab8) reinterpret_cast<uchar4*>(lab8)[q] = make_uchar4(label_byte(a.x), label_byte(a.y), label_byte(b.x), label_byte(b.y));
     } else {
       const uchar4 a = reinterpret_cast<const uchar4*>(labels)[q];
       v[0] = (float)a.x; v[1] = (float)a.y; v[2] = (float)a.z; v[3] = (float)a.w;
+      if (lab8) reinterpret_cast<uchar4*>(lab8)[q] = a;
     }
 #pragma unroll
     for (int j = 0; j < 4; ++j) v[j] = (v[j] - mean) / stdv;
@@ -603,21 +608,23 @@
     const float v = ((float)labels[i] - mean) / stdv;
     if (img) Elem<T>::store(img + i, v);
     if (img32) img32[i] = v;
-  }
-}
-int launch_normalise(int dt, const void* labels, int label_bytes, long n, float mean, float stdv, void* img_t, float* img_f32, hipStream_t s) {
+    if (lab8) lab8[i] = label_byte(labels[i]);
+  }
+}
+int launch_normalise(int dt, const void* labels, int label_bytes, long n, float mean, float stdv, void* img_t, float* img_f32, hipStream_t s,
+                     unsigned char* lab8) {
   if (n <= 0) return MMVAE_OK;
   if (label_bytes != 8 && label_bytes != 1) { set_error("normalise: labels must be int64 or uint8"); return MMVAE_ERR_ARG; }
   const bool aligned = reinterpret_cast<uintptr_t>(labels) % (label_bytes == 8 ? 16 : 4) == 0 && reinterpret_cast<uintptr_t>(img_f32) % 16 == 0 &&
-                       reinterpret_cast<uintptr_t>(img_t) % (dt == DT_F32 ? 16 : 8) == 0;
+                       reinterpret_cast<uintptr_t>(img_t) % (dt == DT_F32 ? 16 : 8) == 0 && reinterpret_cast<uintptr_t>(lab8) % 4 == 0;
   const long nq = aligned ? n >> 2 : 0;
   const dim3 g(rblocks(aligned ? (n >> 2) + 1 : n, 2048)), b(256);
   if (label_bytes == 8) {
-    if (dt == DT_F32) hipLaunchKernelGGL((normalise_kernel<float, long long>), g, b, 0, s, (const long long*)labels, n, nq, mean, stdv, (float*)img_t, img_f32);
-    else hipLaunchKernelGGL((normalise_kernel<bf16_t, long long>), g, b, 0, s, (const long long*)labels, n, nq, mean, stdv, (bf16_t*)img_t, img_f32);
+    if (dt == DT_F32) hipLaunchKernelGGL((normalise_kernel<float, long long>), g, b, 0, s, (const long long*)labels, n, nq, mean, stdv, (float*)img_t, img_f32, lab8);
+    else hipLaunchKernelGGL((normalise_kernel<bf16_t, long long>), g, b, 0, s, (const long long*)labels, n, nq, mean, stdv, (bf16_t*)img_t, img_f32, lab8);
   } else {
-    if (dt == DT_F32) hipLaunchKernelGGL((normalise_kernel<float, unsigned char>), g, b, 0, s, (const unsigned char*)labels, n, nq, mean, stdv, (float*)img_t, img_f32);
-    else hipLaunchKernelGGL((normalise_kernel<bf16_t, unsigned char>), g, b, 0, s, (const unsigned char*)labels, n, nq, mean, stdv, (bf16_t*)img_t, img_f32);
+    if (dt == DT_F32) hipLaunchKernelGGL((normalise_kernel<float, unsigned char>), g, b, 0, s, (const unsigned char*)labels, n, nq, mean, stdv, (float*)img_t, img_f32, lab8);
+    else hipLaunchKernelGGL((normalise_kernel<bf16_t, unsigned char>), g, b, 0, s, (const unsigned char*)labels, n, nq, mean, stdv, (bf16_t*)img_t, img_f32, lab8);
   }
   return check_launch("normalise");
 }
diff --git a/moving-mnist-vae_amd/csrc/vae_net.cpp b/moving-mnist-vae_amd/csrc/vae_net.cpp
--- a/moving-mnist-vae_amd/csrc/vae_net.cpp
+++ b/moving-mnist-vae_amd/csrc/vae_net.cpp
@@ -203,6 +203,8 @@
   P.wscratch2 = take(2L * 1024 * 4096 * 4);
   P.stem_R = take(1024 * 8);
   P.stem_gram = take(1024L * stem_bwd_part_floats() * 4);
+  P.tail_sums = take(1024L * 2 * cfg.out_ch * 4);
+  P.label_u8 = take((long)N * cfg.in_ch * cfg.S * cfg.S);
   P.bytes = (size_t)cur;
   plan_ = P;
   return plan_;
@@ -391,14 +393,18 @@
   a.coefA = r.A; a.coefB = r.B; a.coefC = r.C;
   return a;
 }
-int Net::bn_backward_coefs(const Pass& ps, const Bn& bn, int nparts, int ny, int which, double count, hipStream_t s, float* dbias_conv) {
-  BnBwdFinalizeArgs l = bwd_finalize_args(ps, bn, ps.part, nparts, ny, which, count);
+int Net::bn_backward_coefs(const Pass& ps, const Bn& bn, int nparts, int ny, int which, double count, hipStream_t s, float* dbias_conv,
+                           const float* partials, const float* sum_scale) {
+  if (!partials) partials = ps.part;
+  BnBwdFinalizeArgs l = bwd_finalize_args(ps, bn, partials, nparts, ny, which, count);
+  l.sum_scale = sum_scale;
   if (!sync_bn_on()) l.dbias_conv = dbias_conv;
   MM_TRY(launch_bn_bwd_finalize(l, s));
   if (!sync_bn_on()) return MMVAE_OK;
   float* row = nullptr;
-  MM_TRY(sync_rows(ps, ps.part, nparts, (1 + ny) * bn.C, s, &row));
+  MM_TRY(sync_rows(ps, partials, nparts, (1 + ny) * bn.C, s, &row));
   BnBwdFinalizeArgs g = bwd_finalize_args(ps, bn, row, 1, ny, which, count * ar_world_);
+  g.sum_scale = sum_scale;
   g.dgamma = nullptr; g.dbeta = nullptr;
   g.dbias_conv = dbias_conv; g.dbias_scale = 1.f / (float)ar_world_;
   return launch_bn_bwd_finalize(g, s);
@@ -496,7 +502,9 @@
 int Net::stage_labels(int N, const void* labels, int label_bytes, float mean, float stdv, float* image, void* ws, size_t ws_bytes, hipStream_t s) {
   Pass ps;
   MM_TRY(begin_pass(ps, N, ws, ws_bytes));
-  return launch_normalise(dt(), labels, label_bytes, (long)N * cfg.in_ch * cfg.S * cfg.S, mean, stdv, ps.base + ps.P->x_t, image, s);
+  staged_u8_ = StagedBytes{image, ws, N, mean, stdv, staged_u8_.gen + 1};
+  return launch_normalise(dt(), labels, label_bytes, (long)N * cfg.in_ch * cfg.S * cfg.S, mean, stdv, ps.base + ps.P->x_t, image, s,
+                          reinterpret_cast<unsigned char*>(ps.base + ps.P->label_u8));
 }
 
 int Net::encoder_fwd(int N, const float* x, const float* params, float* bnbuf, long long* nbt, void* ws, size_t ws_bytes,
@@ -735,13 +743,14 @@
 }
 
 int Net::decoder_fwd(int N, const float* encv, const float* params, float* bnbuf, long long* nbt, void* ws, size_t ws_bytes,
-                     float* recon, int training, hipStream_t s) {
+                     float* recon, int training, hipStream_t s, const GaussTail* tail_hint) {
   Pass ps;
   MM_TRY(begin_pass(ps, N, ws, ws_bytes, params, nullptr, bnbuf, nbt, training != 0));
   const Plan& P = *ps.P;
   char* const base = ps.base;
   float* const part = ps.part;
   float* stats = training ? part : nullptr;
+  fwd_tail_ = FwdTail{};
   pack_batch_begin();
   MM_TRY(packs_dec_fwd(ps, s));
   MM_TRY(pack_batch_flush(dt(), s));
@@ -842,12 +851,32 @@
   }
   MM_TRY(np);
   MM_TRY(bn_fwd(ps, bn_out, np, (double)N * Sd * Sd, s));
-  MM_TRY(launch_affine_nchw(r_raw, ps.rows(bn_out).scale, ps.rows(bn_out).shift, recon, N, cfg.out_ch, Sd * Sd, s));
+  if (!fwd_tail_sums_) return launch_affine_nchw(r_raw, ps.rows(bn_out).scale, ps.rows(bn_out).shift, recon, N, cfg.out_ch, Sd * Sd, s);
+  const bool sums = training && tail_hint && tail_hint->target && tail_hint->sigma > 0.f;
+  const StagedBytes& sb = staged_u8_;
+  const bool bytes = sums && sb.image == tail_hint->target && sb.ws == ws && sb.N == N && cfg.in_ch == cfg.out_ch && cfg.S == Sd;
+  if (sums) MM_TRY(launch_gram(ps, N, s));
+  np = launch_recon_tail_fwd(r_raw, ps.rows(bn_out).scale, ps.rows(bn_out).shift, recon, sums ? tail_hint->target : nullptr, sums ? tail_hint->sigma : 1.f,
+                             sums ? tail_hint->coef : 0.f, N, cfg.out_ch, Sd * Sd, reinterpret_cast<float*>(base + P.tail_sums), s,
+                             bytes ? reinterpret_cast<const unsigned char*>(base + P.label_u8) : nullptr, sb.mean, sb.stdv);
+  MM_TRY(np);
+  if (sums) fwd_tail_ = FwdTail{tail_hint->target, tail_hint->sigma, tail_hint->coef, N, ws, np, bytes, sb.gen};
+  return MMVAE_OK;
+}
+
+int Net::launch_gram(const Pass& ps, int N, hipStream_t s) {
+  if (!stem_bwd_fused() || gram_ready_ || gram_fwd_N_ != N || gram_fwd_ws_ != ps.base || wgrad_stream(s) == s) return MMVAE_OK;
+  const Plan& P = *ps.P;
+  MM_TRY(side_fork(s));
+  MM_TRY(launch_stem_gram(dt(), ps.base + P.x_t, reinterpret_cast<float*>(ps.base + P.stem_gram), 1024L * stem_bwd_part_floats(),
+                          reinterpret_cast<double*>(ps.base + P.stem_R), N, cfg.S, H1, W1, wgrad_stream(s)));
+  if (hipEventRecord(gram_ev_, side_) != hipSuccess) { set_error("side stream mark failed"); return MMVAE_ERR_HIP; }
+  gram_ready_ = true;
   return MMVAE_OK;
 }
 
 int Net::decoder_bwd(int N, const float* d_recon, const float* params, float* grads, void* ws, size_t ws_bytes, float* d_enc,
-                     hipStream_t s, const GaussTail* gauss) {
+                     hipStream_t s, const GaussTail* gauss, bool use_fwd_sums) {
   Pass ps;
   MM_TRY(begin_pass(ps, N, ws, ws_bytes, params, grads));
   const Plan& P = *ps.P;
@@ -860,21 +889,26 @@
   pack_batch_begin();
   MM_TRY(packs_dec_bwd(ps, d_enc != nullptr, s));
   MM_TRY(pack_batch_flush(dt(), s));
-  if (stem_bwd_fused() && !gram_ready_ && gram_fwd_N_ == N && gram_fwd_ws_ == ws && wgrad_stream(s) != s) {
-    MM_TRY(side_fork(s));
-    MM_TRY(launch_stem_gram(dt(), base + P.x_t, reinterpret_cast<float*>(base + P.stem_gram), 1024L * stem_bwd_part_floats(),
-                            reinterpret_cast<double*>(base + P.stem_R), N, cfg.S, H1, W1, wgrad_stream(s)));
-    if (hipEventRecord(gram_ev_, side_) != hipSuccess) { set_error("side stream mark failed"); return MMVAE_ERR_HIP; }
-    gram_ready_ = true;
-  }
-  int np = gauss ? launch_gauss_tail_reduce(r_raw, gauss->target, ro.scale, ro.shift, gauss->sigma, gauss->coef, gauss->gscale, N, cfg.out_ch,
-                                            HW, part, s)
-                 : launch_bn_bwd_reduce_nchw(d_recon, r_raw, N, cfg.out_ch, HW, part, s);
+  MM_TRY(launch_gram(ps, N, s));
+  const FwdTail& ft = fwd_tail_;
+  const bool fwd_sums = gauss && use_fwd_sums && fwd_tail_sums_ && ft.nparts > 0 && ft.target == gauss->target && ft.sigma == gauss->sigma &&
+                        ft.coef == gauss->coef && ft.N == N && ft.ws == ws;
+  if (gauss && !fwd_sums) ++tail_reduce_launches_;
+  int np = fwd_sums ? ft.nparts
+         : gauss    ? launch_gauss_tail_reduce(r_raw, gauss->target, ro.scale, ro.shift, gauss->sigma, gauss->coef, gauss->gscale, N, cfg.out_ch,
+                                               HW, part, s)
+                    : launch_bn_bwd_reduce_nchw(d_recon, r_raw, N, cfg.out_ch, HW, part, s);
   MM_TRY(np);
-  MM_TRY(bn_backward_coefs(ps, bn_out, np, 1, 0, (double)N * HW, s, grads + tail_bias));
-  if (gauss)
+  if (fwd_sums)
+    MM_TRY(bn_backward_coefs(ps, bn_out, np, 1, 0, (double)N * HW, s, grads + tail_bias, reinterpret_cast<const float*>(base + P.tail_sums), gauss->gscale));
+  else
+    MM_TRY(bn_backward_coefs(ps, bn_out, np, 1, 0, (double)N * HW, s, grads + tail_bias));
+  if (gauss) {
+    const bool bytes = fwd_sums && ft.bytes && staged_u8_.gen == ft.stage_gen && staged_u8_.ws == ws;
     MM_TRY(launch_gauss_tail_apply(r_raw, gauss->target, ro.scale, ro.shift, gauss->sigma, gauss->coef, gauss->gscale, ro.A, ro.B, ro.C, d_raw,
-                                   N, cfg.out_ch, HW, s));
+                                   N, cfg.out_ch, HW, s, bytes ? reinterpret_cast<const unsigned char*>(base + P.label_u8) : nullptr,
+                                   staged_u8_.mean, staged_u8_.stdv));
+  }
   else
     MM_TRY(launch_bn_bwd_apply_nchw(d_recon, r_raw, ro.A, ro.B, ro.C, d_raw, N, cfg.out_ch, HW, s));
   const bool tail_fused = !dec.empty() && dec.back().C == 16 && tail_join_fusable(dt(), cfg.out_ch, N, Sd, Sd);
diff --git a/moving-mnist-vae_amd/csrc/vae_net.hpp b/moving-mnist-vae_amd/csrc/vae_net.hpp
--- a/moving-mnist-vae_amd/csrc/vae_net.hpp
+++ b/moving-mnist-vae_amd/csrc/vae_net.hpp
@@ -46,6 +46,8 @@
   long stem_R, stem_gram;
   long cvec;
   long act0d;
+  long label_u8;
+  long tail_sums;
   long enc_ws_end;
 };
 
@@ -81,11 +83,12 @@
   int stage_labels(int N, const void* labels, int label_bytes, float mean, float stdv, float* image, void* ws, size_t ws_bytes, hipStream_t s);
   int encoder_bwd(int N, const float* d_mu, const float* d_logvar, const float* params, float* grads, void* ws, size_t ws_bytes,
                   hipStream_t s);
+  struct GaussTail;
   int decoder_fwd(int N, const float* enc, const float* params, float* bnbuf, long long* nbt, void* ws, size_t ws_bytes,
-                  float* recon, int training, hipStream_t s);
+                  float* recon, int training, hipStream_t s, const GaussTail* tail_hint = nullptr);
   struct GaussTail { const float* target; float sigma; float coef; const float* gscale; };
   int decoder_bwd(int N, const float* d_recon, const float* params, float* grads, void* ws, size_t ws_bytes, float* d_enc,
-                  hipStream_t s, const GaussTail* gauss = nullptr);
+                  hipStream_t s, const GaussTail* gauss = nullptr, bool use_fwd_sums = false);
 
  private:
   Plan plan_;
@@ -154,6 +157,9 @@
   void set_defer_join(bool v) { defer_join_ = v; }
   bool join_grad_ = true;
   void set_join_grad(bool v) { join_grad_ = v; }
+  bool fwd_tail_sums_ = true;
+  void set_fwd_tail_sums(bool v) { fwd_tail_sums_ = v; fwd_tail_ = FwdTail{}; }
+  long tail_reduce_launches() const { return tail_reduce_launches_; }
   typedef int (*AllReduceFn)(float* buf, long long n, void* stream, void* user);
   void set_sync_bn(AllReduceFn fn, void* user, int world) { ar_fn_ = fn; ar_user_ = user; ar_world_ = fn ? world : 1; comm_ = comm_side_ = nullptr; }
   void set_sync_bn_comm(Comm* c, Comm* side = nullptr) { comm_ = c; comm_side_ = c ? side : nullptr; ar_fn_ = nullptr; ar_user_ = nullptr; ar_world_ = c ? comm_world(c) : 1; }
@@ -169,7 +175,15 @@
   bool eval_folded_ = false;
   bool store8 = false;
   int fill_consts(const Pass& ps, hipStream_t s);
-  int bn_backward_coefs(const Pass& ps, const Bn& bn, int nparts, int ny, int which, double count, hipStream_t s, float* dbias_conv = nullptr);
+  int bn_backward_coefs(const Pass& ps, const Bn& bn, int nparts, int ny, int which, double count, hipStream_t s, float* dbias_conv = nullptr,
+                        const float* partials = nullptr, const float* sum_scale = nullptr);
+  struct FwdTail { const float* target = nullptr; float sigma = 0.f, coef = 0.f; int N = 0; const void* ws = nullptr; int nparts = 0;
+                   bool bytes = false; long stage_gen = 0; };
+  FwdTail fwd_tail_;
+  struct StagedBytes { const float* image = nullptr; const void* ws = nullptr; int N = 0; float mean = 0.f, stdv = 1.f; long gen = 0; };
+  StagedBytes staged_u8_;
+  int launch_gram(const Pass& ps, int N, hipStream_t s);
+  long tail_reduce_launches_ = 0;
   BnBwdFinalizeArgs bwd_finalize_args(const Pass& ps, const Bn& bn, const float* partials, int nparts, int ny, int which, double count) const;
   int bn_backward_coefs_join(const Pass& ps, const Bn& b2, const Bn& bs, int nparts, double count, hipStream_t s);
 };
diff --git a/moving-mnist-vae_amd/steps.py b/moving-mnist-vae_amd/steps.py
--- a/moving-mnist-vae_amd/steps.py
+++ b/moving-mnist-vae_amd/steps.py
@@ -1,3 +1,4 @@
+import weakref
 from typing import NamedTuple
 
 import torch
@@ -5,9 +6,10 @@
 from ._lib import SUM_PARTIALS, check, cur_stream, lib, ptr
 
 _Staged = NamedTuple("_Staged", [("image_ref", object), ("version", int), ("ws_ptr", int), ("N", int)])
-_Recon = NamedTuple("_Recon", [("data_ptr", int), ("stamp", int)])
+_FwdImage = NamedTuple("_FwdImage", [("image_ref", object), ("version", int), ("N", int)])
+_Recon = NamedTuple("_Recon", [("data_ptr", int), ("stamp", int), ("hint", object)])
 _Tail = NamedTuple("_Tail", [("token", torch.Tensor), ("target", torch.Tensor), ("sigma", float), ("coef", float), ("gscale", torch.Tensor),
-                             ("stamp", int)])
+                             ("stamp", int), ("fwd_sums", bool)])
 
 
 class _PendingLoss:
@@ -23,7 +25,7 @@
 
 
 class _StepState:
-    __slots__ = ("staged", "recon", "tail", "nan_token", "loss")
+    __slots__ = ("staged", "fwd_image", "recon", "tail", "nan_token", "loss")
 
     def __init__(self):
         self.loss = None
@@ -31,6 +33,7 @@
 
     def reset(self):
         self.staged = self.recon = self.tail = None
+        self.fwd_image = None
         self.nan_token = None
 
     @property
@@ -44,6 +47,13 @@
     def take_staged(self, x, ws, N):
         s, self.staged = self.staged, None
         return s is not None and s.image_ref() is x and s.version == x._version and s.ws_ptr == ws.data_ptr() and s.N == N
+
+    def take_fwd_image(self, N, shape):
+        f, self.fwd_image = self.fwd_image, None
+        x = None if f is None else f.image_ref()
+        if x is None or f.version != x._version or f.N != N or tuple(x.shape) != tuple(shape) or x.dtype != torch.float32 or not x.is_contiguous():
+            return None, None
+        return f, x
 
     def tail_token(self, like):
         if self.nan_token is None or self.nan_token.device != like.device:
@@ -60,7 +70,9 @@
         logvar = torch.empty_like(mu) if model.require_rsample else None
         training = bool(model.training)
         ws = model._workspace(N, training)
-        fn = lib().mmvae_encoder_fwd_staged if model._step.take_staged(x, ws, N) else lib().mmvae_encoder_fwd
+        staged = model._step.take_staged(x, ws, N)
+        fn = lib().mmvae_encoder_fwd_staged if staged else lib().mmvae_encoder_fwd
+        model._step.fwd_image = _FwdImage(weakref.ref(x), x._version, N) if staged and training else None
         check(fn(model._h, N, ptr(x), model._net_ptr(model._flat), ptr(model._bnf), ptr(model._bni), ptr(ws), ws.numel(),
                  ptr(mu), ptr(logvar), int(training), cur_stream()), "mmvae_encoder_fwd")
         ctx.model, ctx.N, ctx.training = model, N, training
@@ -93,12 +105,16 @@
         training = bool(model.training)
         recon = torch.empty((N, model.decoder_out_channels, model._dec_side, model._dec_side), device=encoding.device, dtype=torch.float32)
         ws = model._workspace(N, training)
-        check(lib().mmvae_decoder_fwd(model._h, N, ptr(encoding), model._net_ptr(model._flat), ptr(model._bnf), ptr(model._bni), ptr(ws), ws.numel(),
-                                      ptr(recon), int(training), cur_stream()), "mmvae_decoder_fwd")
+        hint, image = model._step.take_fwd_image(N, recon.shape)
+        if not (training and hint is not None and model.fuse_loss_tail and not model.is_categorical() and float(model.sigma_decoder) > 0.0):
+            hint = image = None
+        check(lib().mmvae_decoder_fwd_tail(model._h, N, ptr(encoding), model._net_ptr(model._flat), ptr(model._bnf), ptr(model._bni), ptr(ws),
+                                           ws.numel(), ptr(recon), int(training), ptr(image), float(model.sigma_decoder), float(model.nll) / N,
+                                           cur_stream()), "mmvae_decoder_fwd_tail")
         ctx.model, ctx.N, ctx.training = model, N, training
         ctx.token = model._stamp("dec", training)
         ctx.need_denc = bool(ctx.needs_input_grad[1])
-        model._step.recon = _Recon(recon.data_ptr(), ctx.token) if training else None
+        model._step.recon = _Recon(recon.data_ptr(), ctx.token, hint) if training else None
         return recon
 
     @staticmethod
@@ -122,8 +138,9 @@
         defer = model.defer_join
         check(lib().mmvae_net_defer_join(h, int(defer)), "mmvae_net_defer_join")
         if fused_tail:
-            check(lib().mmvae_decoder_bwd_gauss(h, N, ptr(tail.target), tail.sigma, tail.coef, ptr(tail.gscale), model._net_ptr(model._flat),
-                                                model._net_ptr(G), ptr(ws), ws.numel(), ptr(d_enc), st), "mmvae_decoder_bwd_gauss")
+            check(lib().mmvae_decoder_bwd_gauss_sums(h, N, ptr(tail.target), tail.sigma, tail.coef, ptr(tail.gscale), model._net_ptr(model._flat),
+                                                     model._net_ptr(G), ptr(ws), ws.numel(), ptr(d_enc), int(tail.fwd_sums), st),
+                  "mmvae_decoder_bwd_gauss_sums")
         else:
             check(lib().mmvae_decoder_bwd(h, N, ptr(d_recon), model._net_ptr(model._flat), model._net_ptr(G), ptr(ws), ws.numel(), ptr(d_enc), st),
                   "mmvae_decoder_bwd")
@@ -233,6 +250,8 @@
         lr = step.recon
         ctx.direct_tail = (lr.stamp if (lr is not None and lr.data_ptr == recon.data_ptr() and not categorical and model.fuse_loss_tail and
                                         target.dtype == torch.float32 and target.shape == recon.shape) else None)
+        hint = lr.hint if ctx.direct_tail is not None else None
+        ctx.fwd_sums = hint is not None and hint.image_ref() is target and hint.version == target._version
         ctx.save_for_backward(target, mu, logvar, encoding, recon, true_samples, weight)
         return out[0]
 
@@ -246,7 +265,7 @@
         sigma, coef = float(model.sigma_decoder), float(model.nll) / N
         if ctx.direct_tail is not None and model._stamps.get(("dec", True)) == ctx.direct_tail:
             d_recon = model._step.tail_token(recon)
-            model._step.tail = _Tail(d_recon, target, sigma, coef, g, ctx.direct_tail)
+            model._step.tail = _Tail(d_recon, target, sigma, coef, g, ctx.direct_tail, ctx.fwd_sums)
         else:
             d_recon = torch.empty_like(recon)
             if ctx.categorical:
```

Measured after the change: 869,200 frames/s, median of 6. Within noise of the previous version (+0.3%).
